# OndrejSladky/kmercamel

Hardware: NVIDIA B200
Metric: distinct k-mers/sec for `compute` (k=31, canonical, device-timed) (higher is better)
Workload: dtype u64

## Files before the change

### kmercamel_b200/csrc/emit.cuh

```cuda
#pragma once
#include "engine.cuh"

template <int L> struct NodeSeq {
    const KWord<L> *kmers;
    const u8 *seq;
    const u64 *rec_off, *rec_len;
    u32 n;
    int k;
    KC_HD u64 length(u32 v) const { return kmers ? (u64) k : rec_len[v < n ? v : v - n]; }
    KC_HD u32 symbol(u32 v, u64 pos) const {
        if (kmers) {
            if (v < n) return kmer_symbol(kmers[v], k, (int) pos);
            return 3u - kmer_symbol(kmers[v - n], k, k - 1 - (int) pos);
        }
        if (v < n) return kc_nucleotide_code(seq[rec_off[v] + pos]);
        u32 u = v - n;
        return 3u - kc_nucleotide_code(seq[rec_off[u] + rec_len[u] - 1 - pos]);
    }
};

KC_HD u8 kc_letter(u32 sym, bool upper) {
    const u32 packed = 'A' | ('C' << 8) | ('G' << 16) | ('T' << 24);
    u8 c = (u8) (packed >> (8 * sym));
    return upper ? c : (u8) (c + ('a' - 'A'));
}

template <int L> KC_HD u64 kmer_lower_bound(const KWord<L> *keys, u64 n, const KWord<L> &x) {
    u64 lo = 0, hi = n;
    while (lo < hi) {
        u64 mid = (lo + hi) >> 1;
        if (keys[mid] < x) lo = mid + 1;
        else hi = mid;
    }
    return lo;
}

template <int L> struct KmerIndex {
    const u32 *start = nullptr;
    int bits = 0, shift = 0;
};

template <int L> KC_HD bool kmer_set_contains(const KWord<L> *keys, u64 n, const KmerIndex<L> &ix, const KWord<L> &x) {
    u64 lo = 0, hi = n;
    if (ix.start) {
        const u32 b = x.digit(ix.shift, ix.bits);
        lo = ix.start[b];
        hi = ix.start[b + 1];
    }
    while (lo < hi) {
        const u64 mid = (lo + hi) >> 1;
        if (keys[mid] < x) lo = mid + 1;
        else hi = mid;
    }
    return lo < n && keys[lo] == x;
}

static const u32 KC_EMIT_SHORT = 128;
static const u32 KC_EMIT_CHUNK = 16384;
static const u32 KC_EMIT_SUB = 4;

#ifdef __CUDACC__
template <int L> KmerIndex<L> kc_kmer_index_build(CudaExec &ex, const KWord<L> *keys, u64 n, int k) {
    KmerIndex<L> ix;
    if (n < 1024 || n >= 0xFFFFFFFFULL) return ix;
    int bits = kc_ceil_log2(n) - 1;
    if (bits > 24) bits = 24;
    if (bits > 2 * k) bits = 2 * k;
    const u64 nb = 1ULL << bits;
    u32 *start = ex.alloc<u32>(nb + 1);
    const int shift = 2 * k - bits;
    ex.for_each(n + 1, [=] __device__(u64 i) {
        const u64 b_prev = i == 0 ? 0 : (u64) keys[i - 1].digit(shift, bits) + 1;
        const u64 b_cur = i == n ? nb : (u64) keys[i].digit(shift, bits);
        for (u64 b = b_prev; b <= b_cur; ++b) start[b] = (u32) i;
    }, KP_MISC, n * sizeof(KWord<L>) + nb * 4);
    ix.start = start;
    ix.bits = bits;
    ix.shift = shift;
    return ix;
}

static const u32 KC_RANK_SMALL = 1024;

template <int L>
__global__ void __launch_bounds__(256) kc_rank_small_kernel(PathState s, NodeSeq<L> q, u32 N, u32 *fin_out, u64 *dist_out, u64 *cell) {
    __shared__ u32 jump[2][KC_RANK_SMALL], fin[2][KC_RANK_SMALL];
    __shared__ u64 dist[2][KC_RANK_SMALL];
    __shared__ u32 s_start, s_cyc;
    if (threadIdx.x == 0) {
        s_start = KC_NONE;
        s_cyc = 0;
    }
    __syncthreads();
    for (u32 v = threadIdx.x; v < N; v += 256) {
        const u32 nx = s.edge_from[v];
        jump[0][v] = nx;
        fin[0][v] = v;
        dist[0][v] = q.length(v) - (nx != KC_NONE ? (u64) s.ovl[v] : 0);
        if (s.edge_to[v] == KC_NONE) atomicMin(&s_start, v);
    }
    __syncthreads();
    int rounds = 1;
    while ((1u << (rounds - 1)) < N) ++rounds;
    int cur = 0;
    for (int it = 0; it < rounds; ++it) {
        for (u32 v = threadIdx.x; v < N; v += 256) {
            const u32 j = jump[cur][v];
            if (j == KC_NONE) {
                jump[cur ^ 1][v] = KC_NONE;
                fin[cur ^ 1][v] = fin[cur][v];
                dist[cur ^ 1][v] = dist[cur][v];
            } else {
                jump[cur ^ 1][v] = jump[cur][j];
                fin[cur ^ 1][v] = fin[cur][j];
                dist[cur ^ 1][v] = dist[cur][v] + dist[cur][j];
            }
        }
        __syncthreads();
        cur ^= 1;
    }
    for (u32 v = threadIdx.x; v < N; v += 256) {
        fin_out[v] = fin[cur][v];
        dist_out[v] = dist[cur][v];
        if (jump[cur][v] != KC_NONE) s_cyc = 1;
    }
    __syncthreads();
    if (threadIdx.x == 0) {
        const u32 st0 = s_start;
        cell[0] = st0 == KC_NONE ? ~0ULL : (u64) st0;
        cell[1] = s_cyc ? 0 : 1;
        cell[2] = st0 < N ? dist[cur][st0] : 0;
        cell[3] = st0 < N ? fin[cur][st0] : 0;
    }
}
#endif

struct EmitResult {
    u8 *ms = nullptr;
    u8 *maxone = nullptr;
    u64 length = 0;
    u64 n_printed = 0;
    u64 slice_begin = 0, slice_len = 0;
};

template <class Exec, int L>
EmitResult kc_emit_superstring(Exec &ex, const NodeSeq<L> &ns, const NodeView<L> &nv, const PathState &st,
                               const KWord<L> *set_keys, u64 n_set, bool want_maxone, u32 slice_index = 0, u32 n_slices = 1, u64 total_ub = 0) {
    EmitResult res;
    const u64 N = nv.N;
    const int k = nv.k;
    size_t mark = ex.arena->mark();
    u32 *jump_a = ex.template alloc<u32>(N), *jump_b = ex.template alloc<u32>(N);
    u32 *fin_a = ex.template alloc<u32>(N), *fin_b = ex.template alloc<u32>(N);
    u64 *dist_a = ex.template alloc<u64>(N), *dist_b = ex.template alloc<u64>(N);
    u64 *cell = ex.template alloc<u64>(6);
    const PathState s = st;
    const NodeSeq<L> q = ns;
    bool ranked = false;
#ifdef __CUDACC__
    if constexpr (Exec::is_device) {
        if (N <= KC_RANK_SMALL) {
            typename Exec::Scope sc(ex, KP_RANK, N * 25);
            kc_rank_small_kernel<L><<<1, 256, 0, ex.stream>>>(s, q, (u32) N, fin_a, dist_a, cell);
            ++ex.launches;
            KC_CUDA(cudaGetLastError());
            ranked = true;
        }
    }
#endif
    if (!ranked) {
        ex.fill_bytes(cell, 0xFF, 16);
        ex.for_each(N, [=] KC_HD_LAMBDA(u64 vv) {
            u32 v = (u32) vv;
            u32 nx = s.edge_from[v];
            jump_a[v] = nx;
            fin_a[v] = v;
            dist_a[v] = q.length(v) - (nx != KC_NONE ? (u64) s.ovl[v] : 0);
            if (s.edge_to[v] == KC_NONE) KC_ATOMIC_MIN((kc_ull *) &cell[0], (kc_ull) v);
        }, KP_RANK, N * 25);
        int rounds = kc_ceil_log2(N) + 1;
        for (int it = 0; it < rounds; ++it) {
            const u32 *ja = jump_a, *fa = fin_a;
            const u64 *da = dist_a;
            u32 *jb = jump_b, *fb = fin_b;
            u64 *db = dist_b;
            ex.for_each(N, [=] KC_HD_LAMBDA(u64 v) {
                u32 j = ja[v];
                if (j == KC_NONE) {
                    jb[v] = KC_NONE;
                    fb[v] = fa[v];
                    db[v] = da[v];
                } else {
                    jb[v] = ja[j];
                    fb[v] = fa[j];
                    db[v] = da[v] + da[j];
                }
            }, KP_RANK, N * 32);
            u32 *t = jump_a; jump_a = jump_b; jump_b = t;
            t = fin_a; fin_a = fin_b; fin_b = t;
            u64 *m = dist_a; dist_a = dist_b; dist_b = m;
        }
        {
            const u32 *ja = jump_a;
            ex.for_each(N, [=] KC_HD_LAMBDA(u64 v) {
                if (ja[v] != KC_NONE) cell[1] = 0;
            });
            const u32 *fa = fin_a;
            const u64 *da = dist_a;
            const u64 NN = N;
            ex.for_each(1, [=] KC_HD_LAMBDA(u64) {
                const u64 st0 = cell[0];
                cell[2] = st0 < NN ? da[st0] : 0;
                cell[3] = st0 < NN ? fa[st0] : 0;
            });
        }
    }
    bool deferred = false;
#ifdef __CUDACC__
    if constexpr (Exec::is_device) deferred = ranked && total_ub && !ns.kmers && !want_maxone && n_slices == 1;
#endif
    const u64 *cellp = deferred ? cell : nullptr;
    u64 info[4] = {0, 1, total_ub, 0};
    if (!deferred) {
        ex.read_n(cell, info, 4);
        const u64 start = info[0];
        if (start >= N) KC_THROW(KC_ERR_INTERNAL, "no start node: the path cover contains only cycles");
        if (info[1] == 0) KC_THROW(KC_ERR_INTERNAL, "cycle in the final path cover");
    }
    const u64 total_h = info[2];
    const u32 fin_start_h = (u32) info[3];
    const u64 total = total_h;
    if (n_slices > 1 && (ns.kmers || want_maxone)) KC_THROW(KC_ERR_ARG, "sliced emission is for record nodes without -M");
    const u64 s_begin = n_slices > 1 ? ((total / n_slices) * slice_index) & ~(u64) 15 : 0;
    const u64 s_end_h = n_slices > 1 && slice_index + 1 < n_slices ? ((total / n_slices) * (slice_index + 1)) & ~(u64) 15 : total;
    const u64 s_end = s_end_h;
    const u32 fin_start = fin_start_h;
    u8 *ms_base = ex.template alloc<u8>(s_end - s_begin + 1);
    u8 *ms = ms_base - s_begin;
    res.ms = ms_base;
    res.length = total;
    res.slice_begin = s_begin;
    res.slice_len = s_end - s_begin;
    const u32 *fa = fin_a;
    const u64 *da = dist_a;
    if (ns.kmers) {
        ex.for_each(N, [=] KC_HD_LAMBDA(u64 vv) {
            u32 v = (u32) vv;
            if (fa[v] != fin_start) return;
            u64 off = total - da[v];
            u32 cnt = (u32) (k - (s.edge_from[v] != KC_NONE ? (int) s.ovl[v] : 0));
            KWord<L> x = q.kmers[v < q.n ? v : v - q.n];
            if (v >= q.n) x = kmer_reverse_complement(x, k);
            for (u32 j = 0; j < cnt; ++j) ms[off + j] = kc_letter(kmer_symbol(x, k, (int) j), j == 0);
        }, KP_EMIT, N * 12 + (u64) q.n * sizeof(KWord<L>) + total);
    } else {
        u32 *chunks = ex.template alloc<u32>(N + 1);
        ex.for_each(N + 1, [=] KC_HD_LAMBDA(u64 vv) {
            const u64 total = cellp ? cellp[2] : total_h;
            const u32 fin_start = cellp ? (u32) cellp[3] : fin_start_h;
            const u64 s_end = cellp ? total : s_end_h;
            u32 c = 0;
            if (vv < N && fa[vv] == fin_start) {
                u32 v = (u32) vv;
                u64 cnt = q.length(v) - (s.edge_from[v] != KC_NONE ? (u64) s.ovl[v] : 0);
                if (cnt > KC_EMIT_SHORT) {
                    u64 off = total - da[v];
                    const u64 a0 = off & ~(u64) 15, a1 = off + cnt;
                    const u64 lo = a0 > s_begin ? a0 : s_begin, hi = a1 < s_end ? a1 : s_end;
                    if (lo < hi) c = (u32) ((hi - a0 + KC_EMIT_CHUNK - 1) / KC_EMIT_CHUNK - (lo - a0) / KC_EMIT_CHUNK);
                }
            }
            chunks[vv] = c;
        }, KP_EMIT, N * 12);
        u32 n_chunks = 0;
        bool bounded = false;
#ifdef __CUDACC__
        if constexpr (Exec::is_device) {
            if (N <= 65536) {
                bounded = true;
                ex.exclusive_scan_nosync(chunks, chunks, N + 1);
                n_chunks = (u32) ((s_end - s_begin) / KC_EMIT_CHUNK + 2 * N + 1);
            }
        }
#endif
        if (!bounded) n_chunks = ex.exclusive_scan(chunks, chunks, N + 1);
        ex.for_each(N, [=] KC_HD_LAMBDA(u64 vv) {
            const u64 total = cellp ? cellp[2] : total_h;
            const u32 fin_start = cellp ? (u32) cellp[3] : fin_start_h;
            const u64 s_end = cellp ? total : s_end_h;
            u32 v = (u32) vv;
            if (fa[v] != fin_start) return;
            u64 len = q.length(v);
            u64 cnt = len - (s.edge_from[v] != KC_NONE ? (u64) s.ovl[v] : 0);
            if (cnt > KC_EMIT_SHORT) return;
            u64 off = total - da[v];
            if (off >= s_end || off + cnt <= s_begin) return;
            u64 n_upper = len - k + 1;
            for (u64 j = 0; j < cnt; ++j)
                if (off + j >= s_begin && off + j < s_end) ms[off + j] = kc_letter(q.symbol(v, j), j < n_upper);
        }, KP_EMIT, N * 12);
        ex.for_each((u64) n_chunks * 256, [=] KC_HD_LAMBDA(u64 w) {
            const u64 total = cellp ? cellp[2] : total_h;
            const u64 s_end = cellp ? total : s_end_h;
            u32 chunk = (u32) (w >> 8), lane = (u32) (w & 255);
            if (chunk >= chunks[N]) return;
            u32 lo = 0, hi = (u32) N;
            while (lo < hi) {
                u32 mid = (lo + hi + 1) >> 1;
                if (chunks[mid] <= chunk) lo = mid;
                else hi = mid - 1;
            }
            u32 v = lo;
            u64 len = q.length(v);
            u64 cnt = len - (s.edge_from[v] != KC_NONE ? (u64) s.ovl[v] : 0);
            u64 n_upper = len - k + 1;
            u64 off = total - da[v];
            const u64 n0 = off & ~(u64) 15;
            const u64 skip = n0 < s_begin ? (s_begin - n0) / KC_EMIT_CHUNK : 0;
            const u64 c0 = n0 + ((u64) (chunk - chunks[v]) + skip) * KC_EMIT_CHUNK + (u64) lane * 16;
            static_assert(KC_EMIT_CHUNK == KC_EMIT_SUB * 256 * 16, "a chunk is 256 work items x KC_EMIT_SUB x 16 bytes");
            for (u32 sub = 0; sub < KC_EMIT_SUB; ++sub) {
            u64 a0 = c0 + (u64) sub * (256 * 16);
            u64 b0 = a0 < off ? off : a0;
            u64 b1 = a0 + 16 < off + cnt ? a0 + 16 : off + cnt;
            if (b0 < s_begin) b0 = s_begin;
            if (b1 > s_end) b1 = s_end;
            if (b0 >= b1) continue;
            const u64 j0 = b0 - off;
#ifdef __CUDA_ARCH__
            const bool one_case = j0 + 16 <= n_upper || j0 >= n_upper;
#else
            const bool one_case = false;
#endif
            if (b1 - b0 == 16 && one_case) {
#ifdef __CUDA_ARCH__
                const u32 u = v < q.n ? v : v - q.n;
                const u64 src0 = v < q.n ? q.rec_off[u] + j0 : q.rec_off[u] + q.rec_len[u] - 16 - j0;
                const u32 *wp = reinterpret_cast<const u32 *>(q.seq + (src0 & ~(u64) 3));
                const u32 sh = (u32) (src0 & 3) * 8;
                u32 in[5];
#pragma unroll
                for (int x = 0; x < 4; ++x) in[x] = wp[x];
                in[4] = sh ? wp[4] : 0u;
                u32 wd[4];
#pragma unroll
                for (int x = 0; x < 4; ++x) wd[x] = __funnelshift_r(in[x], in[x + 1], sh) & 0xDFDFDFDFu;
                if (v >= q.n) {
                    u32 r[4];
#pragma unroll
                    for (int x = 0; x < 4; ++x) {
                        const u32 t = __byte_perm(wd[3 - x], 0u, 0x0123);
                        const u32 cg = ((t >> 1) & 0x01010101u) * 0xFFu;
                        r[x] = t ^ ((cg & 0x04040404u) | (~cg & 0x15151515u));
                    }
#pragma unroll
                    for (int x = 0; x < 4; ++x) wd[x] = r[x];
                }
                if (j0 >= n_upper) {
#pragma unroll
                    for (int x = 0; x < 4; ++x) wd[x] |= 0x20202020u;
                }
                *reinterpret_cast<uint4 *>(ms + b0) = make_uint4(wd[0], wd[1], wd[2], wd[3]);
#endif
            } else if (b1 - b0 == 16) {
                u32 wd[4];
                u64 j = b0 - off;
                for (int x = 0; x < 4; ++x) {
                    u32 t = 0;
                    for (int y = 0; y < 4; ++y) t |= (u32) kc_letter(q.symbol(v, j + 4 * x + y), j + 4 * x + y < n_upper) << (8 * y);
                    wd[x] = t;
                }
                *reinterpret_cast<uint4 *>(ms + b0) = make_uint4(wd[0], wd[1], wd[2], wd[3]);
            } else {
                for (u64 a = b0; a < b1; ++a) ms[a] = kc_letter(q.symbol(v, a - off), a - off < n_upper);
            }
            }
        }, KP_EMIT, 2 * total);
    }
    if (want_maxone) {
        u8 *mo = ex.template alloc<u8>(total + 1);
        res.maxone = mo;
        const bool complements = nv.complements;
        KmerIndex<L> ix;
#ifdef __CUDACC__
        if constexpr (Exec::is_device) ix = kc_kmer_index_build<L>(ex, set_keys, n_set, k);
#endif
        ex.for_each(total, [=] KC_HD_LAMBDA(u64 p) {
            u8 c = ms[p];
            if (c <= 'Z' || p + k > total) {
                mo[p] = c;
                return;
            }
            KWord<L> x = KWord<L>::zero();
            for (int i = 0; i < k; ++i) x = x.shl(2) | KWord<L>::from_u64(kc_nucleotide_code(ms[p + i]));
            if (complements) {
                KWord<L> r = kmer_reverse_complement(x, k);
                if (r < x) x = r;
            }
            const bool present = kmer_set_contains(set_keys, n_set, ix, x);
            mo[p] = present ? (u8) (c - ('a' - 'A')) : c;
        }, KP_MAXONE, 2 * total);
    }
    if (deferred) {
        ex.read_n(cell, info, 4);
        if (info[0] >= N) KC_THROW(KC_ERR_INTERNAL, "no start node: the path cover contains only cycles");
        if (info[1] == 0) KC_THROW(KC_ERR_INTERNAL, "cycle in the final path cover");
        if (info[2] > total_ub) KC_THROW(KC_ERR_INTERNAL, "superstring longer than its bound");
        res.length = info[2];
        res.slice_len = info[2];
    }
    res.n_printed = nv.n;
    (void) mark;
    return res;
}
```

### kmercamel_b200/csrc/engine.cuh

```cuda
#pragma once
#include "exec.cuh"
#include "kword.cuh"
#include "sort.cuh"
#ifdef KC_HOST_EMUL
#include <algorithm>
#endif

template <int L> struct NodeView {
    const KWord<L> *first;
    const KWord<L> *last;
    u32 n, N;
    int k;
    bool complements;
    KC_HD u32 mirror(u32 v) const { return v < n ? v + n : v - n; }
    KC_HD KWord<L> first_kmer(u32 v) const { return v < n ? first[v] : kmer_reverse_complement(last[v - n], k); }
    KC_HD KWord<L> last_kmer(u32 v) const { return v < n ? last[v] : kmer_reverse_complement(first[v - n], k); }
};

struct PathState {
    u32 *edge_from;
    u32 *edge_to;
    u8 *ovl;
    u32 *chain_head;
    u32 *chain_tail;
// ... 87 lines not shown
        if (owns_suffix(t, ka, kb)) c.head_w[t] = h;
        if (owns_prefix(h, ka, kb)) c.tail_w[h] = t;
    }

    KC_HD void operator()(u64 g) const {
        const KWord<L + 1> *T = c.T;
        const u64 p_beg = group_pstart[g];
        const KWord<L> ka = tuple_key(T[p_beg]);
        KWord<L> kb = ka;
        bool two = false;
        if (c.nv.complements) {
            kb = kmer_reverse_complement(ka, c.d);
            if (kb < ka) return;
            two = kb != ka;
        }
        const u64 meta_max = (1ULL << 37) - 1;
        const u64 s_beg = tuple_lower_bound(T, (u64) 0, p_beg, tuple_make(ka, 0));
        const u64 s_end = p_beg;
        const u64 pa_end = tuple_lower_bound(T, p_beg, c.nt, tuple_make(ka, meta_max));
        u64 s2_beg = 0, s2_end = 0, p2_beg = 0, p2_end = 0;
        if (two) {
            s2_beg = tuple_lower_bound(T, (u64) 0, c.nt, tuple_make(kb, 0));
            s2_end = tuple_lower_bound(T, s2_beg, c.nt, tuple_make(kb, KC_ROLE_P));
            p2_beg = s2_end;
            p2_end = tuple_lower_bound(T, p2_beg, c.nt, tuple_make(kb, meta_max));
        }
        u64 ca = p_beg, cb = p2_beg;
        for (u32 part = 0; part < 16; ++part) {
            u64 ra0 = ca;
            while (ca < pa_end && tuple_part(T[ca]) == part) ++ca;
            u64 ra1 = ca;
            u64 rb0 = cb;
            while (cb < p2_end && tuple_part(T[cb]) == part) ++cb;
            u64 rb1 = cb;
            if (ra0 == ra1 && rb0 == rb1) continue;
            u64 fa = ra0, fb = rb0;
            u64 ia = s_beg, ib = s2_beg;
            while (true) {
                u32 va = (ia < s_end && fa < ra1) ? tuple_node(T[ia]) : KC_NONE;
                u32 vb = (ib < s2_end && fb < rb1) ? tuple_node(T[ib]) : KC_NONE;
                if (va == KC_NONE && vb == KC_NONE) break;
                u32 i;
                u64 *front;
                u64 rend;
                if (va < vb) {
                    i = va;
                    ++ia;
                    front = &fa;
                    rend = ra1;
                } else {
                    i = vb;
                    ++ib;
                    front = &fb;
                    rend = rb1;
                }
                if (c.st.edge_from[i] != KC_NONE) continue;
                while (*front < rend && c.st.edge_to[tuple_node(T[*front])] != KC_NONE) ++*front;
                for (u64 q = *front; q < rend; ++q) {
                    u32 j = tuple_node(T[q]);
                    if (c.st.edge_to[j] != KC_NONE) continue;
                    if (c.check_cycles) {
                        if (c.nv.complements && j == c.nv.mirror(i)) continue;
                        if (j == c.head_w[i]) continue;
                        if (banned(i, j)) continue;
                    }
                    u64 stampv = ((u64) part << 32) | i;
                    link(i, j, stampv, 1, ka, kb);
                    if (c.nv.complements) link(c.nv.mirror(j), c.nv.mirror(i), stampv, 0, ka, kb);
                    break;
                }
            }
        }
    }
};

#ifdef __CUDACC__
#include <cooperative_groups.h>
__global__ void __launch_bounds__(256) kc_doubling_kernel(u32 *jump_a, u32 *jump_b, u32 *fin_a, u32 *fin_b, u64 *max_a, u64 *max_b, u32 ne, int rounds,
                                                          u32 *active , const u32 *ne_dev ) {
    cooperative_groups::grid_group grid = cooperative_groups::this_grid();
    if (ne_dev) ne = *ne_dev;
    u32 *ja = jump_a, *jb = jump_b, *fa = fin_a, *fb = fin_b;
    u64 *ma = max_a, *mb = max_b;
    const u32 stride = gridDim.x * blockDim.x;
    int it = 0;
    for (; it < rounds; ++it) {
        bool any = false;
        for (u32 r = blockIdx.x * blockDim.x + threadIdx.x; r < ne; r += stride) {
            const u32 j = ja[r];
            if (j == KC_NONE) {
                jb[r] = KC_NONE;
                fb[r] = fa[r];
                mb[r] = ma[r];
            } else {
                any = true;
                jb[r] = ja[j];
                fb[r] = fa[j];
                const u64 m1 = ma[r], m2 = ma[j];
                mb[r] = m1 > m2 ? m1 : m2;
            }
        }
        if (__syncthreads_or(any) && threadIdx.x == 0) atomicOr(&active[it % 3], 1u);
        if (blockIdx.x == 0 && threadIdx.x == 0) active[(it + 1) % 3] = 0;
        grid.sync();
        u32 *t = ja; ja = jb; jb = t;
        t = fa; fa = fb; fb = t;
        u64 *m = ma; ma = mb; mb = m;
        const u32 more = *reinterpret_cast<volatile u32 *>(&active[it % 3]);
        if (!more) {
            ++it;
            break;
        }
    }
    if (ja != jump_a) {
        grid.sync();
        for (u32 r = blockIdx.x * blockDim.x + threadIdx.x; r < ne; r += stride) {
            jump_a[r] = ja[r];
            fin_a[r] = fa[r];
            max_a[r] = ma[r];
        }
    }
}
#endif

#include "small_engine.cuh"

struct EngineStats {
    u64 levels_run = 0, tuples_sorted = 0, groups = 0, edges = 0, ban_rounds = 0, bans = 0;
};

template <class Exec, int L> struct Engine {
    Exec &ex;
    NodeView<L> nv;
    PathState st;
    bool strict;
    bool lower_bound;
    bool use_small = true;
    bool fast_levels = true;
    int small_threads_opt = 0;
    EngineStats stats;

    u32 *live_s = nullptr, *live_p = nullptr;
    u32 *list_buf[4] = {nullptr, nullptr, nullptr, nullptr};
    int list_gen = 0;
    u64 n_s = 0, n_p = 0;
    u32 *head_w, *tail_w, *slot_of;
    u64 *stamp;
    u8 *prim, *ban_flag;
    u32 *ban_i, *ban_j, *ban_ctr;
    static const u32 BAN_CAP = 1u << 20;

    Engine(Exec &e, const NodeView<L> &v, bool strict_, bool lower_bound_) : ex(e), nv(v), strict(strict_), lower_bound(lower_bound_) {}

    void init_state() {
        const u64 N = nv.N;
        st.edge_from = ex.template alloc<u32>(N);
        st.edge_to = ex.template alloc<u32>(N);
        st.ovl = ex.template alloc<u8>(N);
        st.chain_head = ex.template alloc<u32>(N);
        st.chain_tail = ex.template alloc<u32>(N);
        head_w = ex.template alloc<u32>(N);
        tail_w = ex.template alloc<u32>(N);
        slot_of = ex.template alloc<u32>(N);
        stamp = ex.template alloc<u64>(N);
        prim = ex.template alloc<u8>(N);
        ban_flag = ex.template alloc<u8>(N);
        ban_i = ex.template alloc<u32>(BAN_CAP);
        ban_j = ex.template alloc<u32>(BAN_CAP);
        ban_ctr = ex.template alloc<u32>(4);
        PathState s = st;
        u8 *bf = ban_flag;
        u32 *bc = ban_ctr;
        ex.for_each(N, [=] KC_HD_LAMBDA(u64 v) {
            s.edge_from[v] = KC_NONE;
            s.edge_to[v] = KC_NONE;
            s.ovl[v] = 255;
            bf[v] = 0;
            s.chain_head[v] = (u32) v;
            s.chain_tail[v] = (u32) v;
            if (v < 4) bc[v] = 0;
        });
        if (N < 4) ex.fill_bytes(ban_ctr, 0, 16);
        n_s = n_p = N;
    }

    void run() {
        for (int d = nv.k - 1; d >= 0; --d) {
            const u64 done = lower_bound ? 0 : (nv.complements ? 2 : 1);
            if (n_s <= done) break;
            if (run_small(d)) break;
            run_level(d);
        }
    }

    u32 *small_out = nullptr;
    int small_d = 0;

    void check_small() {
#ifdef __CUDACC__
        if constexpr (Exec::is_device) {
            if (!small_out) return;
            u32 h[8 + 128 + 8];
            ex.read_n(small_out, h, 8 + 128 + 8);
            small_out = nullptr;
            if (std::getenv("KC_TRACE")) {
                std::fprintf(stderr, "[kc_trace] small engine: n_s=%llu n_p=%llu levels=%u groups=%u edges=%u ban_rounds=%u bans=%u; clocks per level (* = run):",
                             (unsigned long long) n_s, (unsigned long long) n_p, h[1], h[2], h[3], h[4], h[5]);
                for (int dd = small_d; dd >= 0; --dd) std::fprintf(stderr, " d%d=%u%s", dd, h[8 + dd] & 0x7FFFFFFFu, (h[8 + dd] >> 31) ? "*" : "");
                std::fprintf(stderr, "; phases: stage+mask=%u tuples=%u sort=%u groups=%u replay=%u validate+commit=%u lists=%u writeback=%u\n", h[136], h[137],
                             h[138], h[139], h[140], h[141], h[142], h[143]);
            }
            if (h[0]) KC_THROW(KC_ERR_INTERNAL, "ban list overflow");
            stats.levels_run += h[1];
            stats.groups += h[2];
            stats.edges += h[3];
            stats.ban_rounds += h[4];
            stats.bans += h[5];
        }
#endif
    }

    bool run_small(int d) {
#ifdef __CUDACC__
        if constexpr (Exec::is_device) {
            if (!use_small || lower_bound || n_s + n_p > SmallCfg<L>::T) return false;
            if (!live_s) {
                u32 *a = ex.template alloc<u32>(n_s), *b = ex.template alloc<u32>(n_p);
                ex.for_each(nv.N, [=] KC_HD_LAMBDA(u64 i) {
                    a[i] = (u32) i;
                    b[i] = (u32) i;
                });
                live_s = a;
                live_p = b;
            }
            SmallEngineArgs<L> a;
            a.nv = nv;
            a.st = st;
            a.live_s_a = live_s;
            a.live_p_a = live_p;
            a.live_s_b = ex.template alloc<u32>(n_s);
            a.live_p_b = ex.template alloc<u32>(n_p);
            a.n_s = (u32) n_s;
            a.n_p = (u32) n_p;
            a.head_w = head_w;
            a.tail_w = tail_w;
            a.slot_of = slot_of;
            a.stamp = stamp;
            a.prim = prim;
            a.ban_flag = ban_flag;
            a.ban_i = ban_i;
            a.ban_j = ban_j;
            a.ban_cap = BAN_CAP;
            a.d_start = d;
            a.strict = strict;
            a.out = ex.template alloc<u32>(8 + 128 + 8 + 4 + 8 * (n_s + n_p));
            u32 *lvl_mask = a.out + (8 + 128 + 8);
            ex.fill_bytes(a.out, 0, (8 + 128 + 8 + 4 + 4 * (n_s + n_p)) * 4);
            a.lvl_mask_in = lvl_mask;
            a.end_mask_s_a = lvl_mask + 4;
            a.end_mask_p_a = a.end_mask_s_a + 4 * n_s;
            a.end_mask_s_b = a.end_mask_p_a + 4 * n_p;
            a.end_mask_p_b = a.end_mask_s_b + 4 * n_s;
            const int mask_smem = (int) (SmallCfg<L>::T * sizeof(KWord<L + 1>));
            static KcDevOnce once;
            once.run([&](int) {
                KC_CUDA(cudaFuncSetAttribute(kc_small_engine_kernel<L>, cudaFuncAttributeMaxDynamicSharedMemorySize,
                                             (int) SmallCfg<L>::SMEM));
                KC_CUDA(cudaFuncSetAttribute(kc_small_level_mask_kernel<L>, cudaFuncAttributeMaxDynamicSharedMemorySize, mask_smem));
            });
            {
                typename Exec::Scope sc(ex, KP_SMALL_ENGINE, 0);
                const u32 per_cta = kc_small_mask_levels_per_cta<L>((u32) n_s, (u32) n_p);
                kc_small_level_mask_kernel<L><<<(unsigned) kc_div_up((u64) d + 1, per_cta), 256, mask_smem, ex.stream>>>(nv, live_s, live_p, (u32) n_s, (u32) n_p, d,
                                                                                                                      lvl_mask, a.end_mask_s_a, a.end_mask_p_a);
                ++ex.launches;
            }
            {
                typename Exec::Scope sc(ex, KP_SMALL_ENGINE, 0);
                const u64 nt0 = n_s + n_p;
                const unsigned small_threads = small_threads_opt ? (unsigned) small_threads_opt : ((nt0 > 128 && nt0 <= 256) || nt0 > 512 ? 512u : 256u);
                kc_small_engine_kernel<L><<<1, small_threads, SmallCfg<L>::SMEM, ex.stream>>>(a);
            }
            ++ex.launches;
            KC_CUDA(cudaGetLastError());
            small_out = a.out;
            small_d = d;
            return true;
        }
#endif
        (void) d;
        return false;
    }

    void run_level(int d) {
        typedef KWord<L + 1> TW;
        const u64 nt = n_s + n_p;
        if (n_s == 0 || n_p == 0) return;
        ++stats.levels_run;
        stats.tuples_sorted += nt;
        if (!list_buf[0]) {
            for (int i = 0; i < 4; ++i) list_buf[i] = ex.template alloc<u32>(i < 2 ? n_s : n_p);
        }
        size_t mark = ex.arena->mark();
        TW *T = ex.template alloc<TW>(nt);
        TW *T2 = ex.template alloc<TW>(nt);
        const NodeView<L> v = nv;
        const u32 batch = strict ? nv.N / 16 + 1 : nv.N + 1;
        const u32 *ls = live_s, *lp = live_p;
        const u64 ns = n_s, np = n_p;
        u32 *hw = head_w, *tw = tail_w;
        const PathState s = st;
        ex.for_each(nt, [=] KC_HD_LAMBDA(u64 i) {
            if (i < ns) {
                u32 x = ls ? ls[i] : (u32) i;
                T[i] = tuple_make(kmer_suffix(v.last_kmer(x), d), (u64) x);
                hw[x] = s.chain_head[x];
            } else {
                u32 x = lp ? lp[i - ns] : (u32) (i - ns);
                u64 meta = KC_ROLE_P | ((u64) (x / batch) << 32) | (u64) (u32) ~x;
                T[i] = tuple_make(kmer_prefix(v.first_kmer(x), v.k, d), meta);
                tw[x] = s.chain_tail[x];
            }
        }, KP_TUPLES, nt * (sizeof(KWord<L>) + sizeof(TW)));
        exec_sort<L + 1>(ex, T, T2, nt, 64 + 2 * d);
        u32 *group_pstart = ex.template alloc<u32>(np);
        const TW *Tc = T;
        auto is_group = [=] KC_HD_LAMBDA(u64 i) {
            if (i == 0) return false;
            TW a = Tc[i - 1], b = Tc[i];
            return tuple_is_prefix(b) && !tuple_is_prefix(a) && tuple_key(a) == tuple_key(b);
        };
        auto put_group = [=] KC_HD_LAMBDA(u64 i, u32 r) { group_pstart[r] = (u32) i; };
        LevelCtx<L> c;
        c.nv = nv;
        c.st = st;
        c.T = T;
        c.nt = nt;
        c.d = d;
        c.batch = batch;
        c.head_w = head_w;
        c.tail_w = tail_w;
        c.stamp = stamp;
        c.prim = prim;
        c.ban_flag = ban_flag;
        c.ban_i = ban_i;
        c.ban_j = ban_j;
        c.n_bans = 0;
        c.check_cycles = !lower_bound;
        u32 *new_tail = ex.template alloc<u32>(ns);
        u32 *so = slot_of;
        auto has_edge = [=] KC_HD_LAMBDA(u64 i) { return s.edge_from[ls ? ls[i] : (u32) i] != KC_NONE; };
        auto put_edge = [=] KC_HD_LAMBDA(u64 i, u32 r) {
            u32 x = ls ? ls[i] : (u32) i;
            new_tail[r] = x;
            so[x] = r;
        };
        u64 n_groups = 0, n_edges = 0;
        u32 n_bans = 0;
        bool settled = false, lists_done = false, cycles_pending = false;
#ifdef __CUDACC__
        if constexpr (Exec::is_device) if (fast_levels && (lower_bound || doubling_blocks() > 0)) {
            u64 *cells = ex.template alloc<u64>(6);
            ex.fill_bytes(cells, 0, 40);
            ex.fill_bytes(cells + 5, 0xFF, 8);
            u32 *c_groups = reinterpret_cast<u32 *>(cells), *c_edges = reinterpret_cast<u32 *>(cells + 1);
            u32 *c_ns = reinterpret_cast<u32 *>(cells + 2), *c_np = reinterpret_cast<u32 *>(cells + 3);
            ex.compact_if_nosync(nt, is_group, put_group, c_groups);
            {
                SimulatePairFn<L> sim{c, group_pstart};
                ex.for_each(ns < np ? ns : np, [=] __device__(u64 g) {
                    if (g < *c_groups) sim(g);
                }, KP_SIMULATE);
            }
            ex.compact_if_nosync(ns, has_edge, put_edge, c_edges);
            bool queued = true;
            u32 *jump_a = nullptr, *fin_a = nullptr;
            u64 *max_a = nullptr;
            if (!lower_bound) {
                const u32 ub = (u32) ns;
                jump_a = ex.template alloc<u32>(ub);
                u32 *jump_b = ex.template alloc<u32>(ub);
                fin_a = ex.template alloc<u32>(ub);
                u32 *fin_b = ex.template alloc<u32>(ub);
                max_a = ex.template alloc<u64>(ub);
                u64 *max_b = ex.template alloc<u64>(ub);
                const u64 *stp = stamp;
                u32 *ja = jump_a, *fa = fin_a;
                u64 *ma = max_a;
                ex.for_each(ub, [=] __device__(u64 r) {
                    if (r >= *c_edges) return;
                    u32 x = new_tail[r];
                    u32 t = s.chain_tail[s.edge_from[x]];
                    bool cont = s.edge_from[t] != KC_NONE;
                    ja[r] = cont ? so[t] : KC_NONE;
                    fa[r] = t;
                    ma[r] = stp[x];
                }, KP_DOUBLING, (u64) ub * 36);
                queued = doubling_fused(jump_a, jump_b, fin_a, fin_b, max_a, max_b, ub, kc_ceil_log2(ub) + 1, c_edges);
                if (queued) {
                    ex.for_each(ub, [=] __device__(u64 r) {
                        if (r < *c_edges && ja[r] != KC_NONE) {
                            atomicAdd((kc_ull *) &cells[4], (kc_ull) 1);
                            atomicMin((kc_ull *) &cells[5], (kc_ull) ma[r]);
                        }
                    });
                    ex.for_each(ub, [=] __device__(u64 r) {
                        if (r >= *c_edges || cells[4] != 0) return;
                        u32 x = new_tail[r];
                        u32 h = s.chain_head[x];
                        if (s.edge_to[h] == KC_NONE) {
                            u32 t = fa[r];
                            s.chain_tail[h] = t;
                            s.chain_head[t] = h;
                        }
                    }, KP_COMMIT, (u64) ub * 16);
                }
            }
            if (queued) {
                const u32 *src_s = live_s, *src_p = live_p;
                u32 *dst_s = list_buf[list_gen], *dst_p = list_buf[2 + list_gen];
                ex.compact_if_nosync(ns, [=] __device__(u64 i) { return s.edge_from[src_s ? src_s[i] : (u32) i] == KC_NONE; },
                                     [=] __device__(u64 i, u32 r) { dst_s[r] = src_s ? src_s[i] : (u32) i; }, c_ns);
                ex.compact_if_nosync(np, [=] __device__(u64 i) { return s.edge_to[src_p ? src_p[i] : (u32) i] == KC_NONE; },
                                     [=] __device__(u64 i, u32 r) { dst_p[r] = src_p ? src_p[i] : (u32) i; }, c_np);
                u64 h[5];
                ex.read_n(cells, h, 5);
                n_groups = h[0];
                n_edges = h[1];
                stats.groups += n_groups;
                if (h[4] == 0) {
                    settled = true;
                    if (n_edges) {
                        live_s = dst_s;
                        live_p = dst_p;
                        list_gen ^= 1;
                        n_s = h[2];
                        n_p = h[3];
                    }
// ... 244 lines not shown
```

### kmercamel_b200/csrc/exec.cuh

```cuda
#pragma once
#include <cstring>
#include "kc_common.cuh"
#include <vector>

#ifdef __CUDA_ARCH__
#define KC_ATOMIC_ADD(ptr, v) atomicAdd((ptr), (v))
#define KC_ATOMIC_MIN(ptr, v) atomicMin((ptr), (v))
#define KC_ATOMIC_MAX(ptr, v) atomicMax((ptr), (v))
#define KC_ATOMIC_OR(ptr, v) atomicOr((ptr), (v))
#else
template <typename T> inline T kc_host_atomic_add(T *p, T v) { T o = *p; *p = o + v; return o; }
template <typename T> inline T kc_host_atomic_min(T *p, T v) { T o = *p; if (v < o) *p = v; return o; }
template <typename T> inline T kc_host_atomic_max(T *p, T v) { T o = *p; if (v > o) *p = v; return o; }
template <typename T> inline T kc_host_atomic_or(T *p, T v) { T o = *p; *p = o | v; return o; }
#define KC_ATOMIC_ADD(ptr, v) kc_host_atomic_add((ptr), (v))
#define KC_ATOMIC_MIN(ptr, v) kc_host_atomic_min((ptr), (v))
#define KC_ATOMIC_MAX(ptr, v) kc_host_atomic_max((ptr), (v))
#define KC_ATOMIC_OR(ptr, v) kc_host_atomic_or((ptr), (v))
#endif

typedef unsigned long long kc_ull;

enum KcProfId {
    KP_EXTRACT, KP_SORT_HIST, KP_SORT_SCATTER, KP_SORT_LOCAL, KP_SORT_MISC, KP_COMPACT, KP_SCAN, KP_TUPLES,
// ... 19 lines not shown
    u32 incl = v;
#pragma unroll
    for (int o = 1; o < 32; o <<= 1) {
        u32 t = __shfl_up_sync(0xFFFFFFFFu, incl, o);
        if (lane >= (u32) o) incl += t;
    }
    if (lane == 31) smem_warp[warp] = incl;
    __syncthreads();
    u32 warp_prefix = 0, sum = 0;
#pragma unroll
    for (int wi = 0; wi < 8; ++wi) {
        u32 s = smem_warp[wi];
        if ((u32) wi < warp) warp_prefix += s;
        sum += s;
    }
    __syncthreads();
    *total = sum;
    return warp_prefix + incl - v;
}

static const int KC_CP_ITEMS = 4;
static const int KC_CP_TILE = KC_FE_THREADS * KC_CP_ITEMS;

template <typename Pred>
__global__ void __launch_bounds__(KC_FE_THREADS) kc_compact_count_kernel(u64 n, Pred pred, u32 *block_counts, u32 *grand_total = nullptr) {
    __shared__ u32 sw[8];
    u64 base = (u64) blockIdx.x * KC_CP_TILE + (u64) threadIdx.x * KC_CP_ITEMS;
    u32 c = 0;
#pragma unroll
    for (int j = 0; j < KC_CP_ITEMS; ++j)
        if (base + j < n && pred(base + j)) ++c;
    u32 total;
    kc_block_exclusive_scan_256(c, &total, sw);
    if (threadIdx.x == 0) {
        block_counts[blockIdx.x] = total;
        if (grand_total && total) atomicAdd(grand_total, total);
    }
}

template <typename Pred, typename Emit>
__global__ void __launch_bounds__(KC_FE_THREADS) kc_compact_emit_kernel(u64 n, Pred pred, Emit emit, const u32 *block_offsets) {
    __shared__ u32 sw[8];
    u64 base = (u64) blockIdx.x * KC_CP_TILE + (u64) threadIdx.x * KC_CP_ITEMS;
    bool keep[KC_CP_ITEMS];
    u32 c = 0;
#pragma unroll
    for (int j = 0; j < KC_CP_ITEMS; ++j) {
        keep[j] = base + j < n && pred(base + j);
        c += keep[j];
    }
    u32 total;
    u32 rank = kc_block_exclusive_scan_256(c, &total, sw) + block_offsets[blockIdx.x];
#pragma unroll
    for (int j = 0; j < KC_CP_ITEMS; ++j)
        if (keep[j]) emit(base + j, rank++);
}

__global__ void __launch_bounds__(KC_FE_THREADS) kc_scan_tile_kernel(const u32 *in, u32 *out, u64 n, u32 *tile_sums) {
    __shared__ u32 sw[8];
    u64 base = (u64) blockIdx.x * 1024 + (u64) threadIdx.x * 4;
    u32 v[4], c = 0;
#pragma unroll
    for (int j = 0; j < 4; ++j) {
        v[j] = base + j < n ? in[base + j] : 0;
        c += v[j];
    }
    u32 total;
    u32 p = kc_block_exclusive_scan_256(c, &total, sw);
#pragma unroll
    for (int j = 0; j < 4; ++j) {
        if (base + j < n) out[base + j] = p;
        p += v[j];
    }
    if (threadIdx.x == 0 && tile_sums) tile_sums[blockIdx.x] = total;
}

__global__ void __launch_bounds__(KC_FE_THREADS) kc_scan_walk_kernel(const u32 *in, u32 *out, u64 n, u32 *sum) {
    __shared__ u32 sw[8];
    u32 carry = 0;
    for (u64 t0 = 0; t0 < n; t0 += 1024) {
        const u64 base = t0 + (u64) threadIdx.x * 4;
        u32 v[4], c = 0;
#pragma unroll
        for (int j = 0; j < 4; ++j) {
            v[j] = base + j < n ? in[base + j] : 0;
            c += v[j];
        }
        u32 total;
        u32 p = kc_block_exclusive_scan_256(c, &total, sw) + carry;
#pragma unroll
        for (int j = 0; j < 4; ++j) {
            if (base + j < n) out[base + j] = p;
            p += v[j];
        }
        carry += total;
        __syncthreads();
    }
    if (threadIdx.x == 0 && sum) *sum = carry;
}

__global__ void __launch_bounds__(KC_FE_THREADS) kc_scan_add_kernel(u32 *out, u64 n, const u32 *tile_offsets) {
    u64 base = (u64) blockIdx.x * 1024 + (u64) threadIdx.x * 4;
    u32 o = tile_offsets[blockIdx.x];
#pragma unroll
    for (int j = 0; j < 4; ++j)
        if (base + j < n) out[base + j] += o;
}

struct KernelProf {
    bool enabled = false;
    double ms[KP_COUNT] = {0};
    u64 launches[KP_COUNT] = {0};
    u64 bytes[KP_COUNT] = {0};
    struct Rec {
        int id;
        cudaEvent_t a, b;
    };
    std::vector<Rec> pending;
    std::vector<cudaEvent_t> pool;
    cudaEvent_t get() {
        if (!pool.empty()) {
            cudaEvent_t e = pool.back();
            pool.pop_back();
            return e;
        }
        cudaEvent_t e;
        KC_CUDA(cudaEventCreate(&e));
        return e;
    }
    void resolve() {
        for (Rec &r : pending) {
            float t = 0;
            if (cudaEventElapsedTime(&t, r.a, r.b) == cudaSuccess) ms[r.id] += t;
            ++launches[r.id];
            pool.push_back(r.a);
            pool.push_back(r.b);
        }
        pending.clear();
    }
    void reset() {
        for (int i = 0; i < KP_COUNT; ++i) {
            ms[i] = 0;
            launches[i] = 0;
            bytes[i] = 0;
        }
    }
};

struct CudaExec {
    cudaStream_t stream;
    Arena *arena;
    KernelProf *prof = nullptr;
    u64 launches = 0;
    u8 *pinned = nullptr;
    size_t pinned_cap = 0;

    struct Scope {
        CudaExec &ex;
        bool on;
        KernelProf::Rec rec;
        Scope(CudaExec &e, int id, u64 bytes = 0) : ex(e), on(e.prof && e.prof->enabled) {
            if (!on) return;
            rec.id = id;
            rec.a = ex.prof->get();
            rec.b = ex.prof->get();
            ex.prof->bytes[id] += bytes;
            cudaEventRecord(rec.a, ex.stream);
        }
        ~Scope() {
            if (!on) return;
            cudaEventRecord(rec.b, ex.stream);
            ex.prof->pending.push_back(rec);
        }
    };

    static constexpr bool is_device = true;

    template <typename T> T *alloc(size_t n) { return arena->alloc<T>(n); }

    template <typename F> void for_each(u64 n, F f, int id = KP_MISC, u64 bytes = 0) {
        if (n == 0) return;
        Scope sc(*this, id, bytes);
        u64 blocks = kc_div_up(n, KC_FE_THREADS);
        if (blocks > 0x7FFFFFFFULL) KC_THROW(KC_ERR_TOO_LARGE, "for_each grid too large");
        kc_for_each_kernel<<<(unsigned) blocks, KC_FE_THREADS, 0, stream>>>(n, f);
        ++launches;
        KC_CUDA(cudaGetLastError());
    }

    void fill_bytes(void *p, int value, size_t bytes) {
        if (bytes) KC_CUDA(cudaMemsetAsync(p, value, bytes, stream));
    }
    void copy_bytes(void *dst, const void *src, size_t bytes) {
        if (bytes) KC_CUDA(cudaMemcpyAsync(dst, src, bytes, cudaMemcpyDeviceToDevice, stream));
    }
    template <typename T> T read(const T *p) {
        T v;
        read_n(p, &v, 1);
        return v;
    }
    void sync() { KC_CUDA(cudaStreamSynchronize(stream)); }
    template <typename T> void read_n(const T *p, T *host, size_t n) {
        const size_t bytes = n * sizeof(T);
        if (pinned && bytes <= pinned_cap) {
            KC_CUDA(cudaMemcpyAsync(pinned, p, bytes, cudaMemcpyDeviceToHost, stream));
            KC_CUDA(cudaStreamSynchronize(stream));
            std::memcpy(host, pinned, bytes);
            return;
        }
        KC_CUDA(cudaMemcpyAsync(host, p, bytes, cudaMemcpyDeviceToHost, stream));
        KC_CUDA(cudaStreamSynchronize(stream));
    }

    u32 exclusive_scan(const u32 *in, u32 *out, u64 n) {
        if (n == 0) return 0;
        size_t m = arena->mark();
        u32 total = scan_rec(in, out, n, true);
        arena->release(m);
        return total;
    }

    void exclusive_scan_nosync(const u32 *in, u32 *out, u64 n) {
        if (n == 0) return;
        size_t m = arena->mark();
        scan_rec(in, out, n, false);
        arena->release(m);
    }

    template <typename Pred, typename Emit> u64 compact_if(u64 n, Pred pred, Emit emit, u64 bytes = 0) {
        if (n == 0) return 0;
        if (n >= 0xFFFFFFFFULL) KC_THROW(KC_ERR_TOO_LARGE, "compact_if over more than 2^32-1 items");
        Scope sc(*this, KP_COMPACT, bytes);
        size_t m = arena->mark();
        u64 blocks = kc_div_up(n, KC_CP_TILE);
        u32 *counts = arena->alloc<u32>(blocks);
        kc_compact_count_kernel<<<(unsigned) blocks, KC_FE_THREADS, 0, stream>>>(n, pred, counts);
        ++launches;
        KC_CUDA(cudaGetLastError());
        u32 total = scan_rec(counts, counts, blocks, true);
        kc_compact_emit_kernel<<<(unsigned) blocks, KC_FE_THREADS, 0, stream>>>(n, pred, emit, counts);
        ++launches;
        KC_CUDA(cudaGetLastError());
        arena->release(m);
        return total;
    }

    template <typename Pred, typename Emit> void compact_if_nosync(u64 n, Pred pred, Emit emit, u32 *total_dev, u64 bytes = 0) {
        if (n == 0) return;
        if (n >= 0xFFFFFFFFULL) KC_THROW(KC_ERR_TOO_LARGE, "compact_if over more than 2^32-1 items");
        Scope sc(*this, KP_COMPACT, bytes);
        size_t m = arena->mark();
        u64 blocks = kc_div_up(n, KC_CP_TILE);
        u32 *counts = arena->alloc<u32>(blocks);
        kc_compact_count_kernel<<<(unsigned) blocks, KC_FE_THREADS, 0, stream>>>(n, pred, counts, total_dev);
        ++launches;
        KC_CUDA(cudaGetLastError());
        scan_rec(counts, counts, blocks, false);
        kc_compact_emit_kernel<<<(unsigned) blocks, KC_FE_THREADS, 0, stream>>>(n, pred, emit, counts);
        ++launches;
        KC_CUDA(cudaGetLastError());
        arena->release(m);
    }

  private:
    u32 scan_rec(const u32 *in, u32 *out, u64 n, bool want_total) {
        u64 tiles = kc_div_up(n, 1024);
        if (tiles <= 8) {
            u32 *sum = arena->alloc<u32>(1);
            kc_scan_walk_kernel<<<1, KC_FE_THREADS, 0, stream>>>(in, out, n, sum);
            ++launches;
            KC_CUDA(cudaGetLastError());
            return want_total ? read(sum) : 0;
        }
        u32 *sums = arena->alloc<u32>(tiles);
        kc_scan_tile_kernel<<<(unsigned) tiles, KC_FE_THREADS, 0, stream>>>(in, out, n, sums);
        ++launches;
        KC_CUDA(cudaGetLastError());
        u32 total = scan_rec(sums, sums, tiles, want_total);
        kc_scan_add_kernel<<<(unsigned) tiles, KC_FE_THREADS, 0, stream>>>(out, n, sums);
        ++launches;
        KC_CUDA(cudaGetLastError());
        return total;
    }
};

#endif

#ifdef KC_HOST_EMUL
struct HostExec {
    Arena *arena;
    u64 launches = 0;
    static constexpr bool is_device = false;
    template <typename T> T *alloc(size_t n) { return arena->alloc<T>(n); }
    template <typename F> void for_each(u64 n, F f, int = 0, u64 = 0) {
        for (u64 i = 0; i < n; ++i) f(i);
    }
    void fill_bytes(void *p, int value, size_t bytes) { std::memset(p, value, bytes); }
    void copy_bytes(void *dst, const void *src, size_t bytes) { std::memmove(dst, src, bytes); }
    template <typename T> T read(const T *p) { return *p; }
    template <typename T> void read_n(const T *p, T *host, size_t n) { std::memcpy(host, p, n * sizeof(T)); }
    void sync() {}
    u32 exclusive_scan(const u32 *in, u32 *out, u64 n) {
        u32 s = 0;
        for (u64 i = 0; i < n; ++i) {
            u32 v = in[i];
            out[i] = s;
            s += v;
        }
        return s;
    }
    template <typename Pred, typename Emit> u64 compact_if(u64 n, Pred pred, Emit emit, u64 = 0) {
        u64 r = 0;
        for (u64 i = 0; i < n; ++i)
            if (pred(i)) emit(i, (u32) r++);
        return r;
    }
};
#endif
```

### kmercamel_b200/csrc/kcgpu.cu

```cuda
#include "../../include/kcgpu.h"

#include "emit.cuh"
#include "engine.cuh"
#include "exec.cuh"
#include "group.cuh"
#include "kmerset.cuh"
#include "kmerset_fast.cuh"
#include "kmerset_sig.cuh"
#include "kword.cuh"
#include "masks.cuh"
#include "runs.cuh"
#include "sort.cuh"
#include "stage1.cuh"

#include <chrono>
#include <mutex>
#include <new>
#include <string>
#include <thread>
#include <vector>

static double kc_now_ms() {
    return std::chrono::duration<double, std::milli>(std::chrono::steady_clock::now().time_since_epoch()).count();
}
static const bool kc_trace = std::getenv("KC_TRACE") != nullptr;
#define KC_TRACE_POINT(label)                                                               \
    do {                                                                                    \
        if (kc_trace) std::fprintf(stderr, "[kc_trace] %-28s %.3f ms\n", (label), kc_now_ms()); \
    } while (0)

struct kc_ctx {
    int device = 0;
    cudaStream_t stream = nullptr;
    bool own_stream = false;
    Arena arena;
    KernelProf prof;
    u8 *pin_in = nullptr;
    size_t pin_in_cap = 0;
    u8 *pin_out = nullptr;
    size_t pin_out_cap = 0;
    static const size_t KC_PIN_SMALL = 4096;
    u8 *pin_small = nullptr;
    cudaEvent_t ev[6] = {nullptr, nullptr, nullptr, nullptr, nullptr, nullptr};
    static const int KC_H2D_CHUNKS = 4;
    cudaStream_t copy_stream = nullptr;
    cudaEvent_t chunk_ev[KC_H2D_CHUNKS] = {nullptr, nullptr, nullptr, nullptr};
    bool small_engine = true;
    int small_threads = 0;
    bool sparse_switch = true;
    KsfTuning fast;
    u64 fast_runs = 0, fast_fallbacks = 0;
    SigTuning sig;
    u64 sig_runs = 0, sig_fallbacks = 0;
    u64 sig_overflow_bytes = 0;
    bool fast_heuristics = true;
    u64 fast_overflow_bytes = 0;
    u64 total_launches = 0;
    KcGroup grp;
    bool arena_limited = false;
    std::string last_error;
};

namespace {

void set_error(kc_ctx *ctx, const KcError &e) {
    if (!ctx) return;
    char buf[512];
    std::snprintf(buf, sizeof(buf), "%s (%s:%d)", e.what, e.file, e.line);
    ctx->last_error = buf;
}

#define KC_API_BEGIN try {
#define KC_API_END(ctx)                                                \
    }                                                                  \
    catch (const KcError &e) {                                         \
        set_error((ctx), e);                                           \
        return e.code;                                                 \
    }                                                                  \
    catch (const std::bad_alloc &) {                                   \
        if (ctx) (ctx)->last_error = "host allocation failed";         \
        return KC_ERR_OOM;                                             \
    }                                                                  \
    catch (...) {                                                      \
        if (ctx) (ctx)->last_error = "unknown failure";                \
        return KC_ERR_INTERNAL;                                        \
    }

void check_params(const kc_params *p) {
    if (!p) KC_THROW(KC_ERR_ARG, "params is NULL");
    if (p->k < 1 || p->k > 127) KC_THROW(KC_ERR_ARG, "k must be in 1..127");
    if (p->min_frequency < 1 || p->min_frequency > 255) KC_THROW(KC_ERR_ARG, "min_frequency must be in 1..255");
    if (p->min_frequency != 1 && p->assume_simplitigs) KC_THROW(KC_ERR_ARG, "-z is not compatible with -S");
}

#define KC_LARGE_ONLY "inputs of 2^32 bytes or more are built by the signature construction only (k >= 26, no -z, no -M, no -S)"
void check_large_input(const kc_ctx *ctx, const kc_params *p, u64 n_bytes) {
    if (n_bytes < KC_POS32_BYTES) return;
    if (p->assume_simplitigs) KC_THROW(KC_ERR_TOO_LARGE, KC_LARGE_ONLY "; -S was asked");
    if (p->min_frequency > 1) KC_THROW(KC_ERR_TOO_LARGE, KC_LARGE_ONLY "; -z (min_frequency > 1) was asked");
    if (p->want_maxone) KC_THROW(KC_ERR_TOO_LARGE, KC_LARGE_ONLY "; -M (want_maxone) was asked");
    if (p->k < 26) KC_THROW(KC_ERR_TOO_LARGE, KC_LARGE_ONLY "; k is below 26");
    if (!ctx->sig.enabled) KC_THROW(KC_ERR_TOO_LARGE, KC_LARGE_ONLY "; it is switched off (option sig_set = 0)");
    if (!kc_sig_plan(n_bytes, p->k, ctx->sig).ok) KC_THROW(KC_ERR_TOO_LARGE, KC_LARGE_ONLY "; its bucket plan does not fit this input");
}

void ensure_arena(kc_ctx *ctx, size_t need) {
    need = (need + 4095) & ~(size_t) 4095;
    if (ctx->arena.cap >= need) return;
    if (ctx->arena.cap && ctx->arena_limited && need >= ctx->arena.cap) return;
    if (ctx->arena.base) {
        KC_CUDA(cudaFree(ctx->arena.base));
        ctx->arena.base = nullptr;
        ctx->arena.cap = 0;
    }
    size_t free_b = 0, total_b = 0;
    KC_CUDA(cudaMemGetInfo(&free_b, &total_b));
    size_t limit = (size_t) (free_b * 0.92);
    size_t want = need < limit ? need : (limit & ~(size_t) 4095);
    ctx->arena_limited = want < need;
    KC_CUDA(cudaMalloc(&ctx->arena.base, want));
    ctx->arena.cap = want;
    ctx->arena.reset();
}

size_t estimate_arena(u64 n_bytes, u64 n_recs, int limbs, bool complements, bool simplitigs, bool pessimistic = false,
                      const KsfTuning *fast = nullptr, const SigPlan *sig = nullptr) {
    const double wb = 8.0 * limbs;
    const double c = complements ? 2.0 : 1.0;
    double stage1 = n_bytes * (1.0 + 2.0 * (wb + 4.0) + 1.0 + 1.0 + 0.2);
    if (n_bytes >= KC_POS32_BYTES && sig && sig->ok) {
        stage1 = n_bytes * (1.0 + 0.125) + (double) kc_sig_arena_bytes(*sig, n_bytes);
    } else if (fast) {
        const KsfPlan pl = kc_ksf_plan(n_bytes, *fast);
        if (pl.ok) {
            const double f = n_bytes * 1.2 + (double) (pl.slots[0] + pl.slots[1]) * (wb + 4.0) + (double) pl.n_leaf * 28.0 + 65536.0;
            if (f > stage1) stage1 = f;
        }
    }
    double nodes = simplitigs ? (double) n_recs : (pessimistic ? n_bytes * 0.85 : n_bytes / 64.0 + 1e6);
    double N = c * nodes;
    double engine = N * (60.0 + 2.0 * 2.0 * (wb + 8.0) + 12.0 + 40.0);
    double emit = N * 32.0 + 3.0 * n_bytes;
    double total = (stage1 + engine + emit) * 1.1 + (256u << 20);
    return (size_t) total;
}

template <class F> void run_with_arena(kc_ctx *ctx, size_t need, size_t need_max, F body) {
    ensure_arena(ctx, need);
    try {
        ctx->arena.reset();
        body();
    } catch (const KcError &e) {
        if (e.code != KC_ERR_OOM || need_max <= ctx->arena.cap || ctx->arena_limited) throw;
        KC_CUDA(cudaStreamSynchronize(ctx->stream));
        ensure_arena(ctx, need_max);
        ctx->arena.reset();
        body();
    }
}

struct DevInput {
    const u8 *seq;
    u64 n_bytes;
    const u64 *rec_off, *rec_len;
    u64 n_recs;
    InputChunks *chunks = nullptr;
};

struct DevResult {
    const u8 *ms = nullptr, *maxone = nullptr;
    u64 length = 0, n_kmers = 0, n_occ = 0, n_nodes = 0, n_simplitigs = 0;
    u64 lower_bound = 0;
    u64 slice_begin = 0, slice_len = 0;
};

template <int L> u64 run_stage1(kc_ctx *ctx, CudaExec &ex, const DevInput &in, const kc_params &p, KWord<L> **uniq_out, u8 **cnt_out,
                               u64 *n_occ) {
    KC_CUDA(cudaEventRecord(ctx->ev[0], ex.stream));
    KC_CUDA(cudaEventRecord(ctx->ev[1], ex.stream));
    if (in.chunks) in.chunks->wait_all(ex.stream);
    KmerSet<L> set = kc_kmerset_build<L>(ex, in.seq, in.n_bytes, p.k, p.complements != 0, p.min_frequency, nullptr, true);
    KC_CUDA(cudaEventRecord(ctx->ev[2], ex.stream));
    *n_occ = set.n_occ;
    *uniq_out = set.keys;
    *cnt_out = set.cnt;
    return set.n_kept;
}

template <int L>
u64 run_stage1_runs(kc_ctx *ctx, CudaExec &ex, const DevInput &in, const kc_params &p, RunNodes *runs, KWord<L> **set_out, u64 *n_occ) {
    KC_CUDA(cudaEventRecord(ctx->ev[0], ex.stream));
    KC_CUDA(cudaEventRecord(ctx->ev[1], ex.stream));
    KC_TRACE_POINT("stage1: begin");
    const u64 nb = in.n_bytes;
    const size_t fwords = kc_runs_flag_words(nb);
    u32 *flags = ex.arena->alloc_top<u32>(fwords);
    ex.fill_bytes(flags, 0, fwords * 4);
    u64 *cells = ex.arena->alloc_top<u64>(2);
    ex.fill_bytes(cells, 0, 16);
    const bool expect_duplicates = ctx->fast_heuristics && (p.min_frequency > 1 || (ctx->fast_overflow_bytes && nb >= ctx->fast_overflow_bytes / 2 && nb <= ctx->fast_overflow_bytes * 2));
    const bool large = nb >= KC_POS32_BYTES;
    const bool sig_overflowed = ctx->fast_heuristics && ctx->sig_overflow_bytes && nb >= ctx->sig_overflow_bytes / 2 && nb <= ctx->sig_overflow_bytes * 2;
    if (!p.want_maxone && p.min_frequency == 1 && (large || !sig_overflowed)) {
        u64 *cells4 = ex.arena->alloc_top<u64>(4);
        ex.fill_bytes(cells4, 0, 32);
        if (kc_kmerset_build_sig<L>(ex, in.seq, nb, p.k, p.complements != 0, flags, cells4, ctx->sig, in.chunks)) {
            KC_TRACE_POINT("stage1: signature set launched");
            u64 hc[4];
            bool aborted = false;
            *runs = kc_runs_from_flags(ex, flags, nb, p.k, cells4, hc, 4, &aborted);
            if (!aborted) {
                ++ctx->sig_runs;
                *n_occ = hc[2];
                *set_out = nullptr;
                KC_CUDA(cudaEventRecord(ctx->ev[2], ex.stream));
                return hc[2] ? hc[0] : 0;
            }
            ++ctx->sig_fallbacks;
            ctx->sig_overflow_bytes = nb;
            if (large) KC_THROW(KC_ERR_TOO_LARGE, KC_LARGE_ONLY "; it overflowed on this input (too repetitive)");
            ex.fill_bytes(flags, 0, fwords * 4);
        }
    }
    if (large) KC_THROW(KC_ERR_INTERNAL, "an input of 2^32 bytes or more reached the 32-bit set constructions");
    if (!p.want_maxone && !expect_duplicates) {
        KsfPlan plan;
        u64 *cells4 = ex.arena->alloc_top<u64>(4);
        ex.fill_bytes(cells4, 0, 32);
        if (kc_kmerset_build_fast<L>(ex, in.seq, nb, p.k, p.complements != 0, p.min_frequency, flags, cells4, ctx->fast, &plan, in.chunks)) {
            KC_TRACE_POINT("stage1: fast set launched");
            u64 hc[4];
            bool aborted = false;
            *runs = kc_runs_from_flags(ex, flags, nb, p.k, cells4, hc, 4, &aborted);
            if (!aborted) {
                ++ctx->fast_runs;
                if (ex.prof && ex.prof->enabled && nb > hc[2]) {
                    const u64 d = (nb - hc[2]) * (sizeof(KWord<L>) + 4);
                    ex.prof->bytes[KP_KS_SCATTER0] -= d;
                    ex.prof->bytes[KP_SORT_SCATTER] -= 2 * d * (u64) (plan.n_levels - 1);
                    ex.prof->bytes[KP_KS_RESOLVE] -= d;
                }
                *n_occ = hc[2];
                *set_out = nullptr;
                KC_CUDA(cudaEventRecord(ctx->ev[2], ex.stream));
                return hc[2] ? hc[0] : 0;
            }
            ++ctx->fast_fallbacks;
            ctx->fast_overflow_bytes = nb;
            ex.fill_bytes(flags, 0, fwords * 4);
        }
    }
    if (in.chunks) in.chunks->wait_all(ex.stream);
    KmerSet<L> set = kc_kmerset_build<L>(ex, in.seq, nb, p.k, p.complements != 0, p.min_frequency, flags, p.want_maxone != 0, cells);
    KC_TRACE_POINT("stage1: set built");
    *n_occ = set.n_occ;
    *set_out = set.keys;
    if (set.n_occ == 0 || set.n_kept == 0) {
        KC_CUDA(cudaEventRecord(ctx->ev[2], ex.stream));
        return 0;
    }
    if (p.want_maxone) {
        const u64 kept = set.n_kept;
        KC_CUDA(cudaMemcpyAsync(cells, &kept, 8, cudaMemcpyHostToDevice, ex.stream));
    }
    u64 host_cells[2];
    *runs = kc_runs_from_flags(ex, flags, nb, p.k, cells, host_cells);
    const u64 n_kept = p.want_maxone ? set.n_kept : host_cells[0];
    KC_TRACE_POINT("stage1: runs built");
    KC_CUDA(cudaEventRecord(ctx->ev[2], ex.stream));
    return n_kept;
}

struct ExtFlags {
    const u32 *flags = nullptr;
    u64 kept = 0, n_occ = 0;
    u64 *cells4 = nullptr;
    bool aborted = false;
};

template <int L>
void run_pipeline(kc_ctx *ctx, CudaExec &ex, const DevInput &in, const kc_params &p, DevResult &res, ExtFlags *ext = nullptr,
                  bool lower_bound = false, u32 slice_index = 0, u32 n_slices = 1) {
    const bool complements = p.complements != 0;
    KWord<L> *uniq = nullptr;
    u8 *cnt = nullptr;
    u64 U = 0, n_occ = 0;
    NodeView<L> nv;
    NodeSeq<L> ns;
    nv.k = p.k;
    nv.complements = complements;
    ns.k = p.k;
    ns.kmers = nullptr;
    ns.seq = in.seq;
    ns.rec_off = in.rec_off;
    ns.rec_len = in.rec_len;
    u64 n_nodes = 0;
    const u64 *node_off = in.rec_off, *node_len = in.rec_len;
    if (in.chunks && (p.assume_simplitigs || ext)) in.chunks->wait_all(ex.stream);
    if (!p.assume_simplitigs) {
        RunNodes runs;
        if (ext && ext->cells4) {
            u64 hc[4];
            runs = kc_runs_from_flags(ex, ext->flags, in.n_bytes, p.k, ext->cells4, hc, 4, &ext->aborted);
            if (ext->aborted) {
                ext->kept = hc[3];
                return;
            }
            U = hc[2] ? hc[0] : 0;
            n_occ = hc[2];
            KC_CUDA(cudaEventRecord(ctx->ev[2], ex.stream));
        } else if (ext) {
            u64 *cells = ex.arena->alloc_top<u64>(2);
            ex.fill_bytes(cells, 0, 16);
            u64 host_cells[2];
            runs = kc_runs_from_flags(ex, ext->flags, in.n_bytes, p.k, cells, host_cells);
            U = runs.n_runs ? ext->kept : 0;
            n_occ = ext->n_occ;
            KC_CUDA(cudaEventRecord(ctx->ev[2], ex.stream));
        } else {
            U = run_stage1_runs<L>(ctx, ex, in, p, &runs, &uniq, &n_occ);
        }
        if (U == 0) KC_THROW(KC_ERR_EMPTY, "the input contains no k-mers");
        res.n_simplitigs = runs.n_runs;
        if (ctx->sparse_switch && runs.n_runs * 5 >= U) runs = kc_kmer_nodes_from_runs(ex, in.seq, runs, p.k);
        n_nodes = runs.n_runs;
        node_off = runs.rec_off;
        node_len = runs.rec_len;
        if (n_nodes * (complements ? 2 : 1) >= 0xFFFFFFF0ULL) KC_THROW(KC_ERR_TOO_LARGE, "too many nodes for one GPU");
    } else {
        if (in.n_recs == 0) KC_THROW(KC_ERR_EMPTY, "input cannot be empty");
        if (in.n_recs * (complements ? 2 : 1) >= 0xFFFFFFF0ULL) KC_THROW(KC_ERR_TOO_LARGE, "too many records for one GPU");
        KC_CUDA(cudaEventRecord(ctx->ev[0], ex.stream));
        if (p.want_maxone) {
            U = run_stage1<L>(ctx, ex, in, p, &uniq, &cnt, &n_occ);
        } else {
            KC_CUDA(cudaEventRecord(ctx->ev[1], ex.stream));
            KC_CUDA(cudaEventRecord(ctx->ev[2], ex.stream));
        }
        n_nodes = in.n_recs;
        res.n_simplitigs = in.n_recs;
    }
    {
        KWord<L> *first = ex.alloc<KWord<L>>(n_nodes), *last = ex.alloc<KWord<L>>(n_nodes);
        u32 *err = ex.alloc<u32>(1);
        ex.fill_bytes(err, 0, 4);
        kc_extract_node_ends<L>(ex, in.seq, in.n_bytes, node_off, node_len, n_nodes, p.k, first, last, err,
                                p.assume_simplitigs != 0);
        if (p.assume_simplitigs && ex.read(err)) KC_THROW(KC_ERR_BAD_SEQ, "-S input must hold only ACGT records of at least k bases");
        nv.first = first;
        nv.last = last;
        nv.n = (u32) n_nodes;
        ns.rec_off = node_off;
        ns.rec_len = node_len;
    }
    nv.N = nv.n * (complements ? 2u : 1u);
    ns.n = nv.n;
    KC_TRACE_POINT("pipeline: nodes ready");
    Engine<CudaExec, L> eng(ex, nv, p.assume_simplitigs != 0, lower_bound);
    eng.use_small = ctx->small_engine;
    eng.small_threads_opt = ctx->small_threads;
    eng.init_state();
    eng.run();
    KC_TRACE_POINT("pipeline: engine done");
    KC_CUDA(cudaEventRecord(ctx->ev[3], ex.stream));
    if (lower_bound) {
        kc_ull *acc = reinterpret_cast<kc_ull *>(ex.alloc<u64>(2));
        ex.fill_bytes(acc, 0, 16);
        const u64 *len = node_off == in.rec_off ? in.rec_len : node_len;
        const u8 *ovl = eng.st.ovl;
        const u32 n = nv.n;
        ex.for_each(nv.N, [=] __device__(u64 i) {
            if (i < n) atomicAdd(&acc[0], (kc_ull) len[i]);
            if (ovl[i]) atomicAdd(&acc[1], (kc_ull) ovl[i]);
        });
        u64 h[2];
        ex.read_n(reinterpret_cast<const u64 *>(acc), h, 2);
        eng.check_small();
        const u64 strands = complements ? 2 : 1;
        res.lower_bound = (h[0] * strands - h[1]) / strands;
        KC_CUDA(cudaEventRecord(ctx->ev[4], ex.stream));
        res.n_kmers = U;
        res.n_occ = n_occ;
        res.n_nodes = nv.n;
        return;
    }
    EmitResult er;
    try {
        er = kc_emit_superstring<CudaExec, L>(ex, ns, nv, eng.st, uniq, U, p.want_maxone != 0, slice_index, n_slices, in.n_bytes + n_nodes * (u64) p.k + 16);
    } catch (const KcError &) {
        eng.check_small();
        throw;
    }
    KC_CUDA(cudaEventRecord(ctx->ev[4], ex.stream));
    eng.check_small();
    res.ms = er.ms;
    res.maxone = er.maxone;
    res.length = er.length;
    res.slice_begin = er.slice_begin;
    res.slice_len = er.slice_len;
    res.n_kmers = U;
    res.n_occ = n_occ;
    res.n_nodes = nv.n;
}

void dispatch_pipeline(kc_ctx *ctx, CudaExec &ex, const DevInput &in, const kc_params &p, DevResult &res, bool lower_bound = false) {
    if (p.k < 32) run_pipeline<1>(ctx, ex, in, p, res, nullptr, lower_bound);
    else if (p.k < 64) run_pipeline<2>(ctx, ex, in, p, res, nullptr, lower_bound);
    else run_pipeline<4>(ctx, ex, in, p, res, nullptr, lower_bound);
}

void fill_times(kc_ctx *ctx, kc_output *out) {
    float t = 0;
    out->t = kc_stage_times{0, 0, 0, 0, 0};
    if (cudaEventElapsedTime(&t, ctx->ev[0], ctx->ev[1]) == cudaSuccess) out->t.extract_ms = t;
    if (cudaEventElapsedTime(&t, ctx->ev[1], ctx->ev[2]) == cudaSuccess) out->t.count_ms = t;
    if (cudaEventElapsedTime(&t, ctx->ev[2], ctx->ev[3]) == cudaSuccess) out->t.path_ms = t;
    if (cudaEventElapsedTime(&t, ctx->ev[3], ctx->ev[4]) == cudaSuccess) out->t.emit_ms = t;
    if (cudaEventElapsedTime(&t, ctx->ev[0], ctx->ev[4]) == cudaSuccess) out->t.total_ms = t;
    (void) cudaGetLastError();
}

template <int L>
void count_only(kc_ctx *ctx, CudaExec &ex, const DevInput &in, const kc_params &p, uint64_t **keys, uint8_t **counts, uint64_t *n) {
    KWord<L> *uniq = nullptr;
    u8 *cnt = nullptr;
    u64 n_occ = 0;
    u64 U = run_stage1<L>(ctx, ex, in, p, &uniq, &cnt, &n_occ);
    *n = U;
    *keys = (uint64_t *) std::malloc(U ? U * sizeof(KWord<L>) : 8);
    *counts = (uint8_t *) std::malloc(U ? U : 1);
    if (!*keys || !*counts) KC_THROW(KC_ERR_OOM, "host allocation failed");
    if (U) {
        KC_CUDA(cudaMemcpyAsync(*keys, uniq, U * sizeof(KWord<L>), cudaMemcpyDeviceToHost, ex.stream));
        KC_CUDA(cudaMemcpyAsync(*counts, cnt, U, cudaMemcpyDeviceToHost, ex.stream));
    }
    KC_CUDA(cudaStreamSynchronize(ex.stream));
}

KC_HD u64 kc_mix64(u64 x) {
    x ^= x >> 30;
    x *= 0xbf58476d1ce4e5b9ULL;
    x ^= x >> 27;
    x *= 0x94d049bb133111ebULL;
    x ^= x >> 31;
    return x;
}

template <int L>
void digest_only(kc_ctx *ctx, CudaExec &ex, const DevInput &in, const kc_params &p, const u32 *win_mask, uint64_t *digest) {
    KC_CUDA(cudaEventRecord(ctx->ev[0], ex.stream));
    KmerSet<L> set = kc_kmerset_build<L>(ex, in.seq, in.n_bytes, p.k, p.complements != 0, p.min_frequency, nullptr, true, nullptr, win_mask);
    const u64 U = set.n_kept;
    kc_ull *acc = reinterpret_cast<kc_ull *>(ex.alloc<u64>(4));
    ex.fill_bytes(acc, 0, 32);
    const KWord<L> *keys = set.keys;
    const u8 *cnt = set.cnt;
    const bool counted = p.min_frequency > 1;
    ex.for_each(kc_div_up(U, 32) * 32, [=] __device__(u64 i) {
        u64 h = 0, wv = 0;
        if (i < U) {
            h = kc_mix64(keys[i].w[0] + 0x9e3779b97f4a7c15ULL);
#pragma unroll
            for (int l = 1; l < L; ++l) h = kc_mix64(h ^ (keys[i].w[l] + 0x9e3779b97f4a7c15ULL * (u64) (l + 1)));
            wv = counted ? h * ((u64) cnt[i] + 1) : h;
        }
        u64 s = h, x = h;
#pragma unroll
        for (int o = 16; o > 0; o >>= 1) {
            s += __shfl_xor_sync(0xFFFFFFFFu, s, o);
            x ^= __shfl_xor_sync(0xFFFFFFFFu, x, o);
            wv += __shfl_xor_sync(0xFFFFFFFFu, wv, o);
        }
        if ((threadIdx.x & 31) == 0) {
// ... 113 lines not shown
        const size_t top_mark = ex.arena->top, mark = ex.arena->mark();
        ExtFlags ext;
        ext.flags = reinterpret_cast<const u32 *>(G.heap + G.lay.off_flags);
        ext.cells4 = kc_grp_sig_flags<L>(G, ex, in.seq, nb, p.k, p.complements != 0, ctx->sig);
        if (ext.cells4) {
            run_pipeline<L>(ctx, ex, in, p, res, &ext, false, (u32) G.rank, (u32) G.n);
            if (!ext.aborted) {
                ++ctx->sig_runs;
                finish();
                return;
            }
            if (ext.kept & 2u) {
                G.failed = true;
                KC_THROW(KC_ERR_INTERNAL, "a rank of the group did not arrive (wait timed out)");
            }
            ++ctx->sig_fallbacks;
            ctx->sig_overflow_bytes = nb;
        }
        ex.arena->release(mark);
        ex.arena->top = top_mark;
    }
    const KsfGroupPlan gp = kc_ksf_group_plan(nb, G.n, KsCfg<L>::EX_TILE, ctx->fast);
    const bool expect_duplicates = ctx->fast_heuristics && (p.min_frequency > 1 || (ctx->fast_overflow_bytes && nb >= ctx->fast_overflow_bytes / 2 && nb <= ctx->fast_overflow_bytes * 2));
    if (gp.ok && !expect_duplicates && gp.recv_items() <= G.lay.recv_items) {
        const size_t top_mark = ex.arena->top, mark = ex.arena->mark();
        ExtFlags ext;
        ext.flags = reinterpret_cast<const u32 *>(G.heap + G.lay.off_flags);
        ext.cells4 = kc_grp_fast_flags<L>(G, ex, in.seq, nb, p.k, p.complements != 0, p.min_frequency, gp, ctx->fast);
        run_pipeline<L>(ctx, ex, in, p, res, &ext, false, (u32) G.rank, (u32) G.n);
        if (!ext.aborted) {
            ++ctx->fast_runs;
            finish();
            return;
        }
        if (ext.kept & 2u) {
            G.failed = true;
            KC_THROW(KC_ERR_INTERNAL, "a rank of the group did not arrive (wait timed out)");
        }
        ++ctx->fast_fallbacks;
        ctx->fast_overflow_bytes = nb;
        ex.arena->release(mark);
        ex.arena->top = top_mark;
    }
    ExtFlags ext;
    ext.flags = kc_grp_exact_flags<L>(G, ex, in.seq, nb, p.k, p.complements != 0, p.min_frequency, &ext.kept, &ext.n_occ);
    run_pipeline<L>(ctx, ex, in, p, res, &ext, false, (u32) G.rank, (u32) G.n);
    finish();
}

void group_check_job(kc_ctx *ctx, const kc_params *p, u64 n_bytes) {
    check_params(p);
    KcGroup &G = ctx->grp;
    if (!G.attached()) KC_THROW(KC_ERR_ARG, "this context is not part of a group");
    for (int r = 0; r < G.n; ++r)
        if (!G.peer[r]) KC_THROW(KC_ERR_ARG, "the group's heaps have not been opened");
    if (G.failed) KC_THROW(KC_ERR_INTERNAL, "the group lost its synchronisation in an earlier call; create a new one");
    if (p->assume_simplitigs || p->want_maxone) KC_THROW(KC_ERR_ARG, "the multi-GPU construction supports neither -S nor -M");
    if (kc_limbs_for_k(p->k) > G.lay.limbs) KC_THROW(KC_ERR_ARG, "the group heap was sized for a narrower k-mer word");
    if (n_bytes > G.lay.n_bytes_cap) KC_THROW(KC_ERR_TOO_LARGE, "the input exceeds the capacity the group heap was sized for");
}


}

extern "C" {

int kc_limbs_for_k(int k) { return k < 32 ? 1 : (k < 64 ? 2 : 4); }

int kc_init(int device, void *stream, kc_ctx **out) {
    if (!out) return KC_ERR_ARG;
    *out = nullptr;
    int count = 0;
    if (cudaGetDeviceCount(&count) != cudaSuccess || count == 0 || device < 0 || device >= count) {
        (void) cudaGetLastError();
        return KC_ERR_NO_DEVICE;
    }
    kc_ctx *ctx = new (std::nothrow) kc_ctx();
    if (!ctx) return KC_ERR_OOM;
    try {
        ctx->device = device;
        KC_CUDA(cudaSetDevice(device));
        if (stream) {
            ctx->stream = (cudaStream_t) stream;
        } else {
            KC_CUDA(cudaStreamCreateWithFlags(&ctx->stream, cudaStreamNonBlocking));
            ctx->own_stream = true;
        }
        for (int i = 0; i < 6; ++i) KC_CUDA(cudaEventCreate(&ctx->ev[i]));
        KC_CUDA(cudaHostAlloc(reinterpret_cast<void **>(&ctx->pin_small), kc_ctx::KC_PIN_SMALL, cudaHostAllocDefault));
        if (const char *e = std::getenv("KC_FAST_SET")) ctx->fast.enabled = std::atoi(e) != 0;
        if (const char *e = std::getenv("KC_SIG_SET")) ctx->sig.enabled = std::atoi(e) != 0;
        if (const char *e = std::getenv("KC_FAST_MAX_CTAS")) ctx->fast.max_ctas = std::atoi(e);
        if (const char *e = std::getenv("KC_FAST_TMA")) ctx->fast.tma = std::atoi(e) != 0;
        if (const char *e = std::getenv("KC_SMALL_THREADS")) ctx->small_threads = std::atoi(e);
    } catch (const KcError &e) {
        int code = e.code;
        kc_destroy(ctx);
        return code;
    }
    *out = ctx;
    return KC_OK;
}

void kc_destroy(kc_ctx *ctx) {
    if (!ctx) return;
    cudaSetDevice(ctx->device);
    if (ctx->arena.base) cudaFree(ctx->arena.base);
    if (ctx->pin_in) cudaFreeHost(ctx->pin_in);
    if (ctx->pin_out) cudaFreeHost(ctx->pin_out);
    if (ctx->pin_small) cudaFreeHost(ctx->pin_small);
    group_detach(ctx);
    for (int i = 0; i < 6; ++i)
        if (ctx->ev[i]) cudaEventDestroy(ctx->ev[i]);
    for (int i = 0; i < kc_ctx::KC_H2D_CHUNKS; ++i)
        if (ctx->chunk_ev[i]) cudaEventDestroy(ctx->chunk_ev[i]);
    if (ctx->copy_stream) cudaStreamDestroy(ctx->copy_stream);
    for (cudaEvent_t e : ctx->prof.pool) cudaEventDestroy(e);
    if (ctx->own_stream && ctx->stream) cudaStreamDestroy(ctx->stream);
    delete ctx;
}

int kc_compute_device(kc_ctx *ctx, const kc_params *p, const kc_input *in, kc_output *out) {
    if (!ctx || !in || !out) return KC_ERR_ARG;
    KC_API_BEGIN
    check_params(p);
    check_large_input(ctx, p, in->n_bytes);
    if ((reinterpret_cast<uintptr_t>(in->seq) & 15) != 0) KC_THROW(KC_ERR_ARG, "device sequence pointer must be 16-byte aligned");
    KC_CUDA(cudaSetDevice(ctx->device));
    const int limbs = kc_limbs_for_k(p->k);
    CudaExec ex{ctx->stream, &ctx->arena};
    ex.prof = &ctx->prof;
    ex.pinned = ctx->pin_small;
    ex.pinned_cap = ctx->pin_small ? kc_ctx::KC_PIN_SMALL : 0;
    DevInput di{in->seq, in->n_bytes, in->rec_off, in->rec_len, in->n_recs};
    DevResult res;
    KC_TRACE_POINT("compute_device: start");
    const SigPlan sig = kc_sig_plan(in->n_bytes, p->k, ctx->sig);
    run_with_arena(ctx, estimate_arena(in->n_bytes, in->n_recs, limbs, p->complements != 0, p->assume_simplitigs != 0, false, &ctx->fast, &sig),
                   estimate_arena(in->n_bytes, in->n_recs, limbs, p->complements != 0, p->assume_simplitigs != 0, true, &ctx->fast, &sig),
                   [&] { dispatch_pipeline(ctx, ex, di, *p, res); });
    KC_TRACE_POINT("compute_device: launched");
    KC_CUDA(cudaStreamSynchronize(ctx->stream));
    KC_TRACE_POINT("compute_device: synced");
    out->ms = const_cast<u8 *>(res.ms);
    out->ms_maxone = const_cast<u8 *>(res.maxone);
    out->length = res.length;
    out->n_kmers = res.n_kmers;
    out->n_occurrences = res.n_occ;
    out->n_nodes = res.n_nodes;
    out->n_simplitigs = res.n_simplitigs;
    out->n_launches = ex.launches;
    fill_times(ctx, out);
    ctx->total_launches += ex.launches;
    return KC_OK;
    KC_API_END(ctx)
}

int kc_compute(kc_ctx *ctx, const kc_params *p, const kc_input *in, kc_output *out) {
    if (!ctx || !in || !out) return KC_ERR_ARG;
    KC_API_BEGIN
    check_params(p);
    check_large_input(ctx, p, in->n_bytes);
    KC_CUDA(cudaSetDevice(ctx->device));
    const int limbs = kc_limbs_for_k(p->k);
    const bool simplitigs = p->assume_simplitigs != 0;
    CudaExec ex{ctx->stream, &ctx->arena};
    ex.prof = &ctx->prof;
    ex.pinned = ctx->pin_small;
    ex.pinned_cap = ctx->pin_small ? kc_ctx::KC_PIN_SMALL : 0;
    DevResult res;
    const SigPlan sig = kc_sig_plan(in->n_bytes, p->k, ctx->sig);
    run_with_arena(ctx, estimate_arena(in->n_bytes, in->n_recs, limbs, p->complements != 0, simplitigs, false, &ctx->fast, &sig),
                   estimate_arena(in->n_bytes, in->n_recs, limbs, p->complements != 0, simplitigs, true, &ctx->fast, &sig), [&] {
        u8 *d_seq = ex.alloc<u8>(in->n_bytes + 64);
        InputChunks chunks;
        const bool chunked = !simplitigs && in->n_bytes >= (8u << 20);
        if (chunked) {
            if (!ctx->copy_stream) {
                KC_CUDA(cudaStreamCreateWithFlags(&ctx->copy_stream, cudaStreamNonBlocking));
                for (int c = 0; c < kc_ctx::KC_H2D_CHUNKS; ++c) KC_CUDA(cudaEventCreateWithFlags(&ctx->chunk_ev[c], cudaEventDisableTiming));
            }
            const u64 granule = 32768;
            chunks.chunk_bytes = (in->n_bytes / kc_ctx::KC_H2D_CHUNKS + granule) / granule * granule;
            chunks.ev = ctx->chunk_ev;
            for (u64 off = 0; off < in->n_bytes; off += chunks.chunk_bytes) {
                const u64 len = std::min<u64>(chunks.chunk_bytes, in->n_bytes - off);
                KC_CUDA(cudaMemcpyAsync(d_seq + off, in->seq + off, len, cudaMemcpyHostToDevice, ctx->copy_stream));
                KC_CUDA(cudaEventRecord(ctx->chunk_ev[chunks.n++], ctx->copy_stream));
            }
        } else {
            KC_CUDA(cudaMemcpyAsync(d_seq, in->seq, in->n_bytes, cudaMemcpyHostToDevice, ctx->stream));
        }
        u64 *d_off = nullptr, *d_len = nullptr;
        if (simplitigs) {
            d_off = ex.alloc<u64>(in->n_recs);
            d_len = ex.alloc<u64>(in->n_recs);
            KC_CUDA(cudaMemcpyAsync(d_off, in->rec_off, in->n_recs * 8, cudaMemcpyHostToDevice, ctx->stream));
            KC_CUDA(cudaMemcpyAsync(d_len, in->rec_len, in->n_recs * 8, cudaMemcpyHostToDevice, ctx->stream));
        }
        DevInput di{d_seq, in->n_bytes, d_off, d_len, in->n_recs, chunked ? &chunks : nullptr};
        try {
            dispatch_pipeline(ctx, ex, di, *p, res);
        } catch (...) {
            if (chunked) cudaStreamSynchronize(ctx->copy_stream);
            throw;
        }
        if (chunked) chunks.wait_all(ctx->stream);
    });
    const size_t need = (size_t) res.length * (res.maxone ? 2 : 1) + 64;
    if (ctx->pin_out_cap < need) {
        if (ctx->pin_out) KC_CUDA(cudaFreeHost(ctx->pin_out));
        ctx->pin_out = nullptr;
        ctx->pin_out_cap = 0;
        KC_CUDA(cudaMallocHost(&ctx->pin_out, need + need / 8));
        ctx->pin_out_cap = need + need / 8;
    }
    KC_CUDA(cudaMemcpyAsync(ctx->pin_out, res.ms, res.length, cudaMemcpyDeviceToHost, ctx->stream));
    if (res.maxone)
        KC_CUDA(cudaMemcpyAsync(ctx->pin_out + res.length, res.maxone, res.length, cudaMemcpyDeviceToHost, ctx->stream));
    KC_CUDA(cudaStreamSynchronize(ctx->stream));
    out->ms = ctx->pin_out;
    out->ms_maxone = res.maxone ? ctx->pin_out + res.length : nullptr;
    out->length = res.length;
    out->n_kmers = res.n_kmers;
    out->n_occurrences = res.n_occ;
    out->n_nodes = res.n_nodes;
    out->n_simplitigs = res.n_simplitigs;
    out->n_launches = ex.launches;
    fill_times(ctx, out);
    ctx->total_launches += ex.launches;
    return KC_OK;
    KC_API_END(ctx)
}

int kc_lower_bound(kc_ctx *ctx, const kc_params *p, const kc_input *in, uint64_t *lower_bound, kc_output *stats) {
    if (!ctx || !in || !lower_bound) return KC_ERR_ARG;
    KC_API_BEGIN
    check_params(p);
    if (p->want_maxone) KC_THROW(KC_ERR_ARG, "lowerbound has no mask output");
    if (in->n_bytes >= 0xFFFFFFF0ULL) KC_THROW(KC_ERR_TOO_LARGE, "more than 2^32 sequence bytes on one GPU");
    KC_CUDA(cudaSetDevice(ctx->device));
    const int limbs = kc_limbs_for_k(p->k);
    const bool simplitigs = p->assume_simplitigs != 0;
    CudaExec ex{ctx->stream, &ctx->arena};
    ex.prof = &ctx->prof;
    ex.pinned = ctx->pin_small;
    ex.pinned_cap = ctx->pin_small ? kc_ctx::KC_PIN_SMALL : 0;
    DevResult res;
    run_with_arena(ctx, estimate_arena(in->n_bytes, in->n_recs, limbs, p->complements != 0, simplitigs, false, &ctx->fast),
                   estimate_arena(in->n_bytes, in->n_recs, limbs, p->complements != 0, simplitigs, true, &ctx->fast), [&] {
        u8 *d_seq = ex.alloc<u8>(in->n_bytes + 64);
        KC_CUDA(cudaMemcpyAsync(d_seq, in->seq, in->n_bytes, cudaMemcpyHostToDevice, ctx->stream));
        u64 *d_off = nullptr, *d_len = nullptr;
        if (simplitigs) {
            d_off = ex.alloc<u64>(in->n_recs);
            d_len = ex.alloc<u64>(in->n_recs);
            KC_CUDA(cudaMemcpyAsync(d_off, in->rec_off, in->n_recs * 8, cudaMemcpyHostToDevice, ctx->stream));
            KC_CUDA(cudaMemcpyAsync(d_len, in->rec_len, in->n_recs * 8, cudaMemcpyHostToDevice, ctx->stream));
        }
        DevInput di{d_seq, in->n_bytes, d_off, d_len, in->n_recs};
        dispatch_pipeline(ctx, ex, di, *p, res, true);
    });
    KC_CUDA(cudaStreamSynchronize(ctx->stream));
    *lower_bound = res.lower_bound;
    if (stats) {
        std::memset(stats, 0, sizeof(*stats));
        stats->n_kmers = res.n_kmers;
        stats->n_occurrences = res.n_occ;
        stats->n_nodes = res.n_nodes;
        stats->n_simplitigs = res.n_simplitigs;
        stats->n_launches = ex.launches;
        fill_times(ctx, stats);
    }
    ctx->total_launches += ex.launches;
    return KC_OK;
    KC_API_END(ctx)
}

static u8 *copy_result_to_pinned(kc_ctx *ctx, const u8 *dev, u64 n) {
    const size_t need = (size_t) n + 64;
    if (ctx->pin_out_cap < need) {
        if (ctx->pin_out) KC_CUDA(cudaFreeHost(ctx->pin_out));
        ctx->pin_out = nullptr;
        ctx->pin_out_cap = 0;
        KC_CUDA(cudaMallocHost(&ctx->pin_out, need + need / 8));
        ctx->pin_out_cap = need + need / 8;
    }
    if (n) KC_CUDA(cudaMemcpyAsync(ctx->pin_out, dev, n, cudaMemcpyDeviceToHost, ctx->stream));
    KC_CUDA(cudaStreamSynchronize(ctx->stream));
    return ctx->pin_out;
}

int kc_streaming(kc_ctx *ctx, const kc_params *p, const kc_input *in, kc_output *out) {
    if (!ctx || !in || !out) return KC_ERR_ARG;
    KC_API_BEGIN
    check_params(p);
    if (p->assume_simplitigs || p->want_maxone) KC_THROW(KC_ERR_ARG, "-S and -M belong to the greedy algorithm");
    if (in->n_bytes >= 0xFFFFFFF0ULL) KC_THROW(KC_ERR_TOO_LARGE, "more than 2^32 sequence bytes on one GPU");
    KC_CUDA(cudaSetDevice(ctx->device));
    const int limbs = kc_limbs_for_k(p->k);
    ensure_arena(ctx, estimate_arena(in->n_bytes, 0, limbs, false, true, false, &ctx->fast));
    ctx->arena.reset();
    CudaExec ex{ctx->stream, &ctx->arena};
    ex.prof = &ctx->prof;
    ex.pinned = ctx->pin_small;
    ex.pinned_cap = ctx->pin_small ? kc_ctx::KC_PIN_SMALL : 0;
    std::memset(out, 0, sizeof(*out));
    KC_CUDA(cudaEventRecord(ctx->ev[0], ctx->stream));
    const u64 padded = (in->n_bytes + 31) / 32 * 32 + 64;
    u8 *d_seq = ex.alloc<u8>(padded);
    ex.fill_bytes(d_seq + (in->n_bytes & ~(u64) 31), '\n', padded - (in->n_bytes & ~(u64) 31));
    KC_CUDA(cudaMemcpyAsync(d_seq, in->seq, in->n_bytes, cudaMemcpyHostToDevice, ctx->stream));
    KC_CUDA(cudaEventRecord(ctx->ev[1], ctx->stream));
    StreamingResult r;
    const bool compl_ = p->complements != 0;
    if (limbs == 1) r = kc_streaming_run<1>(ex, d_seq, in->n_bytes, p->k, compl_, p->min_frequency, ctx->fast, &ctx->fast_runs, &ctx->fast_fallbacks);
    else if (limbs == 2) r = kc_streaming_run<2>(ex, d_seq, in->n_bytes, p->k, compl_, p->min_frequency, ctx->fast, &ctx->fast_runs, &ctx->fast_fallbacks);
    else r = kc_streaming_run<4>(ex, d_seq, in->n_bytes, p->k, compl_, p->min_frequency, ctx->fast, &ctx->fast_runs, &ctx->fast_fallbacks);
    for (int i = 2; i <= 4; ++i) KC_CUDA(cudaEventRecord(ctx->ev[i], ctx->stream));
    out->ms = copy_result_to_pinned(ctx, r.ms, r.length);
    out->length = r.length;
    out->n_kmers = r.n_kept;
    out->n_occurrences = r.n_occ;
    out->n_launches = ex.launches;
    fill_times(ctx, out);
    ctx->total_launches += ex.launches;
    return KC_OK;
    KC_API_END(ctx)
}

int kc_maskopt(kc_ctx *ctx, const uint8_t *ms, uint64_t n, int k, int complements, int minimize, kc_output *out) {
    if (!ctx || (!ms && n) || !out) return KC_ERR_ARG;
    KC_API_BEGIN
    if (k < 1 || k > 127) KC_THROW(KC_ERR_ARG, "k must be in 1..127");
    if (n + 1 >= 0xFFFFFFF0ULL) KC_THROW(KC_ERR_TOO_LARGE, "more than 2^32 sequence bytes on one GPU");
    KC_CUDA(cudaSetDevice(ctx->device));
    const int limbs = kc_limbs_for_k(k);
    ensure_arena(ctx, estimate_arena(n + 1, 0, limbs, false, true) + 2 * n + (minimize ? (size_t) n * (8 * limbs + 1) + n / 4 : 0));
    ctx->arena.reset();
    CudaExec ex{ctx->stream, &ctx->arena};
    ex.prof = &ctx->prof;
    ex.pinned = ctx->pin_small;
    ex.pinned_cap = ctx->pin_small ? kc_ctx::KC_PIN_SMALL : 0;
    std::memset(out, 0, sizeof(*out));
    KC_CUDA(cudaEventRecord(ctx->ev[0], ctx->stream));
    u8 *d_seq = ex.alloc<u8>(n + 64);
    ex.fill_bytes(d_seq + (n & ~(u64) 31), '\n', n + 64 - (n & ~(u64) 31));
    if (n) KC_CUDA(cudaMemcpyAsync(d_seq, ms, n, cudaMemcpyHostToDevice, ctx->stream));
    KC_CUDA(cudaEventRecord(ctx->ev[1], ctx->stream));
    MaskoptResult r;
    if (limbs == 1) r = kc_maskopt_run<1>(ex, d_seq, n, k, complements != 0, minimize != 0);
    else if (limbs == 2) r = kc_maskopt_run<2>(ex, d_seq, n, k, complements != 0, minimize != 0);
    else r = kc_maskopt_run<4>(ex, d_seq, n, k, complements != 0, minimize != 0);
    for (int i = 2; i <= 4; ++i) KC_CUDA(cudaEventRecord(ctx->ev[i], ctx->stream));
    out->ms = copy_result_to_pinned(ctx, r.ms, r.length);
    out->length = r.length;
    out->n_kmers = r.n_kmers;
    out->n_launches = ex.launches;
    fill_times(ctx, out);
    ctx->total_launches += ex.launches;
    return KC_OK;
    KC_API_END(ctx)
}

int kc_copy_to_host(kc_ctx *ctx, void *dst_host, const void *src_device, uint64_t n) {
    if (!ctx || (!dst_host && n) || (!src_device && n)) return KC_ERR_ARG;
    KC_API_BEGIN
    KC_CUDA(cudaSetDevice(ctx->device));
    if (n) KC_CUDA(cudaMemcpyAsync(dst_host, src_device, n, cudaMemcpyDeviceToHost, ctx->stream));
    KC_CUDA(cudaStreamSynchronize(ctx->stream));
    return KC_OK;
    KC_API_END(ctx)
}

int kc_count_kmers(kc_ctx *ctx, const kc_params *p, const kc_input *in, uint64_t **keys, uint8_t **counts, uint64_t *n) {
    if (!ctx || !in || !keys || !counts || !n) return KC_ERR_ARG;
    KC_API_BEGIN
    check_params(p);
    if (in->n_bytes >= 0xFFFFFFF0ULL) KC_THROW(KC_ERR_TOO_LARGE, "more than 2^32 sequence bytes on one GPU");
    KC_CUDA(cudaSetDevice(ctx->device));
    const int limbs = kc_limbs_for_k(p->k);
    size_t need = (size_t) ((double) in->n_bytes * (1.0 + 2.0 * 8 * limbs + 4.0) * 1.15) + (256u << 20);
    ensure_arena(ctx, need);
    ctx->arena.reset();
    CudaExec ex{ctx->stream, &ctx->arena};
    ex.prof = &ctx->prof;
    ex.pinned = ctx->pin_small;
    ex.pinned_cap = ctx->pin_small ? kc_ctx::KC_PIN_SMALL : 0;
    u8 *d_seq = ex.alloc<u8>(in->n_bytes + 64);
    KC_CUDA(cudaMemcpyAsync(d_seq, in->seq, in->n_bytes, cudaMemcpyHostToDevice, ctx->stream));
    DevInput di{d_seq, in->n_bytes, nullptr, nullptr, in->n_recs};
    if (p->k < 32) count_only<1>(ctx, ex, di, *p, keys, counts, n);
    else if (p->k < 64) count_only<2>(ctx, ex, di, *p, keys, counts, n);
    else count_only<4>(ctx, ex, di, *p, keys, counts, n);
    ctx->total_launches += ex.launches;
    return KC_OK;
    KC_API_END(ctx)
}

int kc_partial_presort(kc_ctx *ctx, const uint64_t *kmers, uint64_t n, int k, uint64_t *out) {
    if (!ctx || (n && (!kmers || !out))) return KC_ERR_ARG;
    KC_API_BEGIN
    if (k < 1 || k > 127) KC_THROW(KC_ERR_ARG, "k must be in 1..127");
    if (n >= 0xFFFFFFF0ULL) KC_THROW(KC_ERR_TOO_LARGE, "too many k-mers");
    if (n == 0) return KC_OK;
    KC_CUDA(cudaSetDevice(ctx->device));
    const int limbs = kc_limbs_for_k(k);
    ensure_arena(ctx, (size_t) (n * (16.0 * limbs + 64.0)) + (64u << 20));
    ctx->arena.reset();
    CudaExec ex{ctx->stream, &ctx->arena};
    ex.prof = &ctx->prof;
    ex.pinned = ctx->pin_small;
    ex.pinned_cap = ctx->pin_small ? kc_ctx::KC_PIN_SMALL : 0;
    u64 *src = ex.alloc<u64>(n * limbs), *dst = ex.alloc<u64>(n * limbs);
    KC_CUDA(cudaMemcpyAsync(src, kmers, n * limbs * 8, cudaMemcpyHostToDevice, ctx->stream));
    const int sfb = 2 * k < 8 ? 2 * k : 8;
    const int pos = 2 * k - sfb, limb = pos >> 6, off = pos & 63;
    const u64 *perm = kc_partial_presort_perm(ex, n, [=] __device__(u64 i) {
        u64 v = src[i * limbs + limb] >> off;
        if (off + sfb > 64 && limb + 1 < limbs) v |= src[i * limbs + limb + 1] << (64 - off);
        return (u32) (v & ((1u << sfb) - 1u));
    });
    ex.for_each(n * limbs, [=] __device__(u64 t) { dst[t] = src[(perm[t / limbs] & 0xFFFFFFFFULL) * limbs + t % limbs]; });
    KC_CUDA(cudaMemcpyAsync(out, dst, n * limbs * 8, cudaMemcpyDeviceToHost, ctx->stream));
    KC_CUDA(cudaStreamSynchronize(ctx->stream));
    ctx->total_launches += ex.launches;
    return KC_OK;
    KC_API_END(ctx)
}

int kc_kmer_digest(kc_ctx *ctx, const kc_params *p, const kc_input *in, int masked, uint64_t *digest) {
    if (!ctx || !in || !digest) return KC_ERR_ARG;
    KC_API_BEGIN
    check_params(p);
    if (masked && p->min_frequency != 1) KC_THROW(KC_ERR_ARG, "a masked superstring has no counts");
    if (in->n_bytes + 1 >= 0xFFFFFFF0ULL) KC_THROW(KC_ERR_TOO_LARGE, "more than 2^32 sequence bytes on one GPU");
    KC_CUDA(cudaSetDevice(ctx->device));
    const int limbs = kc_limbs_for_k(p->k);
    const u64 nb = masked ? in->n_bytes + 1 : in->n_bytes;
    size_t need = (size_t) ((double) nb * (1.0 + 2.0 * 8 * limbs + 4.0 + 0.2) * 1.15) + (256u << 20);
    ensure_arena(ctx, need);
    ctx->arena.reset();
    CudaExec ex{ctx->stream, &ctx->arena};
    ex.prof = &ctx->prof;
    ex.pinned = ctx->pin_small;
    ex.pinned_cap = ctx->pin_small ? kc_ctx::KC_PIN_SMALL : 0;
    u8 *d_seq = ex.alloc<u8>(nb + 64);
    if (in->n_bytes) KC_CUDA(cudaMemcpyAsync(d_seq, in->seq, in->n_bytes, cudaMemcpyHostToDevice, ctx->stream));
    u32 *win_mask = nullptr;
    if (masked) {
        ex.fill_bytes(d_seq + in->n_bytes, '\n', 64);
        const u64 tile = kc_shard_granule(p->k);
        const u64 mwords = kc_div_up(nb, tile) * (tile / 32) + 1;
        win_mask = ex.arena->alloc_top<u32>(mwords);
        const u64 len = in->n_bytes;
        const int k = p->k;
        u32 *wm = win_mask;
        const u8 *sq = d_seq;
        ex.for_each(mwords, [=] __device__(u64 w) {
            u32 m = 0;
            for (int i = 0; i < 32; ++i) {
                const u64 q = w * 32 + i;
                if (q + 1 >= (u64) k && q < len && sq[q + 1 - k] <= 'Z') m |= 1u << i;
            }
            wm[w] = m;
        }, KP_MISC, len + len / 8);
    }
    DevInput di{d_seq, nb, nullptr, nullptr, in->n_recs};
    if (limbs == 1) digest_only<1>(ctx, ex, di, *p, win_mask, digest);
    else if (limbs == 2) digest_only<2>(ctx, ex, di, *p, win_mask, digest);
    else digest_only<4>(ctx, ex, di, *p, win_mask, digest);
    ctx->total_launches += ex.launches;
    return KC_OK;
    KC_API_END(ctx)
}

int kc_overlap_path(kc_ctx *ctx, const uint64_t *first, const uint64_t *last, uint64_t n, int k, int complements,
                    int lower_bound, int strict, int64_t *edge_from, uint8_t *overlaps) {
    if (!ctx || !first || !last || !edge_from || !overlaps) return KC_ERR_ARG;
    KC_API_BEGIN
    if (k < 1 || k > 127) KC_THROW(KC_ERR_ARG, "k must be in 1..127");
    if (n == 0) KC_THROW(KC_ERR_EMPTY, "input cannot be empty");
    if (n * (complements ? 2 : 1) >= 0xFFFFFFF0ULL) KC_THROW(KC_ERR_TOO_LARGE, "too many nodes for one GPU");
    KC_CUDA(cudaSetDevice(ctx->device));
    const int limbs = kc_limbs_for_k(k);
    ensure_arena(ctx, estimate_arena(0, n, limbs, complements != 0, true) + n * 16 * limbs);
    ctx->arena.reset();
    CudaExec ex{ctx->stream, &ctx->arena};
    ex.prof = &ctx->prof;
    ex.pinned = ctx->pin_small;
    ex.pinned_cap = ctx->pin_small ? kc_ctx::KC_PIN_SMALL : 0;
    if (k < 32) overlap_only<1>(ctx, ex, first, last, n, k, complements != 0, lower_bound != 0, strict != 0, edge_from, overlaps);
    else if (k < 64) overlap_only<2>(ctx, ex, first, last, n, k, complements != 0, lower_bound != 0, strict != 0, edge_from, overlaps);
    else overlap_only<4>(ctx, ex, first, last, n, k, complements != 0, lower_bound != 0, strict != 0, edge_from, overlaps);
    ctx->total_launches += ex.launches;
    return KC_OK;
    KC_API_END(ctx)
}

uint64_t kc_shard_granule(int k) {
    const int limbs = kc_limbs_for_k(k);
    return limbs == 1 ? KsCfg<1>::EX_TILE : (limbs == 2 ? KsCfg<2>::EX_TILE : KsCfg<4>::EX_TILE);
}

int kc_group_alloc(kc_ctx *ctx, int n_ranks, int rank, int k, uint64_t n_bytes_cap, uint8_t *handle_out) {
    if (!ctx || !handle_out) return KC_ERR_ARG;
    KC_API_BEGIN
    group_alloc_common(ctx, n_ranks, rank, k, n_bytes_cap, false);
    cudaIpcMemHandle_t h;
    KC_CUDA(cudaIpcGetMemHandle(&h, ctx->grp.heap));
    static_assert(sizeof(cudaIpcMemHandle_t) == 64, "IPC handle size");
    std::memcpy(handle_out, &h, 64);
    return KC_OK;
    KC_API_END(ctx)
}

int kc_group_open(kc_ctx *ctx, const uint8_t *all_handles) {
    if (!ctx || !all_handles) return KC_ERR_ARG;
    KC_API_BEGIN
    KcGroup &G = ctx->grp;
    if (!G.heap) KC_THROW(KC_ERR_ARG, "kc_group_alloc first");
    KC_CUDA(cudaSetDevice(ctx->device));
    for (int r = 0; r < G.n; ++r) {
        if (r == G.rank || G.peer[r]) continue;
        cudaIpcMemHandle_t h;
        std::memcpy(&h, all_handles + (size_t) r * 64, 64);
        void *pp = nullptr;
        KC_CUDA(cudaIpcOpenMemHandle(&pp, h, cudaIpcMemLazyEnablePeerAccess));
        G.peer[r] = reinterpret_cast<char *>(pp);
        G.ipc_opened[r] = true;
    }
    return KC_OK;
    KC_API_END(ctx)
}

int kc_group_compute_device(kc_ctx *ctx, const kc_params *p, const kc_input *in, kc_output *out, uint64_t *slice_begin, uint64_t *slice_len) {
    if (!ctx || !in || !out) return KC_ERR_ARG;
    KC_API_BEGIN
    group_check_job(ctx, p, in->n_bytes);
    if ((reinterpret_cast<uintptr_t>(in->seq) & 15) != 0) KC_THROW(KC_ERR_ARG, "device sequence pointer must be 16-byte aligned");
    KC_CUDA(cudaSetDevice(ctx->device));
    const int limbs = kc_limbs_for_k(p->k);
    CudaExec ex{ctx->stream, &ctx->arena};
    ex.prof = &ctx->prof;
    ex.pinned = ctx->pin_small;
    ex.pinned_cap = ctx->pin_small ? kc_ctx::KC_PIN_SMALL : 0;
    DevInput di{in->seq, in->n_bytes, nullptr, nullptr, 0};
    DevResult res;
    ensure_arena(ctx, group_arena_need(in->n_bytes, ctx->grp.n, limbs, p->complements != 0, false));
    ctx->arena.reset();
    try {
        if (limbs == 1) group_compute_rank<1>(ctx, ex, di, *p, res);
        else if (limbs == 2) group_compute_rank<2>(ctx, ex, di, *p, res);
        else group_compute_rank<4>(ctx, ex, di, *p, res);
    } catch (const KcError &e) {
        if (e.code != KC_ERR_EMPTY) ctx->grp.failed = true;
        throw;
    }
    KC_CUDA(cudaStreamSynchronize(ctx->stream));
    if (slice_begin) *slice_begin = res.slice_begin;
    if (slice_len) *slice_len = res.slice_len;
    out->ms = const_cast<u8 *>(res.ms);
    out->ms_maxone = nullptr;
    out->length = res.length;
    out->n_kmers = res.n_kmers;
    out->n_occurrences = res.n_occ;
    out->n_nodes = res.n_nodes;
    out->n_simplitigs = res.n_simplitigs;
    out->n_launches = ex.launches;
    fill_times(ctx, out);
    ctx->total_launches += ex.launches;
    return KC_OK;
    KC_API_END(ctx)
}

int kc_group_close(kc_ctx *ctx) {
    if (!ctx) return KC_ERR_ARG;
    group_detach(ctx);
    return KC_OK;
}

int kc_group_plan(int n_ranks, int rank, int k, uint64_t n_bytes, uint64_t *plan) {
    if (!plan || n_ranks < 1 || n_ranks > KC_MAX_PEERS || rank < 0 || rank >= n_ranks || k < 1 || k > 127) return KC_ERR_ARG;
    const u64 tile = kc_shard_granule(k);
    KsfTuning tune;
    const KsfGroupPlan gp = kc_ksf_group_plan(n_bytes, n_ranks, tile, tune);
    const GrpLayout lay = kc_grp_layout(n_bytes, kc_limbs_for_k(k), n_ranks, false, tile, tune);
    const u64 tiles = kc_div_up(n_bytes, tile);
    plan[0] = gp.ok ? 1 : 0;
    plan[1] = std::min<u64>(n_bytes, tiles * (u64) rank / (u64) n_ranks * tile);
    plan[2] = std::min<u64>(n_bytes, tiles * (u64) (rank + 1) / (u64) n_ranks * tile);
    plan[3] = gp.ok ? gp.dig_begin(rank) : (u64) ((rank * 256 + n_ranks - 1) / n_ranks);
    plan[4] = gp.ok ? gp.dig_begin(rank + 1) : (u64) (((rank + 1) * 256 + n_ranks - 1) / n_ranks);
    plan[5] = gp.ok ? gp.n_digits : 256;
    plan[6] = gp.cap_sub;
    plan[7] = lay.total;
    return KC_OK;
}

struct kc_group {
    int n = 0;
    kc_ctx *ctx[KC_MAX_PEERS] = {};
    GrpHostSync hs;
    u8 *pin_out = nullptr;
    size_t pin_out_cap = 0;
    std::mutex out_mutex;
    std::string last_error;
};

static void group_release_heaps(kc_group *g) {
    for (int r = 0; r < g->n; ++r)
        if (g->ctx[r]) {
            cudaSetDevice(g->ctx[r]->device);
            cudaStreamSynchronize(g->ctx[r]->stream);
        }
    for (int r = 0; r < g->n; ++r)
        if (g->ctx[r]) group_detach(g->ctx[r]);
}

int kc_init_multi(int n_gpus, const int *device_ids, kc_group **out) {
    if (!out || !device_ids || n_gpus < 1 || n_gpus > KC_MAX_PEERS) return KC_ERR_ARG;
    *out = nullptr;
    kc_group *g = new (std::nothrow) kc_group();
    if (!g) return KC_ERR_OOM;
    g->n = n_gpus;
    int rc = KC_OK;
    {
        int rcs[KC_MAX_PEERS];
        std::vector<std::thread> th;
        for (int r = 0; r < n_gpus; ++r) th.emplace_back([&, r] { rcs[r] = kc_init(device_ids[r], nullptr, &g->ctx[r]); });
        for (auto &t : th) t.join();
        for (int r = 0; r < n_gpus; ++r)
            if (rcs[r] != KC_OK && rc == KC_OK) rc = rcs[r];
    }
    for (int a = 0; a < n_gpus && rc == KC_OK; ++a)
        for (int b = 0; b < n_gpus && rc == KC_OK; ++b) {
            const int da = device_ids[a], db = device_ids[b];
            if (da == db) continue;
            int can = 0;
            if (cudaSetDevice(da) != cudaSuccess || cudaDeviceCanAccessPeer(&can, da, db) != cudaSuccess || !can) {
                rc = KC_ERR_ARG;
                break;
            }
            const cudaError_t e = cudaDeviceEnablePeerAccess(db, 0);
            if (e != cudaSuccess && e != cudaErrorPeerAccessAlreadyEnabled) rc = KC_ERR_CUDA;
            (void) cudaGetLastError();
        }
    g->hs.n = n_gpus;
    for (int r = 0; r < n_gpus && rc == KC_OK; ++r) {
        if (cudaSetDevice(device_ids[r]) != cudaSuccess) rc = KC_ERR_CUDA;
        for (int i = 0; i < 2 && rc == KC_OK; ++i)
            if (cudaEventCreateWithFlags(&g->hs.ev[r][i], cudaEventDisableTiming) != cudaSuccess) rc = KC_ERR_CUDA;
    }
    if (rc != KC_OK) {
        kc_group_destroy(g);
        return rc;
    }
    *out = g;
    return KC_OK;
}

void kc_group_destroy(kc_group *g) {
    if (!g) return;
    group_release_heaps(g);
    for (int r = 0; r < g->n; ++r)
        if (g->ctx[r]) kc_destroy(g->ctx[r]);
    for (int r = 0; r < g->n; ++r)
        for (int i = 0; i < 2; ++i)
            if (g->hs.ev[r][i]) cudaEventDestroy(g->hs.ev[r][i]);
    if (g->pin_out) cudaFreeHost(g->pin_out);
    delete g;
}

int kc_group_size(const kc_group *g) { return g ? g->n : 0; }
kc_ctx *kc_group_ctx(kc_group *g, int rank) { return g && rank >= 0 && rank < g->n ? g->ctx[rank] : nullptr; }
const char *kc_group_last_error(const kc_group *g) { return g ? g->last_error.c_str() : ""; }

int kc_group_compute(kc_group *g, const kc_params *p, const kc_input *in, kc_output *out) {
    if (!g || !p || !in || !out) return KC_ERR_ARG;
    kc_ctx *c0 = g->ctx[0];
    try {
        check_params(p);
        if (p->assume_simplitigs || p->want_maxone) KC_THROW(KC_ERR_ARG, "the multi-GPU construction supports neither -S nor -M");
        if (in->n_bytes >= 0xFFFFFFF0ULL) KC_THROW(KC_ERR_TOO_LARGE, "more than 2^32 sequence bytes");
        const int limbs = kc_limbs_for_k(p->k);
        const KcGroup &G0 = c0->grp;
        if (!G0.attached() || in->n_bytes > G0.lay.n_bytes_cap || limbs > G0.lay.limbs || G0.failed) {
            group_release_heaps(g);
            const u64 cap = std::min<u64>(0xFFFFFFE0ULL, in->n_bytes + in->n_bytes / 16 + (1u << 20));
            for (int r = 0; r < g->n; ++r) {
                g->ctx[r]->fast = c0->fast;
                g->ctx[r]->fast_heuristics = c0->fast_heuristics;
                g->ctx[r]->fast_overflow_bytes = c0->fast_overflow_bytes;
                group_alloc_common(g->ctx[r], g->n, r, limbs == 1 ? 31 : (limbs == 2 ? 63 : 127), cap, true);
            }
            for (int r = 0; r < g->n; ++r) {
                for (int s = 0; s < g->n; ++s) g->ctx[r]->grp.peer[s] = g->ctx[s]->grp.heap;
                g->ctx[r]->grp.hs = &g->hs;
            }
        }
        {
            std::lock_guard<std::mutex> lk(g->hs.m);
            g->hs.arrived = 0;
            g->hs.aborted = false;
        }
        {
            KcError errs[KC_MAX_PEERS];
            bool bad[KC_MAX_PEERS] = {};
            std::vector<std::thread> th;
            for (int r = 0; r < g->n; ++r)
                th.emplace_back([&, r] {
                    try {
                        KC_CUDA(cudaSetDevice(g->ctx[r]->device));
                        ensure_arena(g->ctx[r], group_arena_need(in->n_bytes, g->n, limbs, p->complements != 0, false));
                    } catch (const KcError &e) {
                        errs[r] = e;
                        bad[r] = true;
                    }
                });
            for (auto &t : th) t.join();
            for (int r = 0; r < g->n; ++r)
                if (bad[r]) throw errs[r];
        }
    } catch (const KcError &e) {
        set_error(c0, e);
        g->last_error = c0->last_error;
        return e.code;
    }
    struct RankOut {
        int code = KC_OK;
        std::string what;
        DevResult res;
        u64 launches = 0;
        kc_output o;
    } ro[KC_MAX_PEERS];
    auto worker = [&](int r) {
        kc_ctx *ctx = g->ctx[r];
        RankOut &R = ro[r];
        try {
            KC_CUDA(cudaSetDevice(ctx->device));
            KcGroup &G = ctx->grp;
            ctx->arena.reset();
            CudaExec ex{ctx->stream, &ctx->arena};
            ex.prof = &ctx->prof;
            ex.pinned = ctx->pin_small;
            ex.pinned_cap = ctx->pin_small ? kc_ctx::KC_PIN_SMALL : 0;
            u8 *seq = reinterpret_cast<u8 *>(G.heap + G.lay.off_seq);
            const u64 nb = in->n_bytes;
            const u64 b = (nb * (u64) r / (u64) g->n) & ~(u64) 255, e = r == g->n - 1 ? nb : ((nb * (u64) (r + 1) / (u64) g->n) & ~(u64) 255);
            if (G.done_pending) {
                u32 *ws = reinterpret_cast<u32 *>(ex.arena->alloc_top<u64>(1));
                ex.fill_bytes(ws, 0, 8);
                kc_grp_wait(G, ex, G.done_seq, ws);
                G.done_pending = false;
            }
            if (e > b) {
                KC_CUDA(cudaMemcpyAsync(seq + b, in->seq + b, e - b, cudaMemcpyHostToDevice, ctx->stream));
                for (int s = 0; s < g->n; ++s)
                    if (s != r) KC_CUDA(cudaMemcpyAsync(G.peer[s] + G.lay.off_seq + b, seq + b, e - b, cudaMemcpyDefault, ctx->stream));
            }
            u32 *ws = reinterpret_cast<u32 *>(ex.arena->alloc_top<u64>(1));
            ex.fill_bytes(ws, 0, 8);
            const u32 s0 = ++G.seq;
            kc_grp_signal(G, ex, s0);
            kc_grp_wait(G, ex, s0, ws);
            DevInput di{seq, nb, nullptr, nullptr, 0};
            const int limbs = kc_limbs_for_k(p->k);
            if (limbs == 1) group_compute_rank<1>(ctx, ex, di, *p, R.res);
            else if (limbs == 2) group_compute_rank<2>(ctx, ex, di, *p, R.res);
            else group_compute_rank<4>(ctx, ex, di, *p, R.res);
            {
                std::lock_guard<std::mutex> lk(g->out_mutex);
                const size_t need = (size_t) R.res.length + 64;
                if (g->pin_out_cap < need) {
                    if (g->pin_out) KC_CUDA(cudaFreeHost(g->pin_out));
                    g->pin_out = nullptr;
                    g->pin_out_cap = 0;
                    KC_CUDA(cudaHostAlloc(reinterpret_cast<void **>(&g->pin_out), need + need / 8, cudaHostAllocPortable));
                    g->pin_out_cap = need + need / 8;
                }
            }
            if (R.res.slice_len)
                KC_CUDA(cudaMemcpyAsync(g->pin_out + R.res.slice_begin, R.res.ms, R.res.slice_len, cudaMemcpyDeviceToHost, ctx->stream));
            KC_CUDA(cudaStreamSynchronize(ctx->stream));
            if (ex.read(ws) & 2u) KC_THROW(KC_ERR_INTERNAL, "a rank of the group did not arrive (wait timed out)");
            R.launches = ex.launches;
            fill_times(ctx, &R.o);
            ctx->total_launches += ex.launches;
        } catch (const KcError &e) {
            R.code = e.code;
            char buf[512];
            std::snprintf(buf, sizeof(buf), "rank %d: %s (%s:%d)", r, e.what, e.file, e.line);
            R.what = buf;
            if (e.code != KC_ERR_EMPTY) {
                ctx->grp.failed = true;
                g->hs.abort();
            }
        } catch (...) {
            R.code = KC_ERR_INTERNAL;
            R.what = "rank " + std::to_string(r) + ": unknown failure";
            ctx->grp.failed = true;
            g->hs.abort();
        }
    };
    std::vector<std::thread> th;
    for (int r = 1; r < g->n; ++r) th.emplace_back(worker, r);
    worker(0);
    for (auto &t : th) t.join();
    for (int r = 0; r < g->n; ++r)
        if (ro[r].code != KC_OK) {
            if (ro[r].code != KC_ERR_EMPTY)
                for (int s = 0; s < g->n; ++s) g->ctx[s]->grp.failed = true;
            g->last_error = ro[r].what;
            c0->last_error = ro[r].what;
            return ro[r].code;
        }
    for (int r = 1; r < g->n; ++r)
        if (ro[r].res.length != ro[0].res.length || ro[r].res.n_kmers != ro[0].res.n_kmers) {
            g->last_error = "the ranks disagree on the result";
            return KC_ERR_INTERNAL;
        }
    std::memset(out, 0, sizeof(*out));
    out->ms = g->pin_out;
    out->length = ro[0].res.length;
    out->n_kmers = ro[0].res.n_kmers;
    out->n_occurrences = ro[0].res.n_occ;
    out->n_nodes = ro[0].res.n_nodes;
    out->n_simplitigs = ro[0].res.n_simplitigs;
    out->t = ro[0].o.t;
    for (int r = 0; r < g->n; ++r) {
        out->n_launches += ro[r].launches;
        if (ro[r].o.t.total_ms > out->t.total_ms) out->t = ro[r].o.t;
    }
    return KC_OK;
}

uint64_t kc_total_launches(const kc_ctx *ctx) { return ctx ? ctx->total_launches : 0; }

int kc_get_stat(const kc_ctx *ctx, const char *name, uint64_t *value) {
    if (!ctx || !name || !value) return KC_ERR_ARG;
    if (std::strcmp(name, "fast_runs") == 0) *value = ctx->fast_runs;
    else if (std::strcmp(name, "fast_fallbacks") == 0) *value = ctx->fast_fallbacks;
    else if (std::strcmp(name, "sig_runs") == 0) *value = ctx->sig_runs;
    else if (std::strcmp(name, "sig_fallbacks") == 0) *value = ctx->sig_fallbacks;
    else if (std::strcmp(name, "total_launches") == 0) *value = ctx->total_launches;
    else if (std::strcmp(name, "arena_bytes") == 0) *value = ctx->arena.cap;
    else if (std::strcmp(name, "arena_high") == 0) *value = ctx->arena.high;
    else if (std::strcmp(name, "fast_max_ctas") == 0) *value = (uint64_t) ctx->fast.max_ctas;
    else return KC_ERR_ARG;
    return KC_OK;
}

int kc_set_option(kc_ctx *ctx, const char *name, int value) {
    if (!ctx || !name) return KC_ERR_ARG;
    if (std::strcmp(name, "sparse_switch") == 0) {
        ctx->sparse_switch = value != 0;
        return KC_OK;
    }
    if (std::strcmp(name, "small_threads") == 0 && (value == 0 || value == 256 || value == 512)) {
        ctx->small_threads = value;
        return KC_OK;
    }
    if (std::strcmp(name, "small_engine") == 0) {
        ctx->small_engine = value != 0;
        return KC_OK;
    }
    if (std::strcmp(name, "fast_set") == 0) {
        ctx->fast.enabled = value != 0;
        return KC_OK;
    }
    if (std::strcmp(name, "fast_leaf_target") == 0 && value >= 1 && value <= 1024) {
        ctx->fast.leaf_target = (u32) value;
        return KC_OK;
    }
    if (std::strcmp(name, "fast_sigmas") == 0 && value >= 0) {
        ctx->fast.sigmas = (double) value;
        return KC_OK;
    }
    if (std::strcmp(name, "fast_tma") == 0 && (value == 0 || value == 1)) {
        ctx->fast.tma = value != 0;
        return KC_OK;
    }
    if (std::strcmp(name, "fast_heuristics") == 0 && (value == 0 || value == 1)) {
        ctx->fast_heuristics = value != 0;
        ctx->fast_overflow_bytes = 0;
        ctx->sig_overflow_bytes = 0;
        return KC_OK;
    }
    if (std::strcmp(name, "fast_max_ctas") == 0 && value >= 0 && value <= (1 << 20)) {
        ctx->fast.max_ctas = value;
        return KC_OK;
    }
    if (std::strcmp(name, "fast_min_items") == 0 && value >= 0) {
        ctx->fast.min_items = (u64) value;
        return KC_OK;
    }
    if (std::strcmp(name, "sig_set") == 0) {
        ctx->sig.enabled = value != 0;
        return KC_OK;
    }
    if (std::strcmp(name, "sig_load_pct") == 0 && value >= 0 && value <= 400) {
        ctx->sig.load_pct = (u32) value;
        return KC_OK;
    }
    if (std::strcmp(name, "sig_min_items") == 0 && value >= 0) {
        ctx->sig.min_items = (u64) value;
        return KC_OK;
    }
    return KC_ERR_ARG;
}

int kc_profile_enable(kc_ctx *ctx, int on) {
    if (!ctx) return KC_ERR_ARG;
    ctx->prof.enabled = on != 0;
    return KC_OK;
}
int kc_profile_count(void) { return KP_COUNT; }
int kc_profile_get(kc_ctx *ctx, int i, const char **name, double *ms, uint64_t *launches, uint64_t *bytes) {
    if (!ctx || i < 0 || i >= KP_COUNT) return KC_ERR_ARG;
    if (!ctx->prof.pending.empty()) {
        cudaStreamSynchronize(ctx->stream);
        ctx->prof.resolve();
    }
    if (name) *name = kc_prof_names[i];
    if (ms) *ms = ctx->prof.ms[i];
    if (launches) *launches = ctx->prof.launches[i];
    if (bytes) *bytes = ctx->prof.bytes[i];
    return KC_OK;
}
int kc_profile_reset(kc_ctx *ctx) {
    if (!ctx) return KC_ERR_ARG;
    cudaStreamSynchronize(ctx->stream);
    ctx->prof.resolve();
    ctx->prof.reset();
    return KC_OK;
}

void kc_free(void *p) { std::free(p); }

const char *kc_strerror(int code) {
    switch (code) {
        case KC_OK: return "ok";
        case KC_ERR_CUDA: return "CUDA error";
        case KC_ERR_ARG: return "invalid argument";
        case KC_ERR_OOM: return "out of memory";
        case KC_ERR_EMPTY: return "input contains no k-mers";
        case KC_ERR_BAD_SEQ: return "invalid sequence for -S";
        case KC_ERR_TOO_LARGE: return "input too large for one GPU";
        case KC_ERR_INTERNAL: return "internal error";
        case KC_ERR_NO_DEVICE: return "no CUDA device";
        default: return "unknown error";
    }
}

const char *kc_last_error(const kc_ctx *ctx) { return ctx ? ctx->last_error.c_str() : ""; }

}
```

### kmercamel_b200/csrc/runs.cuh

```cuda
#pragma once
#include "exec.cuh"
#include "kmerset.cuh"
#include "sort.cuh"

#ifdef __CUDACC__

static const int KC_RUN_WORDS = 4;
static const int KC_RUN_PER_THREAD = 32 * KC_RUN_WORDS;
static const int KC_RUN_TILE = 256 * KC_RUN_PER_THREAD;

KC_D void kc_runs_load(const u32 *flags, u64 word, u64 n_words, u32 (&f)[KC_RUN_WORDS], u32 &prev, u32 &next) {
#pragma unroll
    for (int j = 0; j < KC_RUN_WORDS; ++j) f[j] = word + j < n_words ? flags[word + j] : 0u;
    prev = word && word <= n_words ? flags[word - 1] >> 31 : 0u;
    next = word + KC_RUN_WORDS <= n_words ? flags[word + KC_RUN_WORDS] & 1u : 0u;
}

KC_D u32 kc_runs_starts(u32 f, u32 prev) { return f & ~((f << 1) | prev); }
KC_D u32 kc_runs_ends(u32 f, u32 next) { return f & ~((f >> 1) | (next << 31)); }

__global__ void __launch_bounds__(256) kc_runs_count_kernel(const u32 *flags, u64 n_words, u32 *block_counts, kc_ull *total_runs) {
    __shared__ u32 sw[8];
    const u64 word = ((u64) blockIdx.x * 256 + threadIdx.x) * KC_RUN_WORDS;
    u32 f[KC_RUN_WORDS], prev, next;
    kc_runs_load(flags, word, n_words, f, prev, next);
    u32 c = 0;
#pragma unroll
    for (int j = 0; j < KC_RUN_WORDS; ++j) c += __popc(kc_runs_starts(f[j], j ? f[j - 1] >> 31 : prev));
    u32 total;
    kc_block_exclusive_scan<256>(c, &total, sw);
    if (threadIdx.x == 0) {
        block_counts[blockIdx.x] = total;
        if (total) atomicAdd(total_runs, (kc_ull) total);
    }
}

__global__ void __launch_bounds__(256) kc_runs_emit_kernel(const u32 *flags, u64 n_words, const u32 *block_offsets, u64 *rec_off, u64 *rec_len) {
    __shared__ u32 sw[8];
    const u64 word = ((u64) blockIdx.x * 256 + threadIdx.x) * KC_RUN_WORDS;
    u32 f[KC_RUN_WORDS], prev, next;
    kc_runs_load(flags, word, n_words, f, prev, next);
    u32 c = 0;
#pragma unroll
    for (int j = 0; j < KC_RUN_WORDS; ++j) c += __popc(kc_runs_starts(f[j], j ? f[j - 1] >> 31 : prev));
    u32 total;
    u32 before = kc_block_exclusive_scan<256>(c, &total, sw) + block_offsets[blockIdx.x];
    if (c == 0 && (f[0] | f[1] | f[2] | f[3]) == 0) return;
    static_assert(KC_RUN_WORDS == 4, "the early exit above spells the words out");
#pragma unroll
    for (int j = 0; j < KC_RUN_WORDS; ++j) {
        const u64 base = (word + j) * 32;
        const u32 starts = kc_runs_starts(f[j], j ? f[j - 1] >> 31 : prev);
        const u32 ends = kc_runs_ends(f[j], j + 1 < KC_RUN_WORDS ? f[j + 1] & 1u : next);
        u32 s = starts;
        u32 r = before;
        while (s) {
            const int i = __ffs(s) - 1;
            s &= s - 1;
            rec_off[r++] = base + i;
        }
        u32 e = ends;
        while (e) {
            const int i = __ffs(e) - 1;
            e &= e - 1;
            rec_len[before + __popc(starts & (0xFFFFFFFFu >> (31 - i))) - 1] = base + i;
        }
        before += __popc(starts);
    }
}

struct RunNodes {
    u64 *rec_off = nullptr, *rec_len = nullptr;
    u64 n_runs = 0;
};

inline size_t kc_runs_flag_words(u64 n_pos) { return (size_t) kc_div_up(n_pos, 32) + 1; }

inline RunNodes kc_runs_from_flags(CudaExec &ex, const u32 *flags, u64 n_pos, int k, u64 *cells, u64 *host_cells, int n_cells = 2,
                                   bool *aborted = nullptr) {
    RunNodes runs;
    for (int i = 0; i < n_cells; ++i) host_cells[i] = 0;
    if (aborted) *aborted = false;
    if (n_pos == 0) return runs;
    const size_t mark = ex.arena->mark();
    const u64 n_words = kc_div_up(n_pos, 32);
    const u32 blocks = (u32) kc_div_up(n_pos, (u64) KC_RUN_TILE);
    u32 *counts = ex.alloc<u32>(blocks);
    {
        CudaExec::Scope sc(ex, KP_RUNS, n_pos / 8);
        kc_runs_count_kernel<<<blocks, 256, 0, ex.stream>>>(flags, n_words, counts, reinterpret_cast<kc_ull *>(cells + 1));
    }
    ++ex.launches;
    KC_CUDA(cudaGetLastError());
    ex.exclusive_scan_nosync(counts, counts, blocks);
    ex.read_n(cells, host_cells, (size_t) n_cells);
    if (n_cells >= 4 && host_cells[3] != 0) {
        if (aborted) *aborted = true;
        ex.arena->release(mark);
        return runs;
    }
    const u64 n_runs = host_cells[1];
    if (n_runs >= 0xFFFFFFF0ULL) KC_THROW(KC_ERR_TOO_LARGE, "too many first-occurrence runs for one GPU");
    if (n_runs == 0) {
        ex.arena->release(mark);
        return runs;
    }
    u64 *rec_off = ex.arena->alloc_top<u64>(n_runs), *rec_len = ex.arena->alloc_top<u64>(n_runs);
    {
        CudaExec::Scope sc(ex, KP_RUNS, n_pos / 8 + 16 * n_runs);
        kc_runs_emit_kernel<<<blocks, 256, 0, ex.stream>>>(flags, n_words, counts, rec_off, rec_len);
    }
    ++ex.launches;
    KC_CUDA(cudaGetLastError());
    ex.for_each(n_runs, [=] __device__(u64 r) {
        const u64 e_s = rec_off[r], e_t = rec_len[r];
        rec_len[r] = e_t - e_s + k;
        rec_off[r] = e_s - (k - 1);
    }, KP_RUNS, 32 * n_runs);
    ex.arena->release(mark);
    runs.rec_off = rec_off;
    runs.rec_len = rec_len;
    runs.n_runs = n_runs;
    return runs;
}

template <class DigitOf> u64 *kc_partial_presort_perm(CudaExec &ex, u64 n, DigitOf digit_of) {
    KWord<1> *keys = ex.alloc<KWord<1>>(n), *tmp = ex.alloc<KWord<1>>(n);
    ex.for_each(n, [=] __device__(u64 i) { keys[i].w[0] = ((u64) digit_of(i) << 32) | i; }, KP_MISC, n * 16);
    kc_sort<1>(ex, keys, tmp, n, 40);
    return reinterpret_cast<u64 *>(keys);
}

inline RunNodes kc_kmer_nodes_from_runs(CudaExec &ex, const u8 *seq, const RunNodes &runs, int k) {
    RunNodes out;
    const u64 n_runs = runs.n_runs;
    if (n_runs == 0) return out;
    const size_t mark = ex.arena->mark();
    u32 *pre = ex.alloc<u32>(n_runs + 1);
    const u64 *r_off = runs.rec_off, *r_len = runs.rec_len;
    ex.for_each(n_runs + 1, [=] __device__(u64 r) { pre[r] = r < n_runs ? (u32) (r_len[r] - (u64) k + 1) : 0u; }, KP_RUNS, n_runs * 12);
    const u64 U = ex.exclusive_scan(pre, pre, n_runs + 1);
    if (U >= 0xFFFFFFF0ULL) KC_THROW(KC_ERR_TOO_LARGE, "too many k-mer nodes for one GPU");
    u64 *n_off = ex.arena->alloc_top<u64>(U), *n_len = ex.arena->alloc_top<u64>(U);
    u64 *tmp_off = ex.alloc<u64>(U);
    ex.for_each(U, [=] __device__(u64 i) {
        const u32 r = kc_upper_bound_u32(pre, (u32) n_runs + 1, (u32) i) - 1;
        tmp_off[i] = r_off[r] + (i - pre[r]);
    }, KP_RUNS, U * 12);
    const int nb = k < 4 ? k : 4;
    const u64 *perm = kc_partial_presort_perm(ex, U, [=] __device__(u64 i) {
        u32 d = 0;
        for (int j = 0; j < nb; ++j) d = (d << 2) | (kc_nucleotide_code(seq[tmp_off[i] + j]) & 3u);
        return d;
    });
    ex.for_each(U, [=] __device__(u64 j) {
        n_off[j] = tmp_off[perm[j] & 0xFFFFFFFFULL];
        n_len[j] = (u64) k;
    }, KP_RUNS, U * 32);
    ex.arena->release(mark);
    out.rec_off = n_off;
    out.rec_len = n_len;
    out.n_runs = U;
    return out;
}

#endif
```

### kmercamel_b200/csrc/small_engine.cuh

```cuda
#pragma once

#ifdef __CUDACC__

template <int L> struct SmallCfg {
    static constexpr u32 T = L <= 2 ? 4096 : 2048;
    static constexpr u32 H = T / 2;
    static constexpr u32 NS = 1024;
    static constexpr u32 RANK_SORT = 384;
    static constexpr bool STAGE_KMERS = false;
    static constexpr size_t SMEM = (size_t) T * sizeof(KWord<L + 1>) + (size_t) H * (4 * 6 + 8 * 2) + (size_t) NS * (8 + 4 * 7 + 3) +
                                   (STAGE_KMERS ? (size_t) NS * 2 * sizeof(KWord<L>) + 16 : 0);
};

template <int L> struct SmallEngineArgs {
    NodeView<L> nv;
    PathState st;
    u32 *live_s_a, *live_p_a, *live_s_b, *live_p_b;
    u32 n_s, n_p;
    u32 *head_w, *tail_w, *slot_of;
    u64 *stamp;
    u8 *prim, *ban_flag;
    u32 *ban_i, *ban_j;
    u32 ban_cap;
    int d_start;
    bool strict;
    u32 *out;
    const u32 *lvl_mask_in;
    u32 *end_mask_s_a, *end_mask_p_a, *end_mask_s_b, *end_mask_p_b;
};

static const u32 KC_SMALL_MASK_LEVELS = 2;
template <int L> KC_HD u32 kc_small_mask_table_slots(u32 n_p) {
    u32 H2 = 64;
    while (H2 < 2 * n_p) H2 <<= 1;
    return H2;
}
template <int L> KC_HD u32 kc_small_mask_levels_per_cta(u32 n_s, u32 n_p) {
    const u32 avail = (u32) ((SmallCfg<L>::T * sizeof(KWord<L + 1>) - (size_t) (n_s + n_p) * sizeof(KWord<L>)) / 4);
    u32 G = avail / kc_small_mask_table_slots<L>(n_p);
    if (G > KC_SMALL_MASK_LEVELS) G = KC_SMALL_MASK_LEVELS;
    return G < 1 ? 1 : G;
}

template <int L>
__global__ void __launch_bounds__(256) kc_small_level_mask_kernel(NodeView<L> v, const u32 *__restrict__ ls, const u32 *__restrict__ lp, u32 n_s, u32 n_p,
                                                                  int d_start, u32 *mask_out , u32 *end_mask_s ,
                                                                  u32 *end_mask_p ) {
    extern __shared__ __align__(16) unsigned char kc_smem_raw[];
    __shared__ u32 s_hits;
    const u32 tid = threadIdx.x, NT = blockDim.x;
    KWord<L> *pk = reinterpret_cast<KWord<L> *>(kc_smem_raw), *sk = pk + n_p;
    u32 *tab = reinterpret_cast<u32 *>(sk + n_s);
    const u32 H2 = kc_small_mask_table_slots<L>(n_p);
    const u32 G = kc_small_mask_levels_per_cta<L>(n_s, n_p);
    const int d_hi = d_start - (int) (blockIdx.x * G);
    if (d_hi < 0) return;
    const u32 g = (u32) (d_hi + 1) < G ? (u32) (d_hi + 1) : G;
    for (u32 i = tid; i < n_p; i += NT) pk[i] = v.first_kmer(lp[i]);
    for (u32 i = tid; i < n_s; i += NT) sk[i] = v.last_kmer(ls[i]);
    for (u32 i = tid; i < g * H2; i += NT) tab[i] = KC_NONE;
    if (tid == 0) s_hits = 0;
    __syncthreads();
    for (u32 item = tid; item < g * n_p; item += NT) {
        const u32 lev = item / n_p, i = item - lev * n_p;
        const int d = d_hi - (int) lev;
        u32 *tb = tab + lev * H2;
        const KWord<L> key = kmer_prefix(pk[i], v.k, d);
        u64 h = 0;
#pragma unroll
        for (int q = 0; q < L; ++q) h = (h ^ key.w[q]) * 0x9E3779B97F4A7C15ULL;
        u32 sl = (u32) (h >> 40) & (H2 - 1);
        while (true) {
            const u32 old = atomicCAS(&tb[sl], KC_NONE, i);
            if (old == KC_NONE || kmer_prefix(pk[old], v.k, d) == key) break;
            sl = (sl + 1) & (H2 - 1);
        }
    }
    __syncthreads();
    constexpr u32 PROBED = 0x80000000u;
    u32 hits = 0;
    for (u32 item = tid; item < g * n_s; item += NT) {
        const u32 lev = item / n_s, i = item - lev * n_s;
        const int d = d_hi - (int) lev;
        u32 *tb = tab + lev * H2;
        const KWord<L> key = kmer_suffix(sk[i], d);
        u64 h = 0;
#pragma unroll
        for (int q = 0; q < L; ++q) h = (h ^ key.w[q]) * 0x9E3779B97F4A7C15ULL;
        u32 sl = (u32) (h >> 40) & (H2 - 1);
        while (true) {
            const u32 o = tb[sl];
            if (o == KC_NONE) break;
            if (kmer_prefix(pk[o & ~PROBED], v.k, d) == key) {
                hits |= 1u << lev;
                if (!(o & PROBED)) tb[sl] = o | PROBED;
                atomicOr(&end_mask_s[4 * i + ((u32) d >> 5)], 1u << (d & 31));
                break;
            }
            sl = (sl + 1) & (H2 - 1);
        }
    }
    if (hits) atomicOr(&s_hits, hits);
    __syncthreads();
    if (tid == 0) {
        const u32 hm = s_hits;
        for (u32 lev = 0; lev < g; ++lev)
            if ((hm >> lev) & 1u) atomicOr(&mask_out[(d_hi - (int) lev) >> 5], 1u << ((d_hi - (int) lev) & 31));
    }
    const u32 hm = s_hits;
    for (u32 item = tid; item < g * n_p; item += NT) {
        const u32 lev = item / n_p, i = item - lev * n_p;
        if (!((hm >> lev) & 1u)) continue;
        const int d = d_hi - (int) lev;
        const u32 *tb = tab + lev * H2;
        const KWord<L> key = kmer_prefix(pk[i], v.k, d);
        u64 h = 0;
#pragma unroll
        for (int q = 0; q < L; ++q) h = (h ^ key.w[q]) * 0x9E3779B97F4A7C15ULL;
        u32 sl = (u32) (h >> 40) & (H2 - 1);
        while (true) {
            const u32 o = tb[sl];
            if (kmer_prefix(pk[o & ~PROBED], v.k, d) == key) {
                if (o & PROBED) atomicOr(&end_mask_p[4 * i + ((u32) d >> 5)], 1u << (d & 31));
                break;
            }
            sl = (sl + 1) & (H2 - 1);
        }
    }
}

template <int L> __global__ void __launch_bounds__(512) kc_small_engine_kernel(SmallEngineArgs<L> a) {
    typedef KWord<L + 1> TW;
    constexpr u32 TCAP = SmallCfg<L>::T, HCAP = SmallCfg<L>::H;
    extern __shared__ __align__(16) unsigned char kc_smem_raw[];
    TW *const T0 = reinterpret_cast<TW *>(kc_smem_raw);
    TW *T = T0;
    u64 *max0 = reinterpret_cast<u64 *>(T0 + TCAP);
    u64 *max1 = max0 + HCAP;
    u32 *group_pstart = reinterpret_cast<u32 *>(max1 + HCAP);
    u32 *new_tail = group_pstart + HCAP;
    u32 *jump0 = new_tail + HCAP, *jump1 = jump0 + HCAP, *fin0 = jump1 + HCAP, *fin1 = fin0 + HCAP;
    __shared__ u32 s_groups, s_edges, s_cyc, s_bans, s_live_s, s_live_p;
    __shared__ u32 lvl_mask[4];
    __shared__ kc_ull s_min;
    const u32 tid = threadIdx.x;
    const u32 NT = blockDim.x;
    NodeView<L> v = a.nv;
    PathState s = a.st;
    u32 *head_w = a.head_w, *tail_w = a.tail_w, *slot_of = a.slot_of;
    u64 *stamp = a.stamp;
    u8 *prim = a.prim, *ban_flag = a.ban_flag;
    const bool local_state = v.N <= SmallCfg<L>::NS;
    if (local_state) {
        constexpr u32 NS = SmallCfg<L>::NS;
        u64 *l_stamp = reinterpret_cast<u64 *>(fin1 + HCAP);
        u32 *l32 = reinterpret_cast<u32 *>(l_stamp + NS);
        u8 *l8 = reinterpret_cast<u8 *>(l32 + 7 * NS);
        for (u32 i = tid; i < v.N; i += NT) {
            l32[i] = s.edge_from[i];
            l32[NS + i] = s.edge_to[i];
            l32[2 * NS + i] = s.chain_head[i];
            l32[3 * NS + i] = s.chain_tail[i];
            l8[i] = s.ovl[i];
            l8[2 * NS + i] = 0;
        }
        s.edge_from = l32;
        s.edge_to = l32 + NS;
        s.chain_head = l32 + 2 * NS;
        s.chain_tail = l32 + 3 * NS;
        head_w = l32 + 4 * NS;
        tail_w = l32 + 5 * NS;
        slot_of = l32 + 6 * NS;
        stamp = l_stamp;
        s.ovl = l8;
        prim = l8 + NS;
        ban_flag = l8 + 2 * NS;
        if constexpr (SmallCfg<L>::STAGE_KMERS) {
            KWord<L> *lk = reinterpret_cast<KWord<L> *>((reinterpret_cast<uintptr_t>(l8 + 3 * NS) + 15) & ~(uintptr_t) 15);
            for (u32 i = tid; i < v.n; i += NT) {
                lk[i] = a.nv.first[i];
                lk[NS + i] = a.nv.last[i];
            }
            v.first = lk;
            v.last = lk + NS;
        }
        __syncthreads();
    }
    u32 n_s = a.n_s, n_p = a.n_p;
    u32 *ls = a.live_s_a, *lp = a.live_p_a, *ls2 = a.live_s_b, *lp2 = a.live_p_b;
    u32 *ms = a.end_mask_s_a, *mp = a.end_mask_p_a, *ms2 = a.end_mask_s_b, *mp2 = a.end_mask_p_b;
    __shared__ u32 s_nt;
    const u32 batch = a.strict ? v.N / 16 + 1 : v.N + 1;
    const u32 done = v.complements ? 2u : 1u;
    u32 st_levels = 0, st_groups = 0, st_edges = 0, st_rounds = 0, st_bans = 0;
    long long ph[8] = {0, 0, 0, 0, 0, 0, 0, 0};
    long long ph_t = clock64();
#define KC_PH(i) do { const long long kc_now = clock64(); ph[i] += kc_now - ph_t; ph_t = kc_now; } while (0)

    if (tid < 4) lvl_mask[tid] = a.lvl_mask_in[tid];
    __syncthreads();

    KC_PH(0);
    for (int d = a.d_start; d >= 0; --d) {
        if (n_s <= done || n_p == 0) break;
        const long long lvl_t0 = clock64();
        if (!((lvl_mask[d >> 5] >> (d & 31)) & 1u)) continue;
        ++st_levels;
        const u32 n_live = n_s + n_p;
        T = T0;
        if (tid == 0) {
            s_nt = 0;
            s_groups = 0;
            s_bans = 0;
        }
        __syncthreads();
        for (u32 i = tid; i < n_live; i += NT) {
            if (i < n_s) {
                u32 x = ls[i];
                head_w[x] = s.chain_head[x];
                if ((ms[4 * i + ((u32) d >> 5)] >> (d & 31)) & 1u) T[atomicAdd(&s_nt, 1u)] = tuple_make(kmer_suffix(v.last_kmer(x), d), (u64) x);
            } else {
                u32 x = lp[i - n_s];
                tail_w[x] = s.chain_tail[x];
                if ((mp[4 * (i - n_s) + ((u32) d >> 5)] >> (d & 31)) & 1u) {
                    u64 meta = KC_ROLE_P | ((u64) (x / batch) << 32) | (u64) (u32) ~x;
                    T[atomicAdd(&s_nt, 1u)] = tuple_make(kmer_prefix(v.first_kmer(x), v.k, d), meta);
                }
            }
        }
        for (u32 i = tid; i < n_live && i <= SmallCfg<L>::RANK_SORT; i += NT) group_pstart[i] = 0;
        __syncthreads();
        const u32 nt = s_nt;
        KC_PH(1);
        if (nt <= SmallCfg<L>::RANK_SORT) {
            TW *dst = T0 + HCAP;
            const u32 P = nt ? (NT / nt < 8u ? NT / nt : 8u) : 0u;
            if (P >= 2) {
                u32 *rk = group_pstart;
                if (tid < nt * P) {
                    const u32 part = tid / nt, i = tid - part * nt;
                    const u32 j0 = part * nt / P, j1 = (part + 1) * nt / P;
                    const TW mine = T0[i];
                    u32 r = 0;
#pragma unroll 8
                    for (u32 j = j0; j < j1; ++j) r += T0[j] < mine ? 1u : 0u;
                    atomicAdd(&rk[i], r);
                }
                __syncthreads();
                for (u32 i = tid; i < nt; i += NT) dst[rk[i]] = T0[i];
            } else {
                for (u32 i = tid; i < nt; i += NT) {
                    const TW mine = T0[i];
                    u32 r = 0;
#pragma unroll 8
                    for (u32 j = 0; j < nt; ++j) r += T0[j] < mine ? 1u : 0u;
                    dst[r] = mine;
                }
            }
            T = dst;
            __syncthreads();
        } else {
            kc_block_bitonic<L + 1>(T, nt, NT);
        }
        KC_PH(2);
        for (u32 i = tid + 1; i < nt; i += NT) {
            TW p = T[i - 1], q = T[i];
            if (tuple_is_prefix(q) && !tuple_is_prefix(p) && tuple_key(p) == tuple_key(q)) group_pstart[atomicAdd(&s_groups, 1u)] = i;
        }
        __syncthreads();
        const u32 n_groups = s_groups;
        st_groups += n_groups;
        KC_PH(3);
        if (n_groups) {
            LevelCtx<L> c;
            c.nv = v;
            c.st = s;
            c.T = T;
            c.nt = nt;
            c.d = d;
            c.batch = batch;
            c.head_w = head_w;
            c.tail_w = tail_w;
            c.stamp = stamp;
            c.prim = prim;
            c.ban_flag = ban_flag;
            c.ban_i = a.ban_i;
            c.ban_j = a.ban_j;
            c.check_cycles = true;
            u32 n_bans = 0;
            while (true) {
                c.n_bans = n_bans;
                SimulatePairFn<L> sim{c, group_pstart};
                for (u32 g = tid; g < n_groups; g += NT) sim((u64) g);
                if (tid == 0) {
                    s_edges = 0;
                    s_cyc = 0;
                    s_min = ~0ULL;
                }
                __syncthreads();
                KC_PH(4);
                for (u32 i = tid; i < n_s; i += NT) {
                    u32 x = ls[i];
                    if (s.edge_from[x] != KC_NONE) {
                        u32 r = atomicAdd(&s_edges, 1u);
                        new_tail[r] = x;
                        slot_of[x] = r;
                    }
                }
                __syncthreads();
                const u32 ne = s_edges;
                if (ne == 0) break;
                for (u32 r = tid; r < ne; r += NT) {
                    u32 x = new_tail[r];
                    u32 t = s.chain_tail[s.edge_from[x]];
                    bool cont = s.edge_from[t] != KC_NONE;
                    jump0[r] = cont ? slot_of[t] : KC_NONE;
                    fin0[r] = t;
                    max0[r] = stamp[x];
                }
                __syncthreads();
                u32 *ja = jump0, *jb = jump1, *fa = fin0, *fb = fin1;
                u64 *ma = max0, *mb = max1;
                int rounds = 1;
                while ((1u << (rounds - 1)) < ne) ++rounds;
                for (int it = 0; it < rounds; ++it) {
                    for (u32 r = tid; r < ne; r += NT) {
                        u32 j = ja[r];
                        if (j == KC_NONE) {
                            jb[r] = KC_NONE;
                            fb[r] = fa[r];
                            mb[r] = ma[r];
                        } else {
                            jb[r] = ja[j];
                            fb[r] = fa[j];
                            u64 m1 = ma[r], m2 = ma[j];
                            mb[r] = m1 > m2 ? m1 : m2;
                        }
                    }
                    __syncthreads();
                    u32 *t32 = ja; ja = jb; jb = t32;
                    t32 = fa; fa = fb; fb = t32;
// ... 131 lines not shown
```

### kmercamel_b200/csrc/stage1.cuh

```cuda
#pragma once
#include "exec.cuh"
#include "kword.cuh"
#include "sort.cuh"

#ifdef __CUDACC__

static const int KC_EX_THREADS = 256;
static const int KC_EX_STRIP = 32;
static const int KC_EX_HALO = 4;

KC_D void kc_pack4(u32 w, u32 &codes, u32 &valid) {
    u32 c = ((w >> 1) ^ (w >> 2)) & 0x03030303u;
    codes = (c * 0x40100401u) >> 24;
    const u32 c0 = c & 0x01010101u, c1 = (c >> 1) & 0x01010101u;
    const u32 expect = 0x41414141u + c0 * 2u + c1 * 6u + (c0 & c1) * 11u;
    const u32 d = (w & 0xDFDFDFDFu) ^ expect;
    const u32 z = ~(((d & 0x7F7F7F7Fu) + 0x7F7F7F7Fu) | d) & 0x80808080u;
    valid = (((z >> 7) * 0x08040201u) >> 24) & 0xFu;
}

template <int L, bool WITH_POS>
__global__ void __launch_bounds__(KC_EX_THREADS) kc_extract_kernel(const u8 *__restrict__ seq, u64 n_bytes, int k, int complements,
                                                                    KWord<L + (WITH_POS ? 1 : 0)> *__restrict__ out, kc_ull *counter) {
    __shared__ u64 pk[KC_EX_HALO + KC_EX_THREADS];
// ... 18 lines not shown
                codes = (codes << 8) | c4;
                valid = (valid << 4) | v4;
            }
        } else if (p + KC_EX_STRIP > 0 && (u64) (p < 0 ? 0 : p) < n_bytes) {
            for (int j = 0; j < KC_EX_STRIP; ++j) {
                i64 q = p + j;
                u32 code = 4;
                if (q >= 0 && (u64) q < n_bytes) code = kc_nucleotide_code(seq[q]);
                codes = (codes << 2) | (code & 3);
                valid = (valid << 1) | (code < 4 ? 1u : 0u);
            }
        }
        pk[wi] = codes;
        vm[wi] = valid;
    }
    __syncthreads();

    const int widx = KC_EX_HALO + threadIdx.x;
    const u64 mine = pk[widx];
    const u32 myv = vm[widx];
    int run = 0;
#pragma unroll
    for (int w = 1; w <= KC_EX_HALO; ++w) {
        u32 pv = vm[widx - w];
        if (pv == 0xFFFFFFFFu) {
            run += 32;
        } else {
            run += __ffs(~pv) - 1;
            break;
        }
    }
    u32 em = 0;
#pragma unroll
    for (int j = 0; j < KC_EX_STRIP; ++j) {
        run = ((myv >> (31 - j)) & 1) ? run + 1 : 0;
        if (run >= k) em |= 1u << (31 - j);
    }
    const u32 cnt = __popc(em);
    u32 block_total;
    const u32 my_off = kc_block_exclusive_scan_256(cnt, &block_total, sw);
    if (threadIdx.x == 0 && block_total) block_base = atomicAdd(counter, (kc_ull) block_total);
    __syncthreads();
    if (block_total == 0) return;

    if (L == 1) {
        u64 *stage = reinterpret_cast<u64 *>(kc_smem_raw) + (threadIdx.x >> 5) * (32 * KC_EX_STRIP);
        const u32 lane = threadIdx.x & 31;
        u32 warp_off = cnt;
#pragma unroll
        for (int o = 1; o < 32; o <<= 1) {
            u32 t = __shfl_up_sync(0xFFFFFFFFu, warp_off, o);
            if (lane >= (u32) o) warp_off += t;
        }
        const u32 warp_total = __shfl_sync(0xFFFFFFFFu, warp_off, 31);
        u32 pos = warp_off - cnt;
        kc_ull gpos = block_base + my_off;
        const u64 strip_pos0 = (u64) block_pos0 + (u64) threadIdx.x * KC_EX_STRIP;
        if (em) {
            const u64 prev = pk[widx - 1];
            const u64 mask = (k == 32) ? ~0ULL : ((1ULL << (2 * k)) - 1);
            const int top = 2 * (k - 1);
            KWord<1> pw;
            pw.w[0] = prev & ((1ULL << top) - 1);
            u64 rcs = k > 1 ? kmer_reverse_complement(pw, k - 1).w[0] : 0;
#pragma unroll
            for (int j = 0; j < KC_EX_STRIP; ++j) {
                const int sh = 2 * (31 - j);
                u64 fwd = (mine >> sh);
                if (j < 31) fwd |= prev << (2 * (j + 1));
                fwd &= mask;
                u64 c = (mine >> sh) & 3;
                u64 rcf = rcs | ((3 ^ c) << top);
                rcs = rcf >> 2;
                if ((em >> (31 - j)) & 1) {
                    const u64 canon = (!complements || fwd < rcf) ? fwd : rcf;
                    if (WITH_POS) {
                        *reinterpret_cast<ulonglong2 *>(&out[gpos++]) = make_ulonglong2(strip_pos0 + j, canon);
                    } else {
                        stage[pos++] = canon;
                    }
                }
            }
        }
        if (!WITH_POS) {
            __syncwarp();
            const kc_ull warp_base = block_base + __shfl_sync(0xFFFFFFFFu, my_off, 0);
            u64 *o64 = reinterpret_cast<u64 *>(out);
            for (u32 q = lane; q < warp_total; q += 32) o64[warp_base + q] = stage[q];
        }
    } else {
        if (!em) return;
        const KWord<L> mask = KWord<L>::low_mask(2 * k);
        const int top = 2 * (k - 1);
        const int top_limb = top >> 6, top_off = top & 63;
        KWord<L> fwd = KWord<L>::zero(), rcs = KWord<L>::zero();
        for (int h = k - 1; h >= 1; --h) {
            int gp = widx * 32 - h;
            u64 c = (pk[gp >> 5] >> (2 * (31 - (gp & 31)))) & 3;
            fwd = fwd.shl(2);
            fwd.w[0] |= c;
            KWord<L> rcf = rcs;
#pragma unroll
            for (int i = 0; i < L; ++i)
                if (i == top_limb) rcf.w[i] |= (3 ^ c) << top_off;
            rcs = rcf.shr(2);
        }
        kc_ull pos = block_base + my_off;
#pragma unroll 4
        for (int j = 0; j < KC_EX_STRIP; ++j) {
            u64 c = (mine >> (2 * (31 - j))) & 3;
            fwd = fwd.shl(2);
            fwd.w[0] |= c;
            fwd = fwd & mask;
            KWord<L> rcf = rcs;
#pragma unroll
            for (int i = 0; i < L; ++i)
                if (i == top_limb) rcf.w[i] |= (3 ^ c) << top_off;
            rcs = rcf.shr(2);
            if ((em >> (31 - j)) & 1) {
                const KWord<L> canon = (!complements || fwd < rcf) ? fwd : rcf;
                KWord<L + (WITH_POS ? 1 : 0)> item;
                if (WITH_POS) item.w[0] = (u64) block_pos0 + (u64) threadIdx.x * KC_EX_STRIP + j;
#pragma unroll
                for (int i = 0; i < L; ++i) item.w[i + (WITH_POS ? 1 : 0)] = canon.w[i];
                out[pos++] = item;
            }
        }
    }
}

template <int L, bool WITH_POS>
u64 kc_extract_kmers(CudaExec &ex, const u8 *seq, u64 n_bytes, int k, bool complements, KWord<L + (WITH_POS ? 1 : 0)> *out) {
    if (n_bytes == 0) return 0;
    size_t mark = ex.arena->mark();
    kc_ull *counter = reinterpret_cast<kc_ull *>(ex.alloc<u64>(1));
    ex.fill_bytes(counter, 0, 8);
    u64 blocks = kc_div_up(n_bytes, (u64) KC_EX_THREADS * KC_EX_STRIP);
    const int smem = (L == 1 && !WITH_POS) ? 8 * 32 * KC_EX_STRIP * 8 : 0;
    static KcDevOnce attr_once;
    if (smem) attr_once.run([&](int) { KC_CUDA(cudaFuncSetAttribute(kc_extract_kernel<L, WITH_POS>, cudaFuncAttributeMaxDynamicSharedMemorySize, smem)); });
    {
        CudaExec::Scope sc(ex, KP_EXTRACT, n_bytes);
        kc_extract_kernel<L, WITH_POS><<<(unsigned) blocks, KC_EX_THREADS, smem, ex.stream>>>(seq, n_bytes, k, complements ? 1 : 0,
                                                                                               out, counter);
    }
    ++ex.launches;
    KC_CUDA(cudaGetLastError());
    u64 m = ex.read(reinterpret_cast<u64 *>(counter));
    if (ex.prof && ex.prof->enabled) ex.prof->bytes[KP_EXTRACT] += m * sizeof(KWord<L + (WITH_POS ? 1 : 0)>);
    ex.arena->release(mark);
    return m;
}

template <int L>
void kc_extract_node_ends(CudaExec &ex, const u8 *seq, u64 n_bytes, const u64 *rec_off, const u64 *rec_len, u64 n_recs, int k,
                          KWord<L> *first, KWord<L> *last, u32 *error_flag, bool validate_bytes) {
    ex.for_each(n_recs, [=] __device__(u64 r) {
        u64 off = rec_off[r], len = rec_len[r];
        if (len < (u64) k) {
            *error_flag = 1;
            return;
        }
        KWord<L> f = KWord<L>::zero(), l = KWord<L>::zero();
        for (int i = 0; i < k; ++i) {
            f = f.shl(2);
            f.w[0] |= kc_nucleotide_code(seq[off + i]) & 3;
            l = l.shl(2);
            l.w[0] |= kc_nucleotide_code(seq[off + len - k + i]) & 3;
        }
        first[r] = f;
        last[r] = l;
    });
    if (!validate_bytes) return;
    ex.for_each(n_bytes, [=] __device__(u64 p) {
        u8 c = seq[p];
        if (c != '\n' && kc_nucleotide_code(c) > 3) *error_flag = 1;
    });
}

#endif
```

Before: 74.42 billion.

## Speculatively run the small-graph tail on device without host read-backs

Adds a speculative tail path in which a device kernel derives the node counts from the run cells and initialises the graph state. The small engine and rank kernels read n and N from device memory, so the host no longer has to read sizes back and synchronise between stages. The one-CTA rank kernel now also computes the chunk prefix scan and writes the short nodes' letters, which removes several small emit launches. The cost is buffers sized to upper bounds, a fixed 512-thread engine launch in spec mode, and fallback statuses for cases the speculation cannot handle.

```diff
diff --git a/kmercamel_b200/csrc/emit.cuh b/kmercamel_b200/csrc/emit.cuh
--- a/kmercamel_b200/csrc/emit.cuh
+++ b/kmercamel_b200/csrc/emit.cuh
@@ -82,11 +82,25 @@
 
 static const u32 KC_RANK_SMALL = 1024;
 
+KC_HD u32 kc_emit_node_chunks(u64 cnt, u64 off, u64 s_begin, u64 s_end) {
+    if (cnt <= KC_EMIT_SHORT) return 0;
+    const u64 a0 = off & ~(u64) 15, a1 = off + cnt;
+    const u64 lo = a0 > s_begin ? a0 : s_begin, hi = a1 < s_end ? a1 : s_end;
+    return lo < hi ? (u32) ((hi - a0 + KC_EMIT_CHUNK - 1) / KC_EMIT_CHUNK - (lo - a0) / KC_EMIT_CHUNK) : 0u;
+}
+
 template <int L>
-__global__ void __launch_bounds__(256) kc_rank_small_kernel(PathState s, NodeSeq<L> q, u32 N, u32 *fin_out, u64 *dist_out, u64 *cell) {
+__global__ void __launch_bounds__(256) kc_rank_small_kernel(PathState s, NodeSeq<L> q, u32 N, u32 *fin_out, u64 *dist_out, u64 *cell,
+                                                            const u32 *n_dev, u32 *chunks, u8 *ms) {
     __shared__ u32 jump[2][KC_RANK_SMALL], fin[2][KC_RANK_SMALL];
     __shared__ u64 dist[2][KC_RANK_SMALL];
     __shared__ u32 s_start, s_cyc;
+    __shared__ u32 sw[8];
+    const u32 n_cells = N;
+    if (n_dev) {
+        q.n = n_dev[0];
+        N = n_dev[1];
+    }
     if (threadIdx.x == 0) {
         s_start = KC_NONE;
         s_cyc = 0;
@@ -132,6 +146,43 @@
         cell[2] = st0 < N ? dist[cur][st0] : 0;
         cell[3] = st0 < N ? fin[cur][st0] : 0;
     }
+    if (!chunks) return;
+    const u32 st0 = s_start;
+    const u64 total = st0 < N ? dist[cur][st0] : 0;
+    const u32 fin_start = st0 < N ? fin[cur][st0] : 0;
+    u32 carry = 0;
+    for (u32 t0 = 0; t0 <= n_cells; t0 += 1024) {
+        const u32 base = t0 + threadIdx.x * 4;
+        u32 c4[4], c = 0;
+#pragma unroll
+        for (int j = 0; j < 4; ++j) {
+            const u32 v = base + j;
+            c4[j] = 0;
+            if (v < N && fin[cur][v] == fin_start) {
+                const u64 cnt = q.length(v) - (s.edge_from[v] != KC_NONE ? (u64) s.ovl[v] : 0);
+                c4[j] = kc_emit_node_chunks(cnt, total - dist[cur][v], 0, total);
+            }
+            c += c4[j];
+        }
+        u32 tile;
+        u32 p = kc_block_exclusive_scan_256(c, &tile, sw) + carry;
+#pragma unroll
+        for (int j = 0; j < 4; ++j) {
+            if (base + j <= n_cells) chunks[base + j] = p;
+            p += c4[j];
+        }
+        carry += tile;
+        __syncthreads();
+    }
+    for (u32 v = threadIdx.x; v < N; v += 256) {
+        if (fin[cur][v] != fin_start) continue;
+        const u64 len = q.length(v);
+        const u64 cnt = len - (s.edge_from[v] != KC_NONE ? (u64) s.ovl[v] : 0);
+        if (cnt > KC_EMIT_SHORT) continue;
+        const u64 off = total - dist[cur][v];
+        const u64 n_upper = len - q.k + 1;
+        for (u64 j = 0; j < cnt && off + j < total; ++j) ms[off + j] = kc_letter(q.symbol(v, j), j < n_upper);
+    }
 }
 #endif
 
@@ -143,9 +194,21 @@
     u64 slice_begin = 0, slice_len = 0;
 };
 
+struct EmitSpec {
+    const u32 *n_dev;
+    u64 *cell;
+};
+
+inline void kc_emit_check(const u64 *info, u64 N, u64 total_ub) {
+    if (info[0] >= N) KC_THROW(KC_ERR_INTERNAL, "no start node: the path cover contains only cycles");
+    if (info[1] == 0) KC_THROW(KC_ERR_INTERNAL, "cycle in the final path cover");
+    if (total_ub && info[2] > total_ub) KC_THROW(KC_ERR_INTERNAL, "superstring longer than its bound");
+}
+
 template <class Exec, int L>
 EmitResult kc_emit_superstring(Exec &ex, const NodeSeq<L> &ns, const NodeView<L> &nv, const PathState &st,
-                               const KWord<L> *set_keys, u64 n_set, bool want_maxone, u32 slice_index = 0, u32 n_slices = 1, u64 total_ub = 0) {
+                               const KWord<L> *set_keys, u64 n_set, bool want_maxone, u32 slice_index = 0, u32 n_slices = 1, u64 total_ub = 0,
+                               const EmitSpec *spec = nullptr) {
     EmitResult res;
     const u64 N = nv.N;
     const int k = nv.k;
@@ -153,21 +216,31 @@
     u32 *jump_a = ex.template alloc<u32>(N), *jump_b = ex.template alloc<u32>(N);
     u32 *fin_a = ex.template alloc<u32>(N), *fin_b = ex.template alloc<u32>(N);
     u64 *dist_a = ex.template alloc<u64>(N), *dist_b = ex.template alloc<u64>(N);
-    u64 *cell = ex.template alloc<u64>(6);
+    u64 *cell = spec ? spec->cell : ex.template alloc<u64>(6);
+    const u32 *n_dev = spec ? spec->n_dev : nullptr;
     const PathState s = st;
-    const NodeSeq<L> q = ns;
+    const NodeSeq<L> q = ns, q0 = ns;
     bool ranked = false;
+    bool deferred = false;
+    u8 *ms_pre = nullptr;
+    u32 *chunks_pre = nullptr;
 #ifdef __CUDACC__
     if constexpr (Exec::is_device) {
         if (N <= KC_RANK_SMALL) {
+            deferred = total_ub && !ns.kmers && !want_maxone && n_slices == 1;
+            if (deferred) {
+                ms_pre = ex.template alloc<u8>(total_ub + 1);
+                chunks_pre = ex.template alloc<u32>(N + 1);
+            }
             typename Exec::Scope sc(ex, KP_RANK, N * 25);
-            kc_rank_small_kernel<L><<<1, 256, 0, ex.stream>>>(s, q, (u32) N, fin_a, dist_a, cell);
+            kc_rank_small_kernel<L><<<1, 256, 0, ex.stream>>>(s, q, (u32) N, fin_a, dist_a, cell, n_dev, chunks_pre, ms_pre);
             ++ex.launches;
             KC_CUDA(cudaGetLastError());
             ranked = true;
         }
     }
 #endif
+    if (spec && !deferred) KC_THROW(KC_ERR_INTERNAL, "the speculative tail needs the deferred one-CTA emission");
     if (!ranked) {
         ex.fill_bytes(cell, 0xFF, 16);
         ex.for_each(N, [=] KC_HD_LAMBDA(u64 vv) {
@@ -215,17 +288,11 @@
             });
         }
     }
-    bool deferred = false;
-#ifdef __CUDACC__
-    if constexpr (Exec::is_device) deferred = ranked && total_ub && !ns.kmers && !want_maxone && n_slices == 1;
-#endif
     const u64 *cellp = deferred ? cell : nullptr;
     u64 info[4] = {0, 1, total_ub, 0};
     if (!deferred) {
         ex.read_n(cell, info, 4);
-        const u64 start = info[0];
-        if (start >= N) KC_THROW(KC_ERR_INTERNAL, "no start node: the path cover contains only cycles");
-        if (info[1] == 0) KC_THROW(KC_ERR_INTERNAL, "cycle in the final path cover");
+        kc_emit_check(info, N, 0);
     }
     const u64 total_h = info[2];
     const u32 fin_start_h = (u32) info[3];
@@ -235,7 +302,7 @@
     const u64 s_end_h = n_slices > 1 && slice_index + 1 < n_slices ? ((total / n_slices) * (slice_index + 1)) & ~(u64) 15 : total;
     const u64 s_end = s_end_h;
     const u32 fin_start = fin_start_h;
-    u8 *ms_base = ex.template alloc<u8>(s_end - s_begin + 1);
+    u8 *ms_base = deferred ? ms_pre : ex.template alloc<u8>(s_end - s_begin + 1);
     u8 *ms = ms_base - s_begin;
     res.ms = ms_base;
     res.length = total;
@@ -254,40 +321,34 @@
             for (u32 j = 0; j < cnt; ++j) ms[off + j] = kc_letter(kmer_symbol(x, k, (int) j), j == 0);
         }, KP_EMIT, N * 12 + (u64) q.n * sizeof(KWord<L>) + total);
     } else {
-        u32 *chunks = ex.template alloc<u32>(N + 1);
-        ex.for_each(N + 1, [=] KC_HD_LAMBDA(u64 vv) {
-            const u64 total = cellp ? cellp[2] : total_h;
-            const u32 fin_start = cellp ? (u32) cellp[3] : fin_start_h;
-            const u64 s_end = cellp ? total : s_end_h;
-            u32 c = 0;
-            if (vv < N && fa[vv] == fin_start) {
-                u32 v = (u32) vv;
-                u64 cnt = q.length(v) - (s.edge_from[v] != KC_NONE ? (u64) s.ovl[v] : 0);
-                if (cnt > KC_EMIT_SHORT) {
-                    u64 off = total - da[v];
-                    const u64 a0 = off & ~(u64) 15, a1 = off + cnt;
-                    const u64 lo = a0 > s_begin ? a0 : s_begin, hi = a1 < s_end ? a1 : s_end;
-                    if (lo < hi) c = (u32) ((hi - a0 + KC_EMIT_CHUNK - 1) / KC_EMIT_CHUNK - (lo - a0) / KC_EMIT_CHUNK);
+        u32 *chunks = deferred ? chunks_pre : ex.template alloc<u32>(N + 1);
+        if (!deferred) {
+            ex.for_each(N + 1, [=] KC_HD_LAMBDA(u64 vv) {
+                u32 c = 0;
+                if (vv < N && fa[vv] == fin_start_h) {
+                    u32 v = (u32) vv;
+                    u64 cnt = q.length(v) - (s.edge_from[v] != KC_NONE ? (u64) s.ovl[v] : 0);
+                    c = kc_emit_node_chunks(cnt, total_h - da[v], s_begin, s_end_h);
                 }
-            }
-            chunks[vv] = c;
-        }, KP_EMIT, N * 12);
+                chunks[vv] = c;
+            }, KP_EMIT, N * 12);
+        }
         u32 n_chunks = 0;
         bool bounded = false;
 #ifdef __CUDACC__
         if constexpr (Exec::is_device) {
             if (N <= 65536) {
                 bounded = true;
-                ex.exclusive_scan_nosync(chunks, chunks, N + 1);
+                if (!deferred) ex.exclusive_scan_nosync(chunks, chunks, N + 1);
                 n_chunks = (u32) ((s_end - s_begin) / KC_EMIT_CHUNK + 2 * N + 1);
             }
         }
 #endif
         if (!bounded) n_chunks = ex.exclusive_scan(chunks, chunks, N + 1);
-        ex.for_each(N, [=] KC_HD_LAMBDA(u64 vv) {
-            const u64 total = cellp ? cellp[2] : total_h;
-            const u32 fin_start = cellp ? (u32) cellp[3] : fin_start_h;
-            const u64 s_end = cellp ? total : s_end_h;
+        if (!deferred) ex.for_each(N, [=] KC_HD_LAMBDA(u64 vv) {
+            const u64 total = total_h;
+            const u32 fin_start = fin_start_h;
+            const u64 s_end = s_end_h;
             u32 v = (u32) vv;
             if (fa[v] != fin_start) return;
             u64 len = q.length(v);
@@ -302,6 +363,8 @@
         ex.for_each((u64) n_chunks * 256, [=] KC_HD_LAMBDA(u64 w) {
             const u64 total = cellp ? cellp[2] : total_h;
             const u64 s_end = cellp ? total : s_end_h;
+            NodeSeq<L> q = q0;
+            if (n_dev) q.n = n_dev[0];
             u32 chunk = (u32) (w >> 8), lane = (u32) (w & 255);
             if (chunk >= chunks[N]) return;
             u32 lo = 0, hi = (u32) N;
@@ -401,11 +464,9 @@
             mo[p] = present ? (u8) (c - ('a' - 'A')) : c;
         }, KP_MAXONE, 2 * total);
     }
-    if (deferred) {
+    if (deferred && !spec) {
         ex.read_n(cell, info, 4);
-        if (info[0] >= N) KC_THROW(KC_ERR_INTERNAL, "no start node: the path cover contains only cycles");
-        if (info[1] == 0) KC_THROW(KC_ERR_INTERNAL, "cycle in the final path cover");
-        if (info[2] > total_ub) KC_THROW(KC_ERR_INTERNAL, "superstring longer than its bound");
+        kc_emit_check(info, N, total_ub);
         res.length = info[2];
         res.slice_len = info[2];
     }
diff --git a/kmercamel_b200/csrc/engine.cuh b/kmercamel_b200/csrc/engine.cuh
--- a/kmercamel_b200/csrc/engine.cuh
+++ b/kmercamel_b200/csrc/engine.cuh
@@ -263,7 +263,10 @@
 
     Engine(Exec &e, const NodeView<L> &v, bool strict_, bool lower_bound_) : ex(e), nv(v), strict(strict_), lower_bound(lower_bound_) {}
 
-    void init_state() {
+    const u32 *n_dev = nullptr;
+    u32 *small_status = nullptr, *small_masks = nullptr;
+
+    void alloc_state() {
         const u64 N = nv.N;
         st.edge_from = ex.template alloc<u32>(N);
         st.edge_to = ex.template alloc<u32>(N);
@@ -279,6 +282,11 @@
         ban_i = ex.template alloc<u32>(BAN_CAP);
         ban_j = ex.template alloc<u32>(BAN_CAP);
         ban_ctr = ex.template alloc<u32>(4);
+    }
+
+    void init_state() {
+        alloc_state();
+        const u64 N = nv.N;
         PathState s = st;
         u8 *bf = ban_flag;
         u32 *bc = ban_ctr;
@@ -311,24 +319,28 @@
 #ifdef __CUDACC__
         if constexpr (Exec::is_device) {
             if (!small_out) return;
-            u32 h[8 + 128 + 8];
-            ex.read_n(small_out, h, 8 + 128 + 8);
+            u32 h[KC_SMALL_STATUS_WORDS];
+            ex.read_n(small_out, h, KC_SMALL_STATUS_WORDS);
             small_out = nullptr;
-            if (std::getenv("KC_TRACE")) {
-                std::fprintf(stderr, "[kc_trace] small engine: n_s=%llu n_p=%llu levels=%u groups=%u edges=%u ban_rounds=%u bans=%u; clocks per level (* = run):",
-                             (unsigned long long) n_s, (unsigned long long) n_p, h[1], h[2], h[3], h[4], h[5]);
-                for (int dd = small_d; dd >= 0; --dd) std::fprintf(stderr, " d%d=%u%s", dd, h[8 + dd] & 0x7FFFFFFFu, (h[8 + dd] >> 31) ? "*" : "");
-                std::fprintf(stderr, "; phases: stage+mask=%u tuples=%u sort=%u groups=%u replay=%u validate+commit=%u lists=%u writeback=%u\n", h[136], h[137],
-                             h[138], h[139], h[140], h[141], h[142], h[143]);
-            }
-            if (h[0]) KC_THROW(KC_ERR_INTERNAL, "ban list overflow");
-            stats.levels_run += h[1];
-            stats.groups += h[2];
-            stats.edges += h[3];
-            stats.ban_rounds += h[4];
-            stats.bans += h[5];
+            apply_small_status(h);
         }
 #endif
+    }
+
+    void apply_small_status(const u32 *h) {
+        if (std::getenv("KC_TRACE")) {
+            std::fprintf(stderr, "[kc_trace] small engine: n_s=%llu n_p=%llu levels=%u groups=%u edges=%u ban_rounds=%u bans=%u; clocks per level (* = run):",
+                         (unsigned long long) n_s, (unsigned long long) n_p, h[1], h[2], h[3], h[4], h[5]);
+            for (int dd = small_d; dd >= 0; --dd) std::fprintf(stderr, " d%d=%u%s", dd, h[8 + dd] & 0x7FFFFFFFu, (h[8 + dd] >> 31) ? "*" : "");
+            std::fprintf(stderr, "; phases: stage+mask=%u tuples=%u sort=%u groups=%u replay=%u validate+commit=%u lists=%u writeback=%u\n", h[136], h[137],
+                         h[138], h[139], h[140], h[141], h[142], h[143]);
+        }
+        if (h[0]) KC_THROW(KC_ERR_INTERNAL, "ban list overflow");
+        stats.levels_run += h[1];
+        stats.groups += h[2];
+        stats.edges += h[3];
+        stats.ban_rounds += h[4];
+        stats.bans += h[5];
     }
 
     bool run_small(int d) {
@@ -364,9 +376,16 @@
             a.ban_cap = BAN_CAP;
             a.d_start = d;
             a.strict = strict;
-            a.out = ex.template alloc<u32>(8 + 128 + 8 + 4 + 8 * (n_s + n_p));
-            u32 *lvl_mask = a.out + (8 + 128 + 8);
-            ex.fill_bytes(a.out, 0, (8 + 128 + 8 + 4 + 4 * (n_s + n_p)) * 4);
+            u32 *lvl_mask;
+            if (n_dev) {
+                a.out = small_status;
+                lvl_mask = small_masks;
+            } else {
+                a.out = ex.template alloc<u32>(KC_SMALL_STATUS_WORDS + kc_small_mask_words(n_s, n_p) + 4 * (n_s + n_p));
+                lvl_mask = a.out + KC_SMALL_STATUS_WORDS;
+                ex.fill_bytes(a.out, 0, (KC_SMALL_STATUS_WORDS + kc_small_mask_words(n_s, n_p)) * 4);
+            }
+            a.n_dev = n_dev;
             a.lvl_mask_in = lvl_mask;
             a.end_mask_s_a = lvl_mask + 4;
             a.end_mask_p_a = a.end_mask_s_a + 4 * n_s;
@@ -383,18 +402,19 @@
                 typename Exec::Scope sc(ex, KP_SMALL_ENGINE, 0);
                 const u32 per_cta = kc_small_mask_levels_per_cta<L>((u32) n_s, (u32) n_p);
                 kc_small_level_mask_kernel<L><<<(unsigned) kc_div_up((u64) d + 1, per_cta), 256, mask_smem, ex.stream>>>(nv, live_s, live_p, (u32) n_s, (u32) n_p, d,
-                                                                                                                      lvl_mask, a.end_mask_s_a, a.end_mask_p_a);
+                                                                                                                      lvl_mask, a.end_mask_s_a, a.end_mask_p_a, n_dev);
                 ++ex.launches;
             }
             {
                 typename Exec::Scope sc(ex, KP_SMALL_ENGINE, 0);
                 const u64 nt0 = n_s + n_p;
-                const unsigned small_threads = small_threads_opt ? (unsigned) small_threads_opt : ((nt0 > 128 && nt0 <= 256) || nt0 > 512 ? 512u : 256u);
+                const unsigned small_threads = small_threads_opt ? (unsigned) small_threads_opt
+                                               : n_dev || (nt0 > 128 && nt0 <= 256) || nt0 > 512 ? 512u : 256u;
                 kc_small_engine_kernel<L><<<1, small_threads, SmallCfg<L>::SMEM, ex.stream>>>(a);
             }
             ++ex.launches;
             KC_CUDA(cudaGetLastError());
-            small_out = a.out;
+            small_out = n_dev ? nullptr : a.out;
             small_d = d;
             return true;
         }
diff --git a/kmercamel_b200/csrc/exec.cuh b/kmercamel_b200/csrc/exec.cuh
--- a/kmercamel_b200/csrc/exec.cuh
+++ b/kmercamel_b200/csrc/exec.cuh
@@ -195,6 +195,7 @@
     Arena *arena;
     KernelProf *prof = nullptr;
     u64 launches = 0;
+    u64 read_backs = 0;
     u8 *pinned = nullptr;
     size_t pinned_cap = 0;
 
@@ -245,6 +246,7 @@
     void sync() { KC_CUDA(cudaStreamSynchronize(stream)); }
     template <typename T> void read_n(const T *p, T *host, size_t n) {
         const size_t bytes = n * sizeof(T);
+        ++read_backs;
         if (pinned && bytes <= pinned_cap) {
             KC_CUDA(cudaMemcpyAsync(pinned, p, bytes, cudaMemcpyDeviceToHost, stream));
             KC_CUDA(cudaStreamSynchronize(stream));
diff --git a/kmercamel_b200/csrc/kcgpu.cu b/kmercamel_b200/csrc/kcgpu.cu
--- a/kmercamel_b200/csrc/kcgpu.cu
+++ b/kmercamel_b200/csrc/kcgpu.cu
@@ -12,6 +12,7 @@
 #include "runs.cuh"
 #include "sort.cuh"
 #include "stage1.cuh"
+#include "tail_spec.cuh"
 
 #include <chrono>
 #include <mutex>
@@ -56,6 +57,10 @@
     bool fast_heuristics = true;
     u64 fast_overflow_bytes = 0;
     u64 total_launches = 0;
+    u64 read_backs = 0;
+    bool tail_spec = true;
+    u64 tail_spec_runs = 0, tail_spec_fallbacks = 0;
+    u64 spec_fail_bytes = 0;
     KcGroup grp;
     bool arena_limited = false;
     std::string last_error;
@@ -188,7 +193,91 @@
 }
 
 template <int L>
-u64 run_stage1_runs(kc_ctx *ctx, CudaExec &ex, const DevInput &in, const kc_params &p, RunNodes *runs, KWord<L> **set_out, u64 *n_occ) {
+u32 run_tail_spec(kc_ctx *ctx, CudaExec &ex, const DevInput &in, const kc_params &p, const u32 *flags, u64 *blk, DevResult &res) {
+    const u64 nb = in.n_bytes;
+    const int k = p.k;
+    const bool complements = p.complements != 0;
+    const size_t mark = ex.arena->mark();
+    const u32 C = KC_SPEC_RUNS, N_cap = complements ? 2 * C : C;
+    const u64 n_words = kc_div_up(nb, 32);
+    const u32 blocks = (u32) kc_div_up(nb, (u64) KC_RUN_TILE);
+    u32 *counts = ex.alloc<u32>(blocks);
+    u64 *rec_off = ex.alloc<u64>(C), *rec_len = ex.alloc<u64>(C);
+    kc_ull *n_runs = reinterpret_cast<kc_ull *>(blk + 1);
+    {
+        CudaExec::Scope sc(ex, KP_RUNS, nb / 8);
+        kc_runs_count_kernel<<<blocks, 256, 0, ex.stream>>>(flags, n_words, counts, n_runs);
+        kc_runs_emit_kernel<<<blocks, 256, 0, ex.stream>>>(flags, n_words, counts, rec_off, rec_len, n_runs, C);
+    }
+    ex.launches += 2;
+    KC_CUDA(cudaGetLastError());
+    KC_CUDA(cudaEventRecord(ctx->ev[2], ex.stream));
+    NodeView<L> nv;
+    nv.k = k;
+    nv.complements = complements;
+    nv.n = C;
+    nv.N = N_cap;
+    KWord<L> *first = ex.alloc<KWord<L>>(C), *last = ex.alloc<KWord<L>>(C);
+    nv.first = first;
+    nv.last = last;
+    Engine<CudaExec, L> eng(ex, nv, false, false);
+    eng.small_threads_opt = ctx->small_threads;
+    eng.alloc_state();
+    u32 *spec = reinterpret_cast<u32 *>(blk + KC_SPEC_SPEC);
+    eng.n_dev = spec + 1;
+    eng.small_status = reinterpret_cast<u32 *>(blk + KC_SPEC_SMALL);
+    const u64 mask_words = kc_small_mask_words(N_cap, N_cap);
+    eng.small_masks = ex.alloc<u32>(mask_words + 4 * (u64) (2 * N_cap));
+    eng.live_s = ex.alloc<u32>(N_cap);
+    eng.live_p = ex.alloc<u32>(N_cap);
+    eng.n_s = eng.n_p = N_cap;
+    {
+        CudaExec::Scope sc(ex, KP_RUNS, 32 * (u64) C);
+        kc_spec_nodes_kernel<L><<<1, 1024, 0, ex.stream>>>(blk, spec, ctx->sparse_switch, complements, in.seq, k, rec_off, rec_len, first, last,
+                                                            eng.st, eng.ban_flag, eng.ban_ctr, eng.live_s, eng.live_p, eng.small_masks, (u32) mask_words);
+    }
+    ++ex.launches;
+    KC_CUDA(cudaGetLastError());
+    static_assert(4 * KC_SPEC_RUNS <= SmallCfg<L>::T && 2 * KC_SPEC_RUNS <= SmallCfg<L>::NS && 2 * KC_SPEC_RUNS <= KC_RANK_SMALL,
+                  "the speculative tail runs on the one-CTA kernels");
+    eng.run();
+    KC_CUDA(cudaEventRecord(ctx->ev[3], ex.stream));
+    NodeSeq<L> ns;
+    ns.k = k;
+    ns.kmers = nullptr;
+    ns.seq = in.seq;
+    ns.rec_off = rec_off;
+    ns.rec_len = rec_len;
+    ns.n = C;
+    const EmitSpec es{spec + 1, blk + KC_SPEC_EMIT};
+    const u64 total_ub = nb + (u64) C * k + 16;
+    const EmitResult er = kc_emit_superstring<CudaExec, L>(ex, ns, nv, eng.st, nullptr, 0, false, 0, 1, total_ub, &es);
+    KC_CUDA(cudaEventRecord(ctx->ev[4], ex.stream));
+    KC_TRACE_POINT("tail_spec: queued");
+    u64 h[KC_SPEC_BLOCK_WORDS];
+    ex.read_n(blk, h, KC_SPEC_BLOCK_WORDS);
+    const u32 *hs = reinterpret_cast<const u32 *>(h + KC_SPEC_SPEC);
+    if (hs[0] != KC_SPEC_OK) {
+        ex.arena->release(mark);
+        return hs[0];
+    }
+    eng.apply_small_status(reinterpret_cast<const u32 *>(h + KC_SPEC_SMALL));
+    kc_emit_check(h + KC_SPEC_EMIT, hs[2], total_ub);
+    res.ms = er.ms;
+    res.maxone = nullptr;
+    res.length = h[KC_SPEC_EMIT + 2];
+    res.slice_begin = 0;
+    res.slice_len = res.length;
+    res.n_kmers = h[0];
+    res.n_occ = h[2];
+    res.n_nodes = hs[1];
+    res.n_simplitigs = hs[1];
+    return KC_SPEC_OK;
+}
+
+template <int L>
+u64 run_stage1_runs(kc_ctx *ctx, CudaExec &ex, const DevInput &in, const kc_params &p, RunNodes *runs, KWord<L> **set_out, u64 *n_occ,
+                    DevResult *spec_res = nullptr, bool *spec_done = nullptr) {
     KC_CUDA(cudaEventRecord(ctx->ev[0], ex.stream));
     KC_CUDA(cudaEventRecord(ctx->ev[1], ex.stream));
     KC_TRACE_POINT("stage1: begin");
@@ -202,13 +291,30 @@
     const bool large = nb >= KC_POS32_BYTES;
     const bool sig_overflowed = ctx->fast_heuristics && ctx->sig_overflow_bytes && nb >= ctx->sig_overflow_bytes / 2 && nb <= ctx->sig_overflow_bytes * 2;
     if (!p.want_maxone && p.min_frequency == 1 && (large || !sig_overflowed)) {
-        u64 *cells4 = ex.arena->alloc_top<u64>(4);
-        ex.fill_bytes(cells4, 0, 32);
+        const size_t n_cells = spec_res ? KC_SPEC_BLOCK_WORDS : 4;
+        u64 *cells4 = ex.arena->alloc_top<u64>(n_cells);
+        ex.fill_bytes(cells4, 0, n_cells * 8);
         if (kc_kmerset_build_sig<L>(ex, in.seq, nb, p.k, p.complements != 0, flags, cells4, ctx->sig, in.chunks)) {
             KC_TRACE_POINT("stage1: signature set launched");
             u64 hc[4];
             bool aborted = false;
-            *runs = kc_runs_from_flags(ex, flags, nb, p.k, cells4, hc, 4, &aborted);
+            if (spec_res) {
+                const u32 st = run_tail_spec<L>(ctx, ex, in, p, flags, cells4, *spec_res);
+                if (st == KC_SPEC_OK) {
+                    ++ctx->sig_runs;
+                    ++ctx->tail_spec_runs;
+                    *spec_done = true;
+                    return spec_res->n_kmers;
+                }
+                ++ctx->tail_spec_fallbacks;
+                if (st == KC_SPEC_SIG_OVERFLOW) {
+                    aborted = true;
+                } else {
+                    if (st != KC_SPEC_EMPTY) ctx->spec_fail_bytes = nb;
+                    ex.fill_bytes(cells4 + 1, 0, 8);
+                }
+            }
+            if (!aborted) *runs = kc_runs_from_flags(ex, flags, nb, p.k, cells4, hc, 4, &aborted);
             if (!aborted) {
                 ++ctx->sig_runs;
                 *n_occ = hc[2];
@@ -318,7 +424,12 @@
             n_occ = ext->n_occ;
             KC_CUDA(cudaEventRecord(ctx->ev[2], ex.stream));
         } else {
-            U = run_stage1_runs<L>(ctx, ex, in, p, &runs, &uniq, &n_occ);
+            const u64 nb = in.n_bytes;
+            const bool spec_failed = ctx->fast_heuristics && ctx->spec_fail_bytes && nb >= ctx->spec_fail_bytes / 2 && nb <= ctx->spec_fail_bytes * 2;
+            const bool spec = ctx->tail_spec && !spec_failed && !lower_bound && ctx->small_engine && nb > 0 && nb < KC_POS32_BYTES;
+            bool spec_done = false;
+            U = run_stage1_runs<L>(ctx, ex, in, p, &runs, &uniq, &n_occ, spec ? &res : nullptr, &spec_done);
+            if (spec_done) return;
         }
         if (U == 0) KC_THROW(KC_ERR_EMPTY, "the input contains no k-mers");
         res.n_simplitigs = runs.n_runs;
@@ -738,6 +849,7 @@
     out->n_launches = ex.launches;
     fill_times(ctx, out);
     ctx->total_launches += ex.launches;
+    ctx->read_backs += ex.read_backs;
     return KC_OK;
     KC_API_END(ctx)
 }
@@ -815,6 +927,7 @@
     out->n_launches = ex.launches;
     fill_times(ctx, out);
     ctx->total_launches += ex.launches;
+    ctx->read_backs += ex.read_backs;
     return KC_OK;
     KC_API_END(ctx)
 }
@@ -859,6 +972,7 @@
         fill_times(ctx, stats);
     }
     ctx->total_launches += ex.launches;
+    ctx->read_backs += ex.read_backs;
     return KC_OK;
     KC_API_END(ctx)
 }
@@ -911,6 +1025,7 @@
     out->n_launches = ex.launches;
     fill_times(ctx, out);
     ctx->total_launches += ex.launches;
+    ctx->read_backs += ex.read_backs;
     return KC_OK;
     KC_API_END(ctx)
 }
@@ -945,6 +1060,7 @@
     out->n_launches = ex.launches;
     fill_times(ctx, out);
     ctx->total_launches += ex.launches;
+    ctx->read_backs += ex.read_backs;
     return KC_OK;
     KC_API_END(ctx)
 }
@@ -980,6 +1096,7 @@
     else if (p->k < 64) count_only<2>(ctx, ex, di, *p, keys, counts, n);
     else count_only<4>(ctx, ex, di, *p, keys, counts, n);
     ctx->total_launches += ex.launches;
+    ctx->read_backs += ex.read_backs;
     return KC_OK;
     KC_API_END(ctx)
 }
@@ -1011,6 +1128,7 @@
     KC_CUDA(cudaMemcpyAsync(out, dst, n * limbs * 8, cudaMemcpyDeviceToHost, ctx->stream));
     KC_CUDA(cudaStreamSynchronize(ctx->stream));
     ctx->total_launches += ex.launches;
+    ctx->read_backs += ex.read_backs;
     return KC_OK;
     KC_API_END(ctx)
 }
@@ -1057,6 +1175,7 @@
     else if (limbs == 2) digest_only<2>(ctx, ex, di, *p, win_mask, digest);
     else digest_only<4>(ctx, ex, di, *p, win_mask, digest);
     ctx->total_launches += ex.launches;
+    ctx->read_backs += ex.read_backs;
     return KC_OK;
     KC_API_END(ctx)
 }
@@ -1080,6 +1199,7 @@
     else if (k < 64) overlap_only<2>(ctx, ex, first, last, n, k, complements != 0, lower_bound != 0, strict != 0, edge_from, overlaps);
     else overlap_only<4>(ctx, ex, first, last, n, k, complements != 0, lower_bound != 0, strict != 0, edge_from, overlaps);
     ctx->total_launches += ex.launches;
+    ctx->read_backs += ex.read_backs;
     return KC_OK;
     KC_API_END(ctx)
 }
@@ -1156,6 +1276,7 @@
     out->n_launches = ex.launches;
     fill_times(ctx, out);
     ctx->total_launches += ex.launches;
+    ctx->read_backs += ex.read_backs;
     return KC_OK;
     KC_API_END(ctx)
 }
@@ -1373,6 +1494,7 @@
             R.launches = ex.launches;
             fill_times(ctx, &R.o);
             ctx->total_launches += ex.launches;
+            ctx->read_backs += ex.read_backs;
         } catch (const KcError &e) {
             R.code = e.code;
             char buf[512];
@@ -1430,6 +1552,9 @@
     else if (std::strcmp(name, "sig_runs") == 0) *value = ctx->sig_runs;
     else if (std::strcmp(name, "sig_fallbacks") == 0) *value = ctx->sig_fallbacks;
     else if (std::strcmp(name, "total_launches") == 0) *value = ctx->total_launches;
+    else if (std::strcmp(name, "read_backs") == 0) *value = ctx->read_backs;
+    else if (std::strcmp(name, "tail_spec_runs") == 0) *value = ctx->tail_spec_runs;
+    else if (std::strcmp(name, "tail_spec_fallbacks") == 0) *value = ctx->tail_spec_fallbacks;
     else if (std::strcmp(name, "arena_bytes") == 0) *value = ctx->arena.cap;
     else if (std::strcmp(name, "arena_high") == 0) *value = ctx->arena.high;
     else if (std::strcmp(name, "fast_max_ctas") == 0) *value = (uint64_t) ctx->fast.max_ctas;
@@ -1451,6 +1576,11 @@
         ctx->small_engine = value != 0;
         return KC_OK;
     }
+    if (std::strcmp(name, "tail_spec") == 0 && (value == 0 || value == 1)) {
+        ctx->tail_spec = value != 0;
+        ctx->spec_fail_bytes = 0;
+        return KC_OK;
+    }
     if (std::strcmp(name, "fast_set") == 0) {
         ctx->fast.enabled = value != 0;
         return KC_OK;
@@ -1471,6 +1601,7 @@
         ctx->fast_heuristics = value != 0;
         ctx->fast_overflow_bytes = 0;
         ctx->sig_overflow_bytes = 0;
+        ctx->spec_fail_bytes = 0;
         return KC_OK;
     }
     if (std::strcmp(name, "fast_max_ctas") == 0 && value >= 0 && value <= (1 << 20)) {
diff --git a/kmercamel_b200/csrc/runs.cuh b/kmercamel_b200/csrc/runs.cuh
--- a/kmercamel_b200/csrc/runs.cuh
+++ b/kmercamel_b200/csrc/runs.cuh
@@ -35,18 +35,31 @@
     }
 }
 
-__global__ void __launch_bounds__(256) kc_runs_emit_kernel(const u32 *flags, u64 n_words, const u32 *block_offsets, u64 *rec_off, u64 *rec_len) {
+__global__ void __launch_bounds__(256) kc_runs_emit_kernel(const u32 *flags, u64 n_words, const u32 *block_offsets, u64 *rec_off, u64 *rec_len,
+                                                           const kc_ull *spec_total = nullptr, u64 spec_cap = 0) {
     __shared__ u32 sw[8];
+    if (spec_total && *spec_total > spec_cap) return;
     const u64 word = ((u64) blockIdx.x * 256 + threadIdx.x) * KC_RUN_WORDS;
     u32 f[KC_RUN_WORDS], prev, next;
     kc_runs_load(flags, word, n_words, f, prev, next);
-    u32 c = 0;
+    u32 c = 0, any = 0;
 #pragma unroll
-    for (int j = 0; j < KC_RUN_WORDS; ++j) c += __popc(kc_runs_starts(f[j], j ? f[j - 1] >> 31 : prev));
+    for (int j = 0; j < KC_RUN_WORDS; ++j) {
+        c += __popc(kc_runs_starts(f[j], j ? f[j - 1] >> 31 : prev));
+        any |= kc_runs_ends(f[j], j + 1 < KC_RUN_WORDS ? f[j + 1] & 1u : next);
+    }
+    if (!__syncthreads_or(c | any)) return;
     u32 total;
-    u32 before = kc_block_exclusive_scan<256>(c, &total, sw) + block_offsets[blockIdx.x];
-    if (c == 0 && (f[0] | f[1] | f[2] | f[3]) == 0) return;
-    static_assert(KC_RUN_WORDS == 4, "the early exit above spells the words out");
+    u32 before = kc_block_exclusive_scan<256>(c, &total, sw);
+    if (spec_total) {
+        u32 sum = 0;
+        for (u32 b = threadIdx.x; b < blockIdx.x; b += 256) sum += block_offsets[b];
+        u32 all;
+        kc_block_exclusive_scan<256>(sum, &all, sw);
+        before += all;
+    } else {
+        before += block_offsets[blockIdx.x];
+    }
 #pragma unroll
     for (int j = 0; j < KC_RUN_WORDS; ++j) {
         const u64 base = (word + j) * 32;
diff --git a/kmercamel_b200/csrc/small_engine.cuh b/kmercamel_b200/csrc/small_engine.cuh
--- a/kmercamel_b200/csrc/small_engine.cuh
+++ b/kmercamel_b200/csrc/small_engine.cuh
@@ -1,4 +1,7 @@
 #pragma once
+
+static const u32 KC_SMALL_STATUS_WORDS = 8 + 128 + 8;
+KC_HD u64 kc_small_mask_words(u64 n_s, u64 n_p) { return 4 + 4 * (n_s + n_p); }
 
 #ifdef __CUDACC__
 
@@ -27,6 +30,7 @@
     u32 *out;
     const u32 *lvl_mask_in;
     u32 *end_mask_s_a, *end_mask_p_a, *end_mask_s_b, *end_mask_p_b;
+    const u32 *n_dev;
 };
 
 static const u32 KC_SMALL_MASK_LEVELS = 2;
@@ -45,14 +49,19 @@
 template <int L>
 __global__ void __launch_bounds__(256) kc_small_level_mask_kernel(NodeView<L> v, const u32 *__restrict__ ls, const u32 *__restrict__ lp, u32 n_s, u32 n_p,
                                                                   int d_start, u32 *mask_out , u32 *end_mask_s ,
-                                                                  u32 *end_mask_p ) {
+                                                                  u32 *end_mask_p , const u32 *n_dev ) {
     extern __shared__ __align__(16) unsigned char kc_smem_raw[];
     __shared__ u32 s_hits;
     const u32 tid = threadIdx.x, NT = blockDim.x;
+    const u32 G = kc_small_mask_levels_per_cta<L>(n_s, n_p);
+    if (n_dev) {
+        v.n = n_dev[0];
+        v.N = n_dev[1];
+        n_s = n_p = v.N;
+    }
     KWord<L> *pk = reinterpret_cast<KWord<L> *>(kc_smem_raw), *sk = pk + n_p;
     u32 *tab = reinterpret_cast<u32 *>(sk + n_s);
     const u32 H2 = kc_small_mask_table_slots<L>(n_p);
-    const u32 G = kc_small_mask_levels_per_cta<L>(n_s, n_p);
     const int d_hi = d_start - (int) (blockIdx.x * G);
     if (d_hi < 0) return;
     const u32 g = (u32) (d_hi + 1) < G ? (u32) (d_hi + 1) : G;
@@ -146,6 +155,10 @@
     const u32 tid = threadIdx.x;
     const u32 NT = blockDim.x;
     NodeView<L> v = a.nv;
+    if (a.n_dev) {
+        v.n = a.n_dev[0];
+        v.N = a.n_dev[1];
+    }
     PathState s = a.st;
     u32 *head_w = a.head_w, *tail_w = a.tail_w, *slot_of = a.slot_of;
     u64 *stamp = a.stamp;
@@ -186,7 +199,7 @@
         }
         __syncthreads();
     }
-    u32 n_s = a.n_s, n_p = a.n_p;
+    u32 n_s = a.n_dev ? v.N : a.n_s, n_p = a.n_dev ? v.N : a.n_p;
     u32 *ls = a.live_s_a, *lp = a.live_p_a, *ls2 = a.live_s_b, *lp2 = a.live_p_b;
     u32 *ms = a.end_mask_s_a, *mp = a.end_mask_p_a, *ms2 = a.end_mask_s_b, *mp2 = a.end_mask_p_b;
     __shared__ u32 s_nt;
diff --git a/kmercamel_b200/csrc/stage1.cuh b/kmercamel_b200/csrc/stage1.cuh
--- a/kmercamel_b200/csrc/stage1.cuh
+++ b/kmercamel_b200/csrc/stage1.cuh
@@ -194,6 +194,18 @@
     return m;
 }
 
+template <int L> KC_D void kc_node_end_kmers(const u8 *seq, u64 off, u64 len, int k, KWord<L> &first, KWord<L> &last) {
+    KWord<L> f = KWord<L>::zero(), l = KWord<L>::zero();
+    for (int i = 0; i < k; ++i) {
+        f = f.shl(2);
+        f.w[0] |= kc_nucleotide_code(seq[off + i]) & 3;
+        l = l.shl(2);
+        l.w[0] |= kc_nucleotide_code(seq[off + len - k + i]) & 3;
+    }
+    first = f;
+    last = l;
+}
+
 template <int L>
 void kc_extract_node_ends(CudaExec &ex, const u8 *seq, u64 n_bytes, const u64 *rec_off, const u64 *rec_len, u64 n_recs, int k,
                           KWord<L> *first, KWord<L> *last, u32 *error_flag, bool validate_bytes) {
@@ -203,15 +215,7 @@
             *error_flag = 1;
             return;
         }
-        KWord<L> f = KWord<L>::zero(), l = KWord<L>::zero();
-        for (int i = 0; i < k; ++i) {
-            f = f.shl(2);
-            f.w[0] |= kc_nucleotide_code(seq[off + i]) & 3;
-            l = l.shl(2);
-            l.w[0] |= kc_nucleotide_code(seq[off + len - k + i]) & 3;
-        }
-        first[r] = f;
-        last[r] = l;
+        kc_node_end_kmers<L>(seq, off, len, k, first[r], last[r]);
     });
     if (!validate_bytes) return;
     ex.for_each(n_bytes, [=] __device__(u64 p) {
diff --git a/kmercamel_b200/csrc/tail_spec.cuh b/kmercamel_b200/csrc/tail_spec.cuh
--- /dev/null
+++ b/kmercamel_b200/csrc/tail_spec.cuh
@@ -0,0 +1,54 @@
+#pragma once
+#include "engine.cuh"
+#include "runs.cuh"
+#include "stage1.cuh"
+
+static const u32 KC_SPEC_RUNS = 512;
+
+static const u32 KC_SPEC_SPEC = 4, KC_SPEC_EMIT = 6, KC_SPEC_SMALL = 12;
+static const u32 KC_SPEC_BLOCK_WORDS = KC_SPEC_SMALL + KC_SMALL_STATUS_WORDS / 2;
+
+enum KcSpecStatus : u32 { KC_SPEC_OK = 0, KC_SPEC_SIG_OVERFLOW = 1, KC_SPEC_EMPTY = 2, KC_SPEC_TOO_MANY = 3, KC_SPEC_SPARSE = 4 };
+
+#ifdef __CUDACC__
+
+template <int L>
+__global__ void __launch_bounds__(1024) kc_spec_nodes_kernel(const u64 *cells, u32 *spec, bool sparse_switch, bool complements, const u8 *seq, int k,
+                                                            u64 *rec_off, u64 *rec_len, KWord<L> *first, KWord<L> *last, PathState st, u8 *ban_flag,
+                                                            u32 *ban_ctr, u32 *live_s, u32 *live_p, u32 *masks, u32 mask_words) {
+    const u64 kept = cells[0], runs = cells[1], M = cells[2];
+    const u64 U = M ? kept : 0;
+    const u32 status = cells[3] ? KC_SPEC_SIG_OVERFLOW
+                       : U == 0 ? KC_SPEC_EMPTY
+                       : runs > KC_SPEC_RUNS ? KC_SPEC_TOO_MANY
+                       : sparse_switch && runs * 5 >= U ? KC_SPEC_SPARSE
+                                                        : KC_SPEC_OK;
+    const u32 n = status == KC_SPEC_OK ? (u32) runs : 0u, N = complements ? 2 * n : n;
+    if (threadIdx.x == 0) {
+        spec[0] = status;
+        spec[1] = n;
+        spec[2] = N;
+    }
+    if (status != KC_SPEC_OK) return;
+    for (u32 r = threadIdx.x; r < n; r += blockDim.x) {
+        const u64 e_s = rec_off[r], e_t = rec_len[r];
+        const u64 off = e_s - (k - 1), len = e_t - e_s + k;
+        rec_off[r] = off;
+        rec_len[r] = len;
+        kc_node_end_kmers<L>(seq, off, len, k, first[r], last[r]);
+    }
+    for (u32 v = threadIdx.x; v < N; v += blockDim.x) {
+        st.edge_from[v] = KC_NONE;
+        st.edge_to[v] = KC_NONE;
+        st.ovl[v] = 255;
+        ban_flag[v] = 0;
+        st.chain_head[v] = v;
+        st.chain_tail[v] = v;
+        live_s[v] = v;
+        live_p[v] = v;
+    }
+    for (u32 i = threadIdx.x; i < mask_words; i += blockDim.x) masks[i] = 0;
+    if (threadIdx.x < 4) ban_ctr[threadIdx.x] = 0;
+}
+
+#endif
diff --git a/profiles/step_timeline.py b/profiles/step_timeline.py
--- /dev/null
+++ b/profiles/step_timeline.py
@@ -0,0 +1,66 @@
+import argparse
+import json
+import os
+import sys
+
+ROOT = os.path.dirname(os.path.dirname(os.path.abspath(__file__)))
+sys.path.insert(0, ROOT)
+
+
+def main():
+    ap = argparse.ArgumentParser()
+    ap.add_argument("--out", default=None, help="also write the table as JSON here")
+    ap.add_argument("--steps", type=int, default=5)
+    args = ap.parse_args()
+    import torch
+    from torch.profiler import ProfilerActivity, profile
+    import kmercamel_b200 as kb
+    from kmercamel_b200 import synth
+
+    seq = synth.frame_records(synth.random_genome_records(50, 1_000_000, 12345))[0]
+    d = torch.from_numpy(seq).cuda()
+    ctx = kb.Context(0, torch.cuda.current_stream().cuda_stream)
+    for _ in range(5):
+        ctx.compute_device(d.data_ptr(), d.numel(), k=31)
+    torch.cuda.synchronize()
+    with profile(activities=[ProfilerActivity.CPU, ProfilerActivity.CUDA]) as prof:
+        for i in range(args.steps):
+            with torch.profiler.record_function(f"step{i}"):
+                ctx.compute_device(d.data_ptr(), d.numel(), k=31)
+            torch.cuda.synchronize()
+    events = prof.events()
+    kern = sorted([e for e in events if e.device_type == torch.autograd.DeviceType.CUDA and "memcpy" not in e.name.lower()
+                   and "memset" not in e.name.lower()], key=lambda e: e.time_range.start)
+    steps = sorted([e for e in events if e.name.startswith("step")], key=lambda e: e.time_range.start)
+    last = steps[-1]
+    mine = [e for e in kern if e.time_range.start >= last.time_range.start]
+    ops = sorted([e for e in events if e.device_type == torch.autograd.DeviceType.CUDA and e.time_range.start >= last.time_range.start
+                  and not e.name.startswith("step")],
+                 key=lambda e: e.time_range.start)
+    rows = []
+    prev_end = None
+    for e in ops:
+        gap = 0.0 if prev_end is None else max(0.0, e.time_range.start - prev_end)
+        rows.append({"name": e.name[:90], "us": round(e.time_range.end - e.time_range.start, 2), "gap_before_us": round(gap, 2)})
+        prev_end = max(prev_end or 0, e.time_range.end)
+    busy = sum(r["us"] for r in rows)
+    gaps = sum(r["gap_before_us"] for r in rows)
+    span = ops[-1].time_range.end - ops[0].time_range.start if ops else 0.0
+    print(f"{'kernel / copy':92s} {'us':>8s} {'gap before':>10s}")
+    for r in rows:
+        print(f"{r['name']:92s} {r['us']:8.2f} {r['gap_before_us']:10.2f}")
+    summary = {"gpu": torch.cuda.get_device_name(0), "kernels": len(mine), "device_ops": len(rows), "busy_us": round(busy, 1),
+               "idle_gaps_us": round(gaps, 1), "span_us": round(span, 1), "read_backs_per_step": None}
+    try:
+        r0 = ctx.stat("read_backs")
+        ctx.compute_device(d.data_ptr(), d.numel(), k=31)
+        summary["read_backs_per_step"] = ctx.stat("read_backs") - r0
+    except kb.KcError:
+        pass
+    print(json.dumps(summary))
+    if args.out:
+        json.dump({"summary": summary, "ops": rows}, open(args.out, "w"), indent=1)
+
+
+if __name__ == "__main__":
+    main()
```

Result: faster. 79.65 billion, median of 6 (+7.0%).
